# GabrieleCocco/CLFaceDetection

Hardware: AMD Instinct MI355X
Metric: candidate windows/sec, 1080p, haarcascade_frontalface_alt (higher is better)
Workload: dtype u32 gathers + f32 stage sums; 1 GPU; BASELINE config 3: 64x1920x1080 8-bit frames per step in the whole job (noise/smooth/blocks mix; sharded by whole frames over 1 GPU), haarcascade_frontalface_alt, scaleFactor 1.1f, raw candidates, frames resident in HBM; frames_on_rank_0=64, windows_per_frame=6290352, parallelism=single GPU, device=AMD Radeon Graphics (gfx950:sramecc+:xnack-), 256 CUs, pipeline=vj_stream, two batches in flight

## Files before the change

### clfacedetection_amd/api.py

```python
from __future__ import annotations

import ctypes as C
import os
from dataclasses import dataclass

import numpy as np

from .build import LIB_PATH, build_lib

VJ_MAX_STAGES = 64
VJ_FLAG_COUNTERS = 1 << 0
VJ_FLAG_SIGNED_MEAN = 1 << 1
VJ_FLAG_SKIP_LIST = 1 << 2
VJ_FLAG_SKIP_ROW = 1 << 3
VJ_FLAG_GRID_F64 = 1 << 4
VJ_FLAG_TILTED_AS_UPRIGHT = 1 << 5
VJ_FLAG_CV_CANNY_PRUNING = 1 << 6
VJ_FLAG_CV_SCALE_IMAGE = 1 << 7
VJ_FLAG_CV_FIND_BIGGEST = 1 << 8
VJ_FLAG_CV_ROUGH_SEARCH = 1 << 9
VJ_FLAG_CV_CHAIN_DEVICE = 1 << 10
VJ_FLAG_EQUALIZE_HIST = 1 << 11

CV_HAAR_DO_CANNY_PRUNING = 1
# ... 123 lines not shown
    _fields_ = [("min_w", C.c_int32), ("min_h", C.c_int32), ("max_w", C.c_int32), ("max_h", C.c_int32),
                ("scale_factor", C.c_double), ("min_neighbors", C.c_uint32), ("flags", C.c_uint32)]


class _RocResult(C.Structure):
    _fields_ = [("r", _Result), ("reject_levels", C.c_void_p), ("level_weights", C.c_void_p)]


WINDOW_DTYPE = np.dtype([("frame", "<i4"), ("x", "<i4"), ("y", "<i4"), ("scale", "<i4")])
WINDOW_RESULT_DTYPE = np.dtype([("result", "<i4"), ("reserved", "<i4"), ("stage_sum", "<f8")])
CLOD_WINDOW_RESULT_DTYPE = np.dtype([("result", "<i4"), ("variance", "<f4"), ("stage_sum", "<f4"), ("reserved", "<i4")])
VJ_WINDOW_OUTSIDE = -2**31
RECT_DTYPE = np.dtype([("x", "<i4"), ("y", "<i4"), ("w", "<i4"), ("h", "<i4"), ("weight", "<f4"),
                       ("frame", "<i4"), ("scale_idx", "<i4")])
STAGE_DTYPE = np.dtype([("first_tree", "<i4"), ("n_trees", "<i4"), ("threshold", "<f4"), ("parent", "<i4"),
                        ("next", "<i4"), ("child", "<i4")])
TREE_DTYPE = np.dtype([("first_node", "<i4"), ("n_nodes", "<i4"), ("first_alpha", "<i4")])
_RECT_DESC = np.dtype([("x", "<i4"), ("y", "<i4"), ("w", "<i4"), ("h", "<i4"), ("weight", "<f4")])
NODE_DTYPE = np.dtype([("n_rects", "<i4"), ("tilted", "<i4"), ("threshold", "<f4"), ("left", "<i4"),
                       ("right", "<i4"), ("rect", _RECT_DESC, 3)])

_SIGNATURES = {
    "vj_strerror": (C.c_char_p, [C.c_int]),
    "vj_last_error": (C.c_char_p, []),
    "vj_cascade_load_xml": (C.c_int, [C.c_char_p, C.POINTER(C.c_void_p)]),
    "vj_cascade_load": (C.c_int, [C.c_char_p, C.POINTER(C.c_void_p)]),
    "vj_cascade_save": (C.c_int, [C.c_void_p, C.c_char_p]),
    "vj_cascade_from_arrays": (C.c_int, [C.c_int, C.c_int, C.c_void_p, C.c_int, C.c_void_p, C.c_int, C.c_void_p, C.c_int,
                                         C.c_void_p, C.c_int, C.POINTER(C.c_void_p)]),
    "vj_cascade_free": (None, [C.c_void_p]),
    "vj_cascade_get_info": (C.c_int, [C.c_void_p, C.POINTER(CascadeInfo)]),
    "vj_cascade_stages": (C.c_void_p, [C.c_void_p]),
    "vj_cascade_trees": (C.c_void_p, [C.c_void_p]),
    "vj_cascade_nodes": (C.c_void_p, [C.c_void_p]),
    "vj_cascade_alpha": (C.c_void_p, [C.c_void_p]),
    "vj_cascade_notice": (C.c_char_p, [C.c_void_p]),
    "vj_params_default": (None, [C.POINTER(Params)]),
    "vj_plan_scales": (C.c_int, [C.c_void_p, C.c_int, C.c_int, C.POINTER(Params), C.POINTER(ScaleInfo), C.c_int,
                                 C.POINTER(C.c_int)]),
    "vj_plan_feature_table": (C.c_int, [C.c_void_p, C.c_int, C.POINTER(ScaleInfo), C.c_void_p, C.c_void_p]),
    "vj_plan_tiles": (C.c_int, [C.c_void_p, C.c_int, C.c_int, C.POINTER(Params), C.c_int, C.c_uint32, C.POINTER(TilePlanInfo),
                                C.POINTER(TileInfo), C.c_int, C.POINTER(C.c_int)]),
    "vj_plan_tiles_split": (C.c_int, [C.c_void_p, C.c_int, C.c_int, C.POINTER(Params), C.c_int, C.c_uint32, C.c_float,
                                      C.POINTER(TilePlanInfo), C.POINTER(TileCutInfo), C.POINTER(TileInfo), C.POINTER(C.c_uint64),
                                      C.c_int, C.POINTER(C.c_int)]),
    "vj_env_create": (C.c_int, [C.c_int, C.POINTER(C.c_void_p)]),
    "vj_env_destroy": (None, [C.c_void_p]),
    "vj_env_reserve": (C.c_int, [C.c_void_p, C.c_int, C.c_int, C.c_int]),
    "vj_env_device_name": (C.c_int, [C.c_void_p, C.c_char_p, C.c_size_t]),
    "vj_env_configure": (C.c_int, [C.c_void_p, C.c_char_p, C.c_char_p]),
    "vj_env_query": (C.c_int, [C.c_void_p, C.c_char_p, C.c_char_p, C.c_size_t]),
    "vj_integral": (C.c_int, [C.c_void_p, C.c_void_p, C.c_int, C.c_int, C.c_int, C.c_void_p, C.c_void_p]),
    "vj_integral_image": (C.c_int, [C.c_void_p, C.c_void_p, C.c_void_p, C.c_void_p]),
    "vj_integral_tilted": (C.c_int, [C.c_void_p, C.c_void_p, C.c_void_p]),
    "vj_grayscale": (C.c_int, [C.c_void_p, C.c_void_p, C.c_void_p, C.c_int]),
    "vj_canny": (C.c_int, [C.c_void_p, C.c_void_p, C.c_void_p, C.c_int]),
    "vj_equalize_hist": (C.c_int, [C.c_void_p, C.c_void_p, C.c_void_p, C.c_int]),
    "vj_resize_linear": (C.c_int, [C.c_void_p, C.c_void_p, C.c_int, C.c_int, C.c_void_p, C.c_int]),
    "vj_host_alloc": (C.c_int, [C.c_void_p, C.c_size_t, C.POINTER(C.c_void_p)]),
    "vj_host_free": (None, [C.c_void_p, C.c_void_p]),
    "vj_detect_chain": (C.c_int, [C.c_void_p, C.c_void_p, C.c_void_p, C.POINTER(_Image), C.c_int, C.POINTER(Params),
                                  C.POINTER(Params), C.POINTER(_Result), C.POINTER(_Result)]),
    "vj_stream_create": (C.c_int, [C.c_void_p, C.c_void_p, C.c_int, C.c_int, C.c_int, C.c_int, C.POINTER(Params),
                                   C.POINTER(C.c_void_p)]),
    "vj_stream_submit": (C.c_int, [C.c_void_p, C.POINTER(_Image), C.c_int]),
    "vj_stream_collect": (C.c_int, [C.c_void_p, C.POINTER(_Result)]),
    "vj_stream_destroy": (None, [C.c_void_p]),
    "vj_detect_rois": (C.c_int, [C.c_void_p, C.c_void_p, C.POINTER(_Image), C.c_int, C.c_void_p, C.c_int, C.POINTER(Params),
                                 C.POINTER(_Result)]),
    "vj_detect_opencv": (C.c_int, [C.c_void_p, C.c_void_p, C.POINTER(_Image), C.c_int, C.POINTER(CvParams),
                                   C.POINTER(_Result)]),
    "vj_detect_opencv_rois": (C.c_int, [C.c_void_p, C.c_void_p, C.POINTER(_Image), C.c_int, C.c_void_p, C.c_int, C.POINTER(CvParams),
                                        C.POINTER(_Result)]),
    "vj_detect_opencv_chain": (C.c_int, [C.c_void_p, C.c_void_p, C.c_void_p, C.POINTER(_Image), C.c_int, C.POINTER(CvParams),
                                         C.POINTER(CvParams), C.POINTER(_Result), C.POINTER(_Result)]),
    "vj_cv_params_default": (None, [C.POINTER(CvParams)]),
    "vj_cv_roc_params_default": (None, [C.POINTER(CvRocParams)]),
    "vj_detect_opencv_roc": (C.c_int, [C.c_void_p, C.c_void_p, C.POINTER(_Image), C.c_int, C.POINTER(CvRocParams),
                                       C.POINTER(_RocResult)]),
    "vj_roc_result_free": (None, [C.POINTER(_RocResult)]),
    "vj_run_windows_opencv": (C.c_int, [C.c_void_p, C.c_void_p, C.POINTER(_Image), C.c_int, C.c_void_p, C.c_int, C.c_void_p, C.c_uint32,
                                        C.c_int, C.c_void_p]),
    "vj_run_windows": (C.c_int, [C.c_void_p, C.c_void_p, C.POINTER(_Image), C.c_int, C.c_void_p, C.c_int, C.c_void_p, C.c_uint32,
                                 C.c_int, C.c_uint32, C.c_void_p]),
    "vj_run_windows_timing": (C.c_int, [C.c_void_p, C.POINTER(C.c_float), C.POINTER(C.c_float)]),
    "vj_cv_chain_info_get": (C.c_int, [C.c_void_p, C.POINTER(CvChainInfo)]),
    "vj_cv_rois_info_get": (C.c_int, [C.c_void_p, C.POINTER(CvRoisInfo)]),
    "vj_cv_plan_info_get": (C.c_int, [C.c_void_p, C.c_void_p, C.c_int, C.c_int, C.c_int, C.POINTER(CvParams), C.POINTER(CvPlanInfo)]),
    "vj_detect": (C.c_int, [C.c_void_p, C.c_void_p, C.POINTER(_Image), C.c_int, C.POINTER(Params),
                            C.POINTER(_Result)]),
    "vj_detect_mixed": (C.c_int, [C.c_void_p, C.c_void_p, C.POINTER(_Image), C.c_int, C.POINTER(Params), C.POINTER(MixedOpts),
                                  C.POINTER(_Result)]),
    "vj_detect_opencv_mixed": (C.c_int, [C.c_void_p, C.c_void_p, C.POINTER(_Image), C.c_int, C.POINTER(CvParams), C.POINTER(MixedOpts),
                                         C.POINTER(_Result)]),
    "vj_pack_frames": (C.c_int, [C.c_void_p, C.POINTER(_Image), C.c_int, C.c_uint64, C.c_void_p, C.c_int, C.POINTER(C.c_int),
                                 C.POINTER(C.c_int), C.c_void_p]),
    "vj_mixed_info_get": (C.c_int, [C.c_void_p, C.POINTER(MixedInfo)]),
    "vj_result_free": (None, [C.POINTER(_Result)]),
    "vj_group_rectangles": (C.c_int, [C.c_void_p, C.POINTER(C.c_uint32), C.c_int, C.c_double]),
    "vj_group_rectangles_levels": (C.c_int, [C.c_void_p, C.c_void_p, C.c_void_p, C.c_int, C.c_int, C.c_double]),
    "vj_count_windows": (C.c_int, [C.c_void_p, C.c_int, C.c_int, C.POINTER(Params), C.POINTER(C.c_uint64)]),
    "vj_shard_frames": (C.c_int, [C.c_int, C.c_int, C.c_int, C.POINTER(C.c_int), C.POINTER(C.c_int)]),
    "vj_shard_scales": (C.c_int, [C.c_void_p, C.c_int, C.c_int, C.POINTER(Params), C.c_int, C.c_int, C.POINTER(C.c_uint64)]),
}

_lib = None
# ... 172 lines not shown
    passes: list = None
    launches: list = None
    tile_split: float = 0.0
    balance_state: int = 0
    balance_calls: int = 0
    reject_levels: np.ndarray = None
    level_weights: np.ndarray = None

    @property
    def match_count(self) -> int:
        return len(self.rects)


class Environment:

    def __init__(self, device_index: int = 0):
        h = C.c_void_p()
        _check(load_library().vj_env_create(device_index, C.byref(h)), "vj_env_create")
        self._h = h

    @property
    def device_name(self) -> str:
        buf = C.create_string_buffer(256)
        _check(load_library().vj_env_device_name(self._h, buf, 256), "vj_env_device_name")
        return buf.value.decode()

    def configure(self, key: str, value) -> None:
        _check(load_library().vj_env_configure(self._h, key.encode(), str(value).encode()), f"vj_env_configure({key})")

    def query(self, key: str) -> str:
        buf = C.create_string_buffer(1024)
        _check(load_library().vj_env_query(self._h, key.encode(), buf, len(buf)), f"vj_env_query({key})")
        return buf.value.decode()

    def reserve(self, width: int, height: int, batch: int = 1):
        _check(load_library().vj_env_reserve(self._h, width, height, batch), "vj_env_reserve")

    def integral(self, gray: np.ndarray) -> tuple[np.ndarray, np.ndarray]:
        if gray.dtype != np.uint8 or gray.ndim not in (2, 3):
            raise ValueError("integral expects a 2-D uint8 image or a (h, w, 3|4) uint8 BGR/BGRA image")
        s = np.empty((gray.shape[0] + 1, gray.shape[1] + 1), np.uint32)
        q = np.empty((gray.shape[0] + 1, gray.shape[1] + 1), np.uint64)
        if gray.ndim == 3:
            g = _pixel_contiguous(gray)
            im = _Image(g.ctypes.data, g.shape[1], g.shape[0], g.strides[0], 0, g.shape[2])
            _check(load_library().vj_integral_image(self._h, C.byref(im), s.ctypes.data, q.ctypes.data), "vj_integral_image")
            return s, q
        g = gray if gray.strides[1] == 1 else np.ascontiguousarray(gray)
        h, w = g.shape
        _check(load_library().vj_integral(self._h, g.ctypes.data, w, h, g.strides[0], s.ctypes.data, q.ctypes.data),
               "vj_integral")
        return s, q

    def _one_image(self, img: np.ndarray):
        if img.dtype != np.uint8 or img.ndim not in (2, 3):
            raise ValueError("expected a 2-D uint8 image or a (h, w, 3|4) uint8 BGR/BGRA image")
        g = _pixel_contiguous(img) if img.ndim == 3 else (img if img.strides[1] == 1 else np.ascontiguousarray(img))
        return _Image(g.ctypes.data, g.shape[1], g.shape[0], g.strides[0], 0, g.shape[2] if g.ndim == 3 else 1), g

    def integral_tilted(self, img: np.ndarray) -> np.ndarray:
        im, keep = self._one_image(img)
        t = np.empty((img.shape[0] + 1, img.shape[1] + 1), np.uint32)
        _check(load_library().vj_integral_tilted(self._h, C.byref(im), t.ctypes.data), "vj_integral_tilted")
        return t

    def grayscale(self, img: np.ndarray) -> np.ndarray:
        im, keep = self._one_image(img)
        g = np.empty(img.shape[:2], np.uint8)
        _check(load_library().vj_grayscale(self._h, C.byref(im), g.ctypes.data, g.strides[0]), "vj_grayscale")
        return g

    def canny(self, img, color: bool = False) -> np.ndarray:
        imgs, n, keep = self._images(img, color)
        if n != 1:
            raise ValueError("canny takes one image")
        e = np.empty((imgs[0].height, imgs[0].width), np.uint8)
        _check(load_library().vj_canny(self._h, C.byref(imgs[0]), e.ctypes.data, e.strides[0]), "vj_canny")
        return e

    def equalize_hist(self, img, color: bool = False) -> np.ndarray:
        imgs, n, keep = self._images(img, color)
        if n != 1:
            raise ValueError("equalize_hist takes one image")
        d = np.empty((imgs[0].height, imgs[0].width), np.uint8)
        _check(load_library().vj_equalize_hist(self._h, C.byref(imgs[0]), d.ctypes.data, d.strides[0]), "vj_equalize_hist")
        return d

    def resize_linear(self, img, dst_w: int, dst_h: int, color: bool = False) -> np.ndarray:
        imgs, n, keep = self._images(img, color)
        if n != 1:
            raise ValueError("resize_linear takes one image")
        d = np.empty((int(dst_h), int(dst_w)), np.uint8)
        _check(load_library().vj_resize_linear(self._h, C.byref(imgs[0]), int(dst_w), int(dst_h), d.ctypes.data, d.strides[0]),
               "vj_resize_linear")
        return d

    def host_alloc(self, shape, dtype=np.uint8) -> np.ndarray:
        n = int(np.prod(shape)) * np.dtype(dtype).itemsize
        ptr = C.c_void_p()
        _check(load_library().vj_host_alloc(self._h, n, C.byref(ptr)), "vj_host_alloc")
        buf = (C.c_char * n).from_address(ptr.value)
        arr = np.frombuffer(buf, dtype).reshape(shape)
        self.__dict__.setdefault("_pinned", {})[arr.ctypes.data] = ptr.value
        return arr

    def host_free(self, arr: np.ndarray):
# ... 430 lines not shown
```

### clfacedetection_amd/build.py

```python
from __future__ import annotations

import os
import shutil
import subprocess
import sys

PKG_DIR = os.path.dirname(os.path.abspath(__file__))
CSRC = os.path.join(PKG_DIR, "csrc")
LIB_PATH = os.path.join(PKG_DIR, "libvjhip.so")
SOURCES = ["vj_cascade.cpp", "vj_plan.cpp", "vj_group.cpp", "vj_env.cpp", "vj_cv.cpp", "vj_cv_roi_host.cpp", "vj_cv_roi_levels_host.cpp", "vj_cv_points_host.cpp", "vj_points_host.cpp", "vj_points_driver.cpp", "vj_atlas_host.cpp", "vj_mixed.cpp", "vj_kernels.hip",
           "vj_cv_profile.hip", "vj_cv_tile.hip", "vj_group_dev.hip", "vj_canny.hip", "vj_pyramid.hip", "vj_cv_biggest.hip", "vj_cv_roi.hip", "vj_cv_chain.hip", "vj_cv_points.hip", "vj_points.hip", "vj_atlas.hip", "vj_equalize.hip"]
HEADERS = ["vj_internal.hpp", "vj_device.hpp", "vj_env_internal.hpp", "vj_devutil.hpp", "vj_cv_window.hpp", "vj_group_frame.hpp", "vj_cv_roi_units.hpp", "vj_cv_roi_host.hpp", "vj_cv_roi_levels_host.hpp", "vj_cv_points_units.hpp", "vj_cv_points_host.hpp", "vj_points_units.hpp", "vj_points_host.hpp", "vj_points_driver.hpp", "vj_clod_window.hpp", "vj_grid_parts.hpp", "vj_atlas_units.hpp", "vj_atlas_host.hpp", os.path.join("..", "..", "include", "vj.h")]
FLAGS = ["-O3", "-std=c++17", "-fPIC", "-ffp-contract=off", "-fno-fast-math", "--offload-arch=gfx950",
         "-Wall", "-Wno-unused-function", "-fvisibility=hidden", "-DVJ_BUILDING"] + \
    (["-DVJ_STAMPS=1"] if os.environ.get("VJ_STAMPS") else []) + \
    [f"-D{k}={v}" for k, v in (kv.split("=", 1) for kv in os.environ.get("VJ_DEFINES", "").split(",") if "=" in kv)]


def _hipcc() -> str:
    for cand in (os.environ.get("HIPCC"), shutil.which("hipcc"), "/opt/rocm/bin/hipcc"):
        if cand and os.path.exists(cand):
            return cand
    raise RuntimeError("hipcc not found; libvjhip.so cannot be built")


def _stale() -> bool:
    if not os.path.exists(LIB_PATH):
        return True
    t = os.path.getmtime(LIB_PATH)
    deps = [os.path.join(CSRC, s) for s in SOURCES + HEADERS] + [os.path.abspath(__file__)]
    return any(os.path.getmtime(d) > t for d in deps)


def build_lib(force: bool = False, verbose: bool = False) -> str:
    if not force and not _stale():
        return LIB_PATH
    objs = []
    build_dir = os.path.join(PKG_DIR, "build")
    os.makedirs(build_dir, exist_ok=True)
    hipcc = _hipcc()
    for src in SOURCES:
        obj = os.path.join(build_dir, os.path.splitext(src)[0] + ".o")
        cmd = [hipcc, *FLAGS, "-c", os.path.join(CSRC, src), "-o", obj]
        if verbose:
            print(" ".join(cmd), file=sys.stderr)
        r = subprocess.run(cmd, capture_output=True, text=True)
        if r.returncode != 0:
            raise RuntimeError(f"hipcc failed on {src}:\n{r.stdout}\n{r.stderr}")
        objs.append(obj)
    tmp = LIB_PATH + ".tmp"
    cmd = [hipcc, "-shared", "-fPIC", "--offload-arch=gfx950", *objs, "-o", tmp]
    r = subprocess.run(cmd, capture_output=True, text=True)
    if r.returncode != 0:
        raise RuntimeError(f"link failed:\n{r.stdout}\n{r.stderr}")
    os.replace(tmp, LIB_PATH)
    return LIB_PATH


if __name__ == "__main__":
    print(build_lib(force="--force" in sys.argv, verbose=True))
```

### clfacedetection_amd/csrc/vj_device.hpp

```cpp
#pragma once
#include <stdint.h>
#include "vj_cv_roi_units.hpp"

namespace vj {

struct ScaleDev {
    float    step;
    uint32_t nx;
    uint32_t nwin;
    uint32_t e_lt;
    uint32_t e_dw;
    uint32_t e_dh;
    float    area;
    uint32_t table_first;
    uint32_t q_base;
    uint32_t q_cap;
    uint32_t scale_idx;
    uint32_t ny;
    uint32_t tile_rw;
    uint32_t tile_pitch;
    uint32_t tile_rows;
    uint32_t tile_table_first;
    uint32_t te_lt;
    uint32_t te_dh;
    uint32_t tiles_x;
    uint32_t tile_tw;
    uint32_t tile_th;
    uint32_t tile_row_end;
    uint32_t tile_class;
    uint32_t tile_half;
    int32_t  te_dw;
    uint32_t skip_base;
    uint32_t skip_wpr;
    float    scale_f;
    uint32_t win_w, win_h;
    uint32_t pos_base;
    uint32_t grp_table_first;
    uint32_t grp_te_lt;
    uint32_t grp_te_dh;
    int32_t  grp_te_dw;
    uint32_t tile_tail_first;
    uint32_t grp_tail_first;
    uint32_t sq32;
};
static_assert(sizeof(ScaleDev) == 152, "ScaleDev is 152 bytes");

struct StageDev {
    uint32_t first_node;
    uint32_t n_nodes;
    float    threshold;
    int32_t  on_pass;
    int32_t  on_fail;
    uint32_t n_trees;
    uint32_t order;
    uint32_t sp_first;
    float    sp_delta;
    uint32_t cv_f64;
    uint32_t pad[2];
};
static_assert(sizeof(StageDev) == 48, "StageDev is 48 bytes");

struct UnitDev {
    uint32_t scale;
    uint32_t first;
    uint32_t count;
    uint32_t bw;
};

struct QEntry {
    uint32_t off;
    float    var;
};

struct DetEntry {
    uint32_t off;
    uint32_t scale;
};

struct RoiDev {
    int32_t frame, x, y, w, h;
};
struct RoiUnit {
    uint32_t roi;
    uint32_t slot;
    uint32_t first;
    uint32_t count;
    uint32_t nx, ny;
};
struct RoiDet {
    uint32_t off;
    uint32_t slot;
    uint32_t roi;
};
struct RoiTile {
    uint32_t roi;
    uint32_t slot;
    uint32_t first;
    uint32_t nxy;
    uint32_t twh;
};

struct SpBlock {
    uint32_t first_node;
    uint32_t desc;
};

constexpr int UNIT_WINDOWS = 512;
constexpr int WAVES_PER_BLOCK = 3;
constexpr int GATHER_WAVES_MAX = 4;
constexpr int MAX_SCALES = 128;
constexpr int MAX_PASSES = 8;
constexpr uint32_t Q_PARTS = 8;
constexpr int TILE_WAVES = 8;
constexpr int TILE_W = 64;
constexpr int TILE_WAVE_CAP = 256;
constexpr int TILE_CLASSES = 3;
constexpr int TILE_LDS_HEADER = (TILE_WAVES * TILE_WAVE_CAP * 2 + 32) * 4;
constexpr int TILE_SP_MAX_WINDOWS = 256;
constexpr int TILE_WS_MAX_WINDOWS = 512;
constexpr int TILE_SEG_MAX_WINDOWS = 256;
constexpr int TILE_SP_MAX_BLOCKS = 4;
constexpr int TILE_SP_BLOCK = 64;
constexpr int TILE_TAIL_BLOCK_RECS = (3 * 16 + 8) * TILE_SP_BLOCK / 64;
constexpr uint32_t SQ32_MAX_AREA = 66051;
static_assert(65025ull * SQ32_MAX_AREA < (1ull << 32) && 65025ull * (SQ32_MAX_AREA + 1ull) >= (1ull << 32), "SQ32_MAX_AREA");

struct CascadeArgs {
    const uint32_t* sum;
    const uint64_t* sqsum;
    const uint32_t* table;
    const ScaleDev* scales;
    const StageDev* stages;
    const UnitDev*  units;
    uint32_t n_units;
    const UnitDev*  tile_units;
    uint32_t n_tile_units;
    uint32_t tile_lds_bytes;
    uint32_t* tile_ticket;
    uint32_t n_frames;
    uint32_t n_scales;
    uint32_t frame_elems;
    uint32_t sum_bytes;
    uint32_t stride;
    uint32_t stage_begin, stage_end;
    uint32_t total_waves;
    uint32_t gather_waves;
    const QEntry*   q_in;
    const uint32_t* q_in_count;
    uint32_t* q_ticket;
    uint32_t wide_tail;
    uint32_t min_chunk;
    uint32_t q_slices;
    uint32_t* run_table;
    const UnitDev* q_groups;
    uint32_t n_q_groups;
    QEntry*   q_out;
    uint32_t* q_out_count;
    QEntry*   q_fail;
    uint32_t* q_fail_count;
    uint32_t  n_pass;
    uint32_t  pass_begin[MAX_PASSES + 1];
    QEntry*   q_pass[MAX_PASSES];
    uint32_t* q_pass_count[MAX_PASSES];
    uint32_t  tile_end;
    uint32_t  tile_min_lanes;
    unsigned long long tile_repack_mask;
    uint32_t  tile_sp_begin;
    uint32_t  identity_order;
    uint32_t  n_seg;
    uint32_t  seg_end[4];
    uint32_t  seg_chain;
    uint32_t  tree2;
    uint32_t  tile_ws_min;
    uint32_t  tile_ws_max;
    const SpBlock* sp_blocks;
    uint32_t  n_sp_blocks;
    DetEntry* det;
    uint32_t* det_count;
    uint32_t  det_cap;
    uint32_t  signed_mean;
    unsigned long long* stage_entered;
    unsigned long long* tree_ctr;
    unsigned long long* skip_bits;
    uint32_t  skip_frame_words;
    uint32_t  sp_tail_max;
    uint32_t  max_stage_nodes;
    uint32_t  gather_pairs;
    uint32_t  pos_mode;
    const uint32_t* pos_tab;
    const UnitDev* skip_units;
    uint32_t  n_skip_units;
    const UnitDev* skip_segs;
    uint32_t  n_skip_segs;
};

struct IntegralArgs {
    const uint8_t* gray;
    uint64_t gray_frame_bytes;
    uint32_t gray_stride;
    uint32_t channels;
    uint32_t width, height;
    uint32_t n_frames;
    uint32_t n_bands;
    uint32_t band_pitch;
    uint32_t* band_sum;
    uint32_t* band_sq;
    uint64_t* band_sq_prefix;
    uint32_t* sum;
    uint64_t* sqsum;
    uint32_t frame_elems;
    uint32_t rows_mode;
};
constexpr int BAND_ROWS = 8;

int launch_integral(const IntegralArgs& a, void* stream);
int launch_integral_sum(const IntegralArgs& a, void* stream);
int launch_cascade_pass(const CascadeArgs& a, bool from_grid, bool trees, bool last, bool count, bool general,
                        int n_blocks, void* stream);
int launch_cascade_tile_pass(const CascadeArgs& a, bool trees, bool count, int n_blocks, void* stream);

struct RoiArgs {
    const DetEntry* det_in;
    const uint32_t* det_in_count;
    uint32_t det_in_cap;
    const ScaleDev* scales_in;
    uint32_t frame_bytes;
    uint32_t stride;
    RoiDev* rois;
    uint32_t* n_rois;
    uint32_t max_rois;
    uint32_t n_frames;
    int32_t  frame_w, frame_h;
    int32_t  win_w0, win_h0;
    int32_t  min_w, min_h, max_w, max_h;
    RoiUnit* units;
    uint32_t* n_units;
    uint32_t max_units;
    uint32_t* ticket;
    RoiDet* det;
    uint32_t* det_count;
    uint32_t det_cap;
    RoiTile* tiles;
    uint32_t* n_tiles;
    uint32_t max_tiles;
    uint32_t tile_min_windows;
    uint32_t tile_blocks;
};
int launch_roi_chain(const RoiArgs& r, const CascadeArgs& a, bool from_dets, bool trees, bool count, bool general ,
                     int n_blocks, void* stream, void* stream2 , void* fork_ev, void* join_ev);

constexpr uint32_t GROUP_MAX = 2048;
struct GroupArgs {
    const DetEntry* det;
    const uint32_t* det_count;
    uint32_t det_cap;
    const ScaleDev* scales;
    uint32_t frame_bytes;
    uint32_t stride;
    uint32_t n_frames;
    int32_t  threshold;
    double   eps;
    uint32_t* frame_count;
    uint32_t* frame_cursor;
    uint32_t* grouped_count;
// ... 338 lines not shown
```

### clfacedetection_amd/csrc/vj_env.cpp

```cpp
#include "vj_internal.hpp"
#include "vj_device.hpp"

#include <hip/hip_runtime_api.h>

#include <algorithm>
#include <climits>
#include <cmath>
#include <cstdint>
#include <cstdio>
#include <cstdlib>
#include <cstring>
#include <map>
#include <memory>
#include <string>
#include <tuple>

#include "vj_env_internal.hpp"
#include "vj_grid_parts.hpp"
#include "vj_atlas_units.hpp"

using namespace vj;

namespace vj {

// ... 89 lines not shown
        set_error("stage links form a cycle");
        return VJ_ERR_UNSUPPORTED;
    }
    if (pl->general && e->general_prefix) {
        uint32_t P = 0;
        while (P + 1 < order.size() && order[P] == P && pl->prog.on_fail[P] == STAGE_REJECT &&
               pl->prog.on_pass[P] == (int)(P + 1) && order[P + 1] == P + 1)
            ++P;
        if (P >= 2) pl->general_prefix = P;
    }
    pl->scales_all = plan_scales(c, W, H, p);
    pl->frame_elems = frame_elems_for(W, H);
    const uint32_t stride = (uint32_t)W + 1u;
    const size_t n_nodes = c.nodes.size();

    const uint32_t tile_header_bytes = TILE_LDS_HEADER;
    uint32_t shape_header_bytes = tile_header_bytes;
    if (!pl->trees && !pl->general && e->tile_sp_begin < (int)c.stages.size()) {
        uint32_t mx = 0;
        for (size_t s = 0; s < c.stages.size(); ++s) mx = std::max(mx, pl->prog.n_nodes[s]);
        if (mx <= (uint32_t)TILE_SP_MAX_BLOCKS * TILE_SP_BLOCK) {
            pl->wave_tail = true;
            if (opt.former_shapes) shape_header_bytes += ((2u * 14u * (TILE_SP_BLOCK + 1u) + 2u * mx + 3u) & ~3u) * 4u;
        }
    }
    std::vector<NodeRec> table;
    std::vector<uint32_t> pos_tab;
    std::vector<std::pair<uint32_t, uint32_t>> tile_reach;
    for (const vj_scale_info& si : pl->scales_all) {
        if (!si.accepted || si.nx <= 0 || si.ny <= 0) continue;
        if ((p.scale_mask[0] | p.scale_mask[1]) != 0) {
            const int k = si.scale_idx;
            if (k >= 127 || !((p.scale_mask[k >> 6] >> (k & 63)) & 1ull)) continue;
        }
        if (pl->scales.size() >= (size_t)MAX_SCALES) {
            set_error("more than %d scales", MAX_SCALES);
            return VJ_ERR_LIMIT;
        }
        ScaleDev sd;
        memset(&sd, 0, sizeof(sd));
        sd.step = si.step;
        sd.nx = (uint32_t)si.nx;
        sd.nwin = (uint32_t)si.nx * (uint32_t)si.ny;
        sd.e_lt = (uint32_t)si.equ_y * stride + (uint32_t)si.equ_x;
        sd.e_dw = (uint32_t)si.equ_w;
        sd.e_dh = (uint32_t)si.equ_h * stride;
        sd.area = (float)si.area;
        sd.table_first = (uint32_t)table.size();
        sd.scale_idx = (uint32_t)si.scale_idx;
        sd.scale_f = si.scale;
        sd.win_w = (uint32_t)si.win_w;
        sd.win_h = (uint32_t)si.win_h;
        sd.sq32 = e->sq32 && (uint64_t)sd.win_w * sd.win_h <= SQ32_MAX_AREA ? 1u : 0u;
        table.resize(table.size() + n_nodes);
        int rc = build_node_table(c, W, si, table.data() + sd.table_first);
        if (rc) return rc;
        const uint32_t x_max = (uint32_t)std::lrint((double)((float)(si.nx - 1) * si.step)) + (pl->pos_mode != 0u ? 1u : 0u);
        const uint32_t y_max = (uint32_t)std::lrint((double)((float)(si.ny - 1) * si.step)) + (pl->pos_mode != 0u ? 1u : 0u);
        uint32_t reach = sd.e_lt + sd.e_dh + sd.e_dw;
        for (size_t k = 0; k < n_nodes; ++k) {
            const NodeRec& r = table[sd.table_first + k];
            const uint32_t dw[3] = {r.dw01 & 0xffffu, r.dw01 >> 16, r.dw2_flags & 0xffffu};
            for (int q = 0; q < 3; ++q)
                if (q < 2 || r.w[2] != 0.0f) reach = std::max(reach, (r.lt[q] + r.dh[q] + dw[q]) / 4u);
        }
        reach += y_max * stride + x_max;
        pl->max_reach_elems = std::max(pl->max_reach_elems, reach);
        pl->windows_per_frame += sd.nwin;
        sd.ny = (uint32_t)si.ny;
        if (pl->pos_mode & 2u) {
            if (pos_tab.empty()) pos_tab.push_back(0u);
            sd.pos_base = (uint32_t)pos_tab.size();
            const double stepd = std::max(2.0, (double)si.scale);
            const int n_pos = std::max(si.nx, si.ny) + 1;
            for (int i = 0; i < n_pos; ++i)
                pos_tab.push_back((pl->pos_mode & 1u) ? (uint32_t)std::round((double)i * stepd) : (uint32_t)std::lrint((double)i * stepd));
        }

        uint32_t reach_x = (uint32_t)(si.equ_x + si.equ_w), reach_y = (uint32_t)(si.equ_y + si.equ_h);
        for (size_t k = 0; k < n_nodes; ++k) {
            const NodeRec& r = table[sd.table_first + k];
            const uint32_t dw[3] = {r.dw01 & 0xffffu, r.dw01 >> 16, r.dw2_flags & 0xffffu};
            for (int q = 0; q < 3; ++q)
                if (q < 2 || r.w[2] != 0.0f) {
                    const uint32_t lt = r.lt[q] / 4u;
                    reach_x = std::max(reach_x, lt % stride + dw[q] / 4u);
                    reach_y = std::max(reach_y, lt / stride + (r.dh[q] / 4u) / stride);
                }
        }
        if ((!pl->general || pl->general_prefix) && si.ny < 65536 && si.nx < 65536) {
            static const uint32_t kTw[] = {64, 56, 48, 40, 32, 24, 16, 12, 8}, kTh[] = {32, 28, 24, 20, 16, 12, 8, 6, 4};
            auto former = [&](uint32_t v) { return opt.former_shapes && (v == 56u || v == 40u || v == 28u || v == 20u); };
            uint32_t best_cls = TILE_CLASSES, best_n = 0, b_tw = 0, b_th = 0, b_pitch = 0, b_rows = 0;
            for (uint32_t cls = 0; cls < TILE_CLASSES && best_n < (uint32_t)thresholds.min_windows; ++cls) {
                const int kb = e->tile_class_kb[cls];
                const uint32_t lds_cu = (160u - (uint32_t)e->tile_lds_reserve_kb) * 1024u;
                const uint64_t budget = kb < 0 ? ((lds_cu - 2048u) / (uint32_t)(-kb) - shape_header_bytes) & ~63ull
                                               : std::min<uint64_t>((uint64_t)kb * 1024u, 160u * 1024u - shape_header_bytes);
                for (uint32_t tw : kTw)
                    for (uint32_t th : kTh) {
                        const uint32_t nwt = tw * th;
                        if (nwt > TILE_WAVES * TILE_WAVE_CAP || nwt < 64 || nwt < best_n || (nwt == best_n && best_cls != cls)) continue;
                        if (former(tw) || former(th)) continue;
                        uint32_t pitch = (uint32_t)std::ceil((double)(tw - 1) * (double)si.step) + 3u + reach_x;
                        if (si.step != 2.0f) {
                            pitch = (pitch + 3u) & ~3u;
// ... 609 lines not shown
    }
    pl->last_used = ++e->plan_tick;
    *out = pl.get();
    e->plans[key] = std::move(pl);
    return VJ_OK;
}

int Lane::create() {
    for (auto& x : ev) HIP_TRY(hipEventCreate(&x));
    for (auto& x : pass_ev) HIP_TRY(hipEventCreate(&x));
    for (auto& x : launch_ev) HIP_TRY(hipEventCreate(&x));
    HIP_TRY(hipEventCreateWithFlags(&upload_done, hipEventDisableTiming));
    HIP_TRY(hipEventCreateWithFlags(&integral_done, hipEventDisableTiming));
    HIP_TRY(hipEventCreateWithFlags(&done, hipEventDisableTiming));
    h_pinned_bytes = (size_t)1 << 20;
    HIP_TRY(hipHostMalloc(&h_pinned, h_pinned_bytes, hipHostMallocDefault));
    return VJ_OK;
}

void Lane::destroy() {
    for (DevBuf* b : {&d_gray, &d_counts, &d_det, &d_eq_frames, &d_eq_hist, &d_eq_lut, &d_eq_gray}) b->release();
    if (h_pinned) (void)hipHostFree(h_pinned);
    if (h_stage) (void)hipHostFree(h_stage);
    h_pinned = h_stage = nullptr;
    for (auto& x : ev) if (x) (void)hipEventDestroy(x);
    for (auto& x : pass_ev) if (x) (void)hipEventDestroy(x);
    for (auto& x : launch_ev) if (x) (void)hipEventDestroy(x);
    for (hipEvent_t* x : {&upload_done, &integral_done, &done}) if (*x) (void)hipEventDestroy(*x);
}

int ensure_image_buffers(vj_env* e, int W, int H, int frames, bool need_gray, int channels, Lane* lane) {
    if (!lane) lane = &e->lane0;
    const size_t fe = frame_elems_for(W, H);
    const uint32_t n_bands = ((uint32_t)H + BAND_ROWS - 1) / BAND_ROWS;
    const uint32_t band_pitch = ((uint32_t)W + 3u) & ~3u;
    int rc;
    const size_t sum_bytes = fe * 4 * (size_t)frames, sq_bytes = fe * 8 * (size_t)frames;
    const bool grow = sum_bytes > e->d_sum.cap || sq_bytes > e->d_sqsum.cap;
    if ((rc = e->d_sum.ensure(sum_bytes))) return rc;
    if ((rc = e->d_sqsum.ensure(sq_bytes))) return rc;
    (void)grow;
    if (need_gray) {
        const size_t gstride = ((size_t)W * (size_t)channels + 3) & ~(size_t)3;
        if ((rc = lane->d_gray.ensure(gstride * (size_t)H * (size_t)frames))) return rc;
    }
    const size_t band_elems = (size_t)frames * n_bands * band_pitch;
    if ((rc = e->d_band_sum.ensure(band_elems * 4))) return rc;
    if ((rc = e->d_band_sq.ensure(band_elems * 4))) return rc;
    if ((rc = e->d_band_sqp.ensure(band_elems * 8))) return rc;
    return VJ_OK;
}

int enqueue_integral(vj_env* e, const uint8_t* d_gray, size_t frame_bytes, int stride, int W, int H, int frames,
                     int channels) {
    IntegralArgs ia;
    memset(&ia, 0, sizeof(ia));
    ia.channels = (uint32_t)channels;
    ia.gray = d_gray;
    ia.gray_frame_bytes = frame_bytes;
    ia.gray_stride = (uint32_t)stride;
    ia.width = (uint32_t)W;
    ia.height = (uint32_t)H;
    ia.n_frames = (uint32_t)frames;
    ia.n_bands = ((uint32_t)H + BAND_ROWS - 1) / BAND_ROWS;
    ia.band_pitch = ((uint32_t)W + 3u) & ~3u;
    ia.band_sum = (uint32_t*)e->d_band_sum.p;
    ia.band_sq = (uint32_t*)e->d_band_sq.p;
    ia.band_sq_prefix = (uint64_t*)e->d_band_sqp.p;
    ia.sum = (uint32_t*)e->d_sum.p;
    ia.sqsum = (uint64_t*)e->d_sqsum.p;
    ia.frame_elems = frame_elems_for(W, H);
    ia.rows_mode = (uint32_t)e->integral_rows_mode;
    const size_t used = (size_t)(W + 1) * (size_t)(H + 1);
    const bool zeroed = e->slack_w == W && e->slack_h == H && e->slack_frames >= frames && e->slack_sum == e->d_sum.p &&
                        e->slack_sq == e->d_sqsum.p;
    for (int f = 0; f < frames && !zeroed; ++f) {
        HIP_TRY(hipMemsetAsync((uint32_t*)e->d_sum.p + (size_t)f * ia.frame_elems + used, 0,
                               (ia.frame_elems - used) * 4, e->stream));
        HIP_TRY(hipMemsetAsync((uint64_t*)e->d_sqsum.p + (size_t)f * ia.frame_elems + used, 0,
                               (ia.frame_elems - used) * 8, e->stream));
    }
    if (!zeroed) {
        e->slack_w = W;
        e->slack_h = H;
        e->slack_frames = frames;
        e->slack_sum = e->d_sum.p;
        e->slack_sq = e->d_sqsum.p;
    }
    int hrc = launch_integral(ia, e->stream);
    if (hrc) {
        set_error("integral launch failed: %s", hipGetErrorString((hipError_t)hrc));
        return VJ_ERR_HIP;
    }
    return VJ_OK;
}

int enqueue_tilted(vj_env* e, const uint8_t* d_gray, size_t frame_bytes, int stride, int W, int H, int frames, int channels) {
    const uint32_t fe = frame_elems_for(W, H);
    int rc;
    if ((rc = e->d_tilted.ensure((size_t)fe * 4u * (size_t)frames))) return rc;
    HIP_TRY(hipMemsetAsync(e->d_tilted.p, 0, (size_t)fe * 4u * (size_t)frames, e->stream));
    TiltedArgs ta;
    memset(&ta, 0, sizeof(ta));
    ta.gray = d_gray;
    ta.gray_frame_bytes = frame_bytes;
    ta.gray_stride = (uint32_t)stride;
    ta.channels = (uint32_t)channels;
    ta.width = (uint32_t)W;
    ta.height = (uint32_t)H;
    ta.n_frames = (uint32_t)frames;
    ta.frame_elems = fe;
    ta.tilted = (uint32_t*)e->d_tilted.p;
    const size_t n_bands = ((size_t)H + 7u) / 8u;
    if ((rc = e->d_tilt_diag.ensure((size_t)frames * n_bands * 2u * (size_t)(W + H) * 4u))) return rc;
    if ((rc = e->d_tilt_col.ensure((size_t)frames * n_bands * (size_t)(W + 1) * 4u))) return rc;
    const int hrc = launch_tilted_bands(ta, (uint32_t*)e->d_tilt_diag.p, (uint32_t*)e->d_tilt_col.p, e->stream);
    if (hrc) {
        set_error("tilted integral launch failed (width %d): %s", W, hipGetErrorString((hipError_t)hrc));
        return hrc == (int)hipErrorInvalidValue ? VJ_ERR_LIMIT : VJ_ERR_HIP;
    }
    return VJ_OK;
}

int image_channels(const vj_image& im) { return im.channels <= 1 ? 1 : im.channels; }

int stage_frames(vj_env* e, const vj_image* frames, int n, int W, int H, const uint8_t** d_ptr, size_t* frame_bytes,
                 int* stride, Lane* lane, hipStream_t copy_stream) {
    if (!lane) lane = &e->lane0;
    hipStream_t cs = copy_stream ? copy_stream : e->stream;
    const size_t row_bytes = (size_t)W * (size_t)image_channels(frames[0]);
    bool all_dev = true, contiguous = true;
    for (int i = 0; i < n; ++i) {
        if (!frames[i].on_device) all_dev = false;
        if (i > 0 && (frames[i].stride != frames[0].stride ||
                      frames[i].data != frames[0].data + (size_t)i * (size_t)frames[0].stride * (size_t)H))
            contiguous = false;
    }
    if (all_dev && contiguous) {
        *d_ptr = frames[0].data;
        *stride = frames[0].stride;
// ... 119 lines not shown
        return VJ_ERR_LIMIT;
    }
    std::vector<AtlasFrameDev> recs((size_t)frames);
    for (int i = 0; i < frames; ++i)
        recs[(size_t)i] = AtlasFrameDev{*d_gray + (size_t)i * *frame_bytes, (uint32_t)*stride, (uint32_t)*channels, (uint32_t)W, (uint32_t)H, 0u, 0u,
                                        (uint32_t)(units_per_frame * (uint64_t)i), eq_hist_units((uint32_t)H) * (uint32_t)i};
    if ((rc = lane->d_eq_frames.ensure(recs.size() * sizeof(AtlasFrameDev)))) return rc;
    if ((rc = lane->d_eq_gray.ensure((size_t)pitch * (size_t)H * (size_t)frames))) return rc;
    HIP_TRY(hipMemcpyAsync(lane->d_eq_frames.p, recs.data(), recs.size() * sizeof(AtlasFrameDev), hipMemcpyHostToDevice, e->stream));
    const uint8_t* lut;
    if ((rc = enqueue_equalize_tables(e, lane, lane->d_eq_frames.p, (uint32_t)frames, eq_hist_units((uint32_t)H) * (uint32_t)frames, &lut))) return rc;
    EqualizeArgs a;
    memset(&a, 0, sizeof(a));
    a.frames = (const AtlasFrameDev*)lane->d_eq_frames.p;
    a.n_frames = (uint32_t)frames;
    a.n_units = (uint32_t)(units_per_frame * (uint64_t)frames);
    a.lut = (uint8_t*)lane->d_eq_lut.p;
    a.dst = (uint8_t*)lane->d_eq_gray.p;
    a.dst_pitch = pitch;
    a.dst_h = (uint32_t)H;
    a.dst_frame_bytes = (uint64_t)pitch * (uint64_t)H;
    const int hrc = launch_equalize_apply(a, e->stream);
    if (hrc) {
        set_error("equalization launch failed: %s", hipGetErrorString((hipError_t)hrc));
        return VJ_ERR_HIP;
    }
    *d_gray = (const uint8_t*)lane->d_eq_gray.p;
    *frame_bytes = (size_t)pitch * (size_t)H;
    *stride = (int)pitch;
    *channels = 1;
    return VJ_OK;
}

struct RawDet {
    int frame;
    uint32_t slot, x, y;
};

struct CountsLayout {
    static constexpr size_t q_counts = (size_t)MAX_SCALES * Q_PARTS;
    static constexpr size_t stage_off_u32 = MAX_PASSES * q_counts + 2;
    static constexpr size_t roi_off_u32 = stage_off_u32 + (size_t)(1 + VJ_MAX_LAUNCHES) * VJ_MAX_STAGES * 2;
    static constexpr size_t q2_off_u32 = roi_off_u32 + 8 + (size_t)VJ_MAX_STAGES * 2;
    static constexpr size_t bytes = (q2_off_u32 + MAX_PASSES * q_counts) * sizeof(uint32_t);
    static constexpr size_t pass_tickets_end = (size_t)MAX_PASSES * Q_PARTS;
    static constexpr size_t tile_tickets_begin = q_counts - 8u * TILE_CLASSES;
    static constexpr size_t roi_tickets_begin = q_counts - 40u;
};
static_assert(GRID_PARTS == Q_PARTS, "the grid pass's tickets are pass 0's range of queue 0's counters");
static_assert(CountsLayout::pass_tickets_end <= CountsLayout::roi_tickets_begin, "pass tickets (the grid pass's among them) end before the region pass's");
static_assert(CountsLayout::roi_tickets_begin + 8u <= CountsLayout::tile_tickets_begin, "the region pass's tile tickets end before the tile classes'");

static int enqueue_prepare(vj_env* e, Lane* L, Plan* pl, const vj_image* frames, int nf, int W, int H, bool fixed_queue_layout,
                           hipStream_t copy_stream, bool equalize = false) {
    int rc;
    int channels = image_channels(frames[0]);
    if ((rc = ensure_image_buffers(e, W, H, nf, true, channels, L))) return rc;
    uint64_t q_entries = 0;
    if (!fixed_queue_layout) {
        if ((rc = layout_queues(pl, nf, &q_entries))) return rc;
        const size_t n_pass = pl->pass_bounds.size() - 1;
        for (size_t ps = 1; ps < n_pass; ++ps)
            if ((rc = e->d_q[ps].ensure(std::max<uint64_t>(q_entries, 1) * sizeof(QEntry)))) return rc;
    }
    if ((rc = L->d_counts.ensure(CountsLayout::bytes))) return rc;
    if (L->det_cap == 0) {
        L->det_cap = e->det_cap_init;
        if ((rc = L->d_det.ensure((size_t)L->det_cap * sizeof(DetEntry)))) return rc;
    }
    const uint8_t* d_gray;
    size_t gray_frame_bytes;
    int gray_stride;
    if ((rc = stage_frames(e, frames, nf, W, H, &d_gray, &gray_frame_bytes, &gray_stride, L, copy_stream))) return rc;
    if (copy_stream) {
        HIP_TRY(hipEventRecord(L->upload_done, copy_stream));
        HIP_TRY(hipStreamWaitEvent(e->stream, L->upload_done, 0));
    }
    HIP_TRY(hipEventRecord(L->ev[0], e->stream));
    if (equalize && (rc = enqueue_equalize(e, L, &d_gray, &gray_frame_bytes, &gray_stride, &channels, W, H, nf))) return rc;
    L->src_gray = d_gray;
    L->src_frame_bytes = gray_frame_bytes;
    L->src_stride = gray_stride;
    L->src_channels = channels;
    if ((rc = enqueue_integral(e, d_gray, gray_frame_bytes, gray_stride, W, H, nf, channels))) return rc;
    HIP_TRY(hipEventRecord(L->ev[1], e->stream));
    HIP_TRY(hipEventRecord(L->integral_done, e->stream));
    L->nf = nf;
    return VJ_OK;
}

static int enqueue_cascade(vj_env* e, Lane* L, Plan* pl, int W, int , const vj_params& p) {
    int rc;
    const int nf = L->nf;
    const size_t n_pass = pl->pass_bounds.size() - 1;
    const size_t counts_bytes = CountsLayout::bytes;
    constexpr size_t q_counts = CountsLayout::q_counts;
    uint32_t* d_qcount[MAX_PASSES];
    for (int ps = 0; ps < MAX_PASSES; ++ps) d_qcount[ps] = (uint32_t*)L->d_counts.p + ps * q_counts;
    uint32_t* d_qcount2[MAX_PASSES];
    for (int ps = 0; ps < MAX_PASSES; ++ps) d_qcount2[ps] = (uint32_t*)L->d_counts.p + CountsLayout::q2_off_u32 + ps * q_counts;
    uint32_t* d_det_count = (uint32_t*)L->d_counts.p + MAX_PASSES * q_counts;
    unsigned long long* d_stage_entered = (unsigned long long*)((uint32_t*)L->d_counts.p + CountsLayout::stage_off_u32);
    const bool count = (p.flags & VJ_FLAG_COUNTERS) != 0;
    const int n_blocks = std::max(1, e->n_cu * e->blocks_per_cu);
    {
        HIP_TRY(hipMemsetAsync(L->d_counts.p, 0, counts_bytes, e->stream));
        HIP_TRY(hipEventRecord(L->ev[2], e->stream));
        CascadeArgs ca;
        memset(&ca, 0, sizeof(ca));
        ca.sum = (const uint32_t*)e->d_sum.p;
        ca.sqsum = (const uint64_t*)e->d_sqsum.p;
        ca.table = (const uint32_t*)pl->d_table.p;
        ca.scales = (const ScaleDev*)pl->d_scales.p;
        ca.stages = (const StageDev*)pl->d_stages.p;
        ca.units = (const UnitDev*)pl->d_units.p;
        ca.n_units = (uint32_t)pl->units.size();
        ca.tile_units = (const UnitDev*)pl->d_tile_units.p;
        ca.n_tile_units = (uint32_t)pl->tile_units.size();
        ca.n_frames = (uint32_t)nf;
        ca.n_scales = (uint32_t)pl->scales.size();
        ca.frame_elems = pl->frame_elems;
        ca.sum_bytes = (uint32_t)((uint64_t)pl->frame_elems * 4u * (uint64_t)nf);
        ca.stride = (uint32_t)W + 1u;
        ca.gather_waves = (uint32_t)e->gather_waves_for(nf, pl->general);
        ca.total_waves = (uint32_t)n_blocks * ca.gather_waves;
        ca.det = (DetEntry*)L->d_det.p;
        ca.det_count = d_det_count;
        ca.det_cap = L->det_cap;
        ca.signed_mean = (p.flags & VJ_FLAG_SIGNED_MEAN) ? 1u : 0u;
        ca.stage_entered = d_stage_entered;
        ca.tree_ctr = d_stage_entered;
        ca.n_pass = (uint32_t)n_pass;
        for (size_t ps = 0; ps <= n_pass; ++ps) ca.pass_begin[ps] = pl->pass_bounds[ps];
        for (size_t ps = 1; ps < n_pass; ++ps) {
            ca.q_pass[ps] = (QEntry*)e->d_q[ps].p;
            ca.q_pass_count[ps] = d_qcount[ps];
        }
        ca.tile_end = pl->general ? pl->general_prefix : (uint32_t)e->tile_end;
        ca.tile_min_lanes = (uint32_t)e->tile_min_lanes;
        ca.tile_repack_mask = e->tile_repack_mask;
        ca.tile_sp_begin = (!pl->general && (pl->wave_tail || pl->tree2)) ? (uint32_t)e->tile_sp_begin : 0xffffffffu;
        ca.tree2 = pl->tree2 ? 1u : 0u;
        ca.identity_order = pl->general ? 0u : 1u;
        ca.n_seg = e->tile_segments ? pl->tile_n_seg : 0u;
        for (int k = 0; k < 4; ++k) ca.seg_end[k] = pl->tile_seg_end[k];
        ca.seg_chain = pl->tile_seg_chain;
        ca.sp_blocks = (const SpBlock*)pl->d_sp_blocks.p;
        ca.n_sp_blocks = pl->n_sp_blocks;
        ca.tile_ws_min = pl->wave_tail ? (uint32_t)e->tile_ws_min : 0u;
        ca.tile_ws_max = (uint32_t)std::min(e->tile_ws_max, (int)TILE_WS_MAX_WINDOWS);
        ca.pos_mode = pl->pos_mode;
        ca.pos_tab = (const uint32_t*)pl->d_pos_tab.p;
        ca.gather_pairs = e->pairs_for(nf);
        ca.sp_tail_max = (uint32_t)std::max(0, std::min(e->sp_tail_max, 48));
        ca.max_stage_nodes = pl->max_stage_nodes;
        if (pl->skip_mode && pl->n_skip_units) {
            if ((rc = e->d_skip_bits.ensure((size_t)pl->skip_frame_words * 8u * (size_t)nf))) return rc;
            ca.skip_bits = (unsigned long long*)e->d_skip_bits.p;
            ca.skip_frame_words = pl->skip_frame_words;
            ca.skip_units = (const UnitDev*)pl->d_skip_units.p;
            ca.n_skip_units = pl->n_skip_units;
            ca.skip_segs = (const UnitDev*)pl->d_skip_segs.p;
            ca.n_skip_segs = pl->n_skip_segs;
            const int hrc = launch_skip_bitmap(ca, pl->trees, std::max(1, e->n_cu * 4), e->stream);
// ... 145 lines not shown
            for (size_t ps = split_sets ? 1 : first_joint_pass; ps < n_pass && !hrc; ++ps) {
                if (ps > first_joint_pass && ps < VJ_MAX_PASSES) HIP_TRY(hipEventRecord(L->pass_ev[ps], e->stream));
                CascadeArgs qa = queue_args(ps, split_sets ? 1 : 0);
                if ((rc = begin_launch(VJ_LAUNCH_QUEUE, 0, qa.stage_begin, qa.stage_end, 0, e->stream))) return rc;
                qa.stage_entered = launch_counters();
                hrc = launch_cascade_pass(qa, false, pl->trees, pass_is_last(ps), count, general_kernel, n_blocks, e->stream);
                if ((rc = end_launch(e->stream))) return rc;
            }
            if (hrc) {
                set_error("cascade launch failed: %s", hipGetErrorString((hipError_t)hrc));
                return VJ_ERR_HIP;
            }
            launches = (int)n_pass;
        }
        if (n_pass <= VJ_MAX_PASSES && launches) HIP_TRY(hipEventRecord(L->pass_ev[n_pass], e->stream));
        HIP_TRY(hipEventRecord(L->ev[3], e->stream));
        L->launches = launches;
    }
    L->n_pass = n_pass;
    L->count = count;
    HIP_TRY(hipMemcpyAsync(L->h_pinned, L->d_counts.p, counts_bytes, hipMemcpyDeviceToHost, e->stream));
    const size_t room = (L->h_pinned_bytes - ((counts_bytes + 255) & ~(size_t)255)) / sizeof(DetEntry);
    L->det_copied = (uint32_t)std::min<size_t>(room, L->det_cap);
    HIP_TRY(hipMemcpyAsync((char*)L->h_pinned + ((counts_bytes + 255) & ~(size_t)255), L->d_det.p, (size_t)L->det_copied * sizeof(DetEntry),
                           hipMemcpyDeviceToHost, e->stream));
    HIP_TRY(hipEventRecord(L->done, e->stream));
    L->pending = true;
    return VJ_OK;
}

static int finish_batch(vj_env* e, Lane* L, Plan* pl, int f0, int W, int H, const vj_params& p, std::vector<RawDet>* dets,
                        vj_counters* ctr, vj_timing* tm, std::vector<DetEntry>* raw_out = nullptr) {
    int rc;
    constexpr size_t q_counts = CountsLayout::q_counts;
    const size_t counts_bytes = CountsLayout::bytes;
    for (int attempt = 0; attempt < 3; ++attempt) {
        HIP_TRY(hipEventSynchronize(L->done));
        L->pending = false;
        const size_t n_pass = L->n_pass;
        const int launches = L->launches;
        const bool count = L->count;
        const std::vector<vj_launch>& linfo = L->linfo;
        const uint32_t n_det = ((const uint32_t*)L->h_pinned)[MAX_PASSES * q_counts];
        float ms_i = 0, ms_c = 0, ms_t = 0;
        HIP_TRY(hipEventElapsedTime(&ms_i, L->ev[0], L->ev[1]));
        HIP_TRY(hipEventElapsedTime(&ms_c, L->ev[2], L->ev[3]));
        HIP_TRY(hipEventElapsedTime(&ms_t, L->ev[0], L->ev[3]));
        if (n_det > L->det_cap) {
            const uint32_t want = grown_cap(L->det_cap, n_det);
            if ((rc = L->d_det.ensure((size_t)want * sizeof(DetEntry)))) return rc;
            L->det_cap = want;
            if (L->shared_integrals) {
                HIP_TRY(hipEventRecord(L->ev[0], e->stream));
                if ((rc = enqueue_integral(e, L->src_gray, L->src_frame_bytes, L->src_stride, W, H, L->nf, L->src_channels))) return rc;
                HIP_TRY(hipEventRecord(L->ev[1], e->stream));
            }
            if ((rc = enqueue_cascade(e, L, pl, W, H, p))) return rc;
            continue;
        }
        if (attempt == 0) tm->integral_ms += ms_i;
        tm->cascade_ms += ms_c;
        tm->total_ms += ms_t;
        if (launches && n_pass <= VJ_MAX_PASSES)
            for (size_t ps = 0; ps < n_pass; ++ps) {
                float ms = 0;
                HIP_TRY(hipEventElapsedTime(&ms, L->pass_ev[ps], L->pass_ev[ps + 1]));
                tm->pass_ms[ps] += ms;
                tm->pass_stage_begin[ps] = (int32_t)pl->pass_bounds[ps];
                tm->pass_stage_end[ps] = (int32_t)pl->pass_bounds[ps + 1];
            }
        tm->n_cascade_launches = std::max(tm->n_cascade_launches, launches);
        const unsigned long long* se_all = (const unsigned long long*)((const uint32_t*)L->h_pinned + CountsLayout::stage_off_u32);
        if (linfo.size() <= VJ_MAX_LAUNCHES) {
            for (size_t i = 0; i < linfo.size(); ++i) {
                float ms = 0;
                HIP_TRY(hipEventElapsedTime(&ms, L->launch_ev[2 * i], L->launch_ev[2 * i + 1]));
                vj_launch acc = tm->launch[i];
                tm->launch[i] = linfo[i];
                tm->launch[i].ms = acc.ms + ms;
                const unsigned long long* se = se_all + (1 + i) * VJ_MAX_STAGES;
                for (size_t s = 0; s < (size_t)VJ_MAX_STAGES; ++s)
                    tm->launch[i].stage_entered[s] = acc.stage_entered[s] + (count ? se[s] : 0ull);
            }
            tm->n_launches = (int32_t)linfo.size();
        }
#ifdef VJ_STAMPS
        if (getenv("VJ_DEBUG_STAMPS")) {
            const unsigned long long* se = se_all;
            for (size_t l = 0; l < linfo.size(); ++l)
                fprintf(stderr, "vj launch %zu kind %d class %d: max resident workgroups %llu\n", l, linfo[l].kind, linfo[l].lds_class,
                        se[(1 + l) * VJ_MAX_STAGES + 39]);
            for (size_t l = 0; l < linfo.size(); ++l)
                if (linfo[l].kind == 1)
                    fprintf(stderr, "vj queue launch %zu [%d,%d): chunks %llu sum %llu max %llu | tail A %llu B %llu pairs %llu stages %llu\n", l,
                            linfo[l].stage_begin, linfo[l].stage_end, se[(1 + l) * VJ_MAX_STAGES + 50], se[(1 + l) * VJ_MAX_STAGES + 48],
                            se[(1 + l) * VJ_MAX_STAGES + 49], se[(1 + l) * VJ_MAX_STAGES + 51], se[(1 + l) * VJ_MAX_STAGES + 52],
                            se[(1 + l) * VJ_MAX_STAGES + 53], se[(1 + l) * VJ_MAX_STAGES + 54]);
            for (size_t l = 0; l < linfo.size(); ++l)
                if (linfo[l].kind == VJ_LAUNCH_GRID) {
                    const unsigned long long* g = se + (1 + l) * VJ_MAX_STAGES + 40;
                    const double wgs = (double)std::max(1ull, g[5]), span = (double)(g[3] - ~g[4]);
                    fprintf(stderr, "vj grid launch %zu: workgroups %llu span %.0f ticks | per workgroup last - mean wave end: mean %.0f (%.2f %%) max %llu (%.2f %%) | "
                            "launch end - mean last wave end %.0f (%.2f %%)\n", l, g[5], span, (double)g[0] / wgs, 100.0 * (double)g[0] / wgs / span, g[1],
                            100.0 * (double)g[1] / span, (double)g[3] - (double)g[2] / wgs, 100.0 * ((double)g[3] - (double)g[2] / wgs) / span);
                }
            fprintf(stderr, "vj stamps:");
            for (int i = 40; i < 60; ++i) {
                unsigned long long v = 0;
                for (int l = 1; l <= VJ_MAX_LAUNCHES; ++l) v += se[l * VJ_MAX_STAGES + i];
                fprintf(stderr, " %llu", v);
            }
            fprintf(stderr, "\n");
        }
#endif
        if (count) {
            for (size_t s = 0; s < pl->stages.size(); ++s)
                for (int l = 1; l <= VJ_MAX_LAUNCHES; ++l) ctr->stage_entered[s] += se_all[(size_t)l * VJ_MAX_STAGES + s];
            ctr->stump_evals += se_all[0];
            ctr->gather_bytes += se_all[1];
        }
        std::vector<DetEntry> raw(n_det);
        const uint32_t have = std::min(n_det, L->det_copied);
        if (have) memcpy(raw.data(), (const char*)L->h_pinned + ((counts_bytes + 255) & ~(size_t)255), (size_t)have * sizeof(DetEntry));
        if (n_det > have)
            HIP_TRY(hipMemcpy(raw.data() + have, (const DetEntry*)L->d_det.p + have, (size_t)(n_det - have) * sizeof(DetEntry),
                              hipMemcpyDeviceToHost));
        const uint32_t stride = (uint32_t)W + 1u;
        const uint64_t fbytes = (uint64_t)pl->frame_elems * 4u;
        for (const DetEntry& d : raw) {
            const uint32_t f = (uint32_t)(d.off / fbytes);
            const uint32_t el = (uint32_t)((d.off - (uint64_t)f * fbytes) / 4u);
            dets->push_back(RawDet{f0 + (int)f, d.scale, el % stride, el / stride});
        }
        if (raw_out) *raw_out = std::move(raw);
        return VJ_OK;
    }
    set_error("detection buffer overflow persisted");
    return VJ_ERR_LIMIT;
}

static int detect_subbatch(vj_env* e, Plan* pl, const vj_image* frames, int f0, int nf, int W, int H,
                           const vj_params& p, bool equalize, std::vector<RawDet>* dets, vj_counters* ctr, vj_timing* tm) {
    int rc;
    Lane* L = &e->lane0;
    if ((rc = enqueue_prepare(e, L, pl, frames + f0, nf, W, H, false, nullptr, equalize))) return rc;
    if ((rc = enqueue_cascade(e, L, pl, W, H, p))) return rc;
    return finish_batch(e, L, pl, f0, W, H, p, dets, ctr, tm);
}

static void fill_counters(Plan* pl, int n_frames, const vj_params& p, vj_result* out) {
    if (!(p.flags & VJ_FLAG_COUNTERS)) return;
    vj_counters& k = out->counters;
    k.windows = pl->windows_per_frame * (uint64_t)n_frames;
    const uint64_t child_nodes = k.stump_evals, child_rects = k.gather_bytes;
    uint64_t rect_evals = pl->trees ? child_rects : 0;
    k.stump_evals = pl->trees ? child_nodes : 0;
    for (size_t s = 0; s < pl->stages.size(); ++s) {
        k.stump_evals += k.stage_entered[s] * (pl->trees ? pl->prog.n_roots[s] : pl->prog.n_nodes[s]);
        rect_evals += k.stage_entered[s] * (pl->trees ? pl->prog.n_root_rects[s] : pl->prog.n_rects[s]);
    }
    k.gather_bytes = 48ull * k.windows + 16ull * rect_evals;
}

static int build_result(Plan* pl, std::vector<RawDet>& dets, int n_frames, const vj_params& p, vj_result* out) {
    std::sort(dets.begin(), dets.end(), [](const RawDet& a, const RawDet& b) {
        return std::tie(a.frame, a.slot, a.y, a.x) < std::tie(b.frame, b.slot, b.y, b.x);
    });
    out->count = (uint32_t)dets.size();
    if (!dets.empty()) {
        out->rects = (vj_rect*)malloc(dets.size() * sizeof(vj_rect));
        if (!out->rects) return VJ_ERR_NOMEM;
        for (size_t i = 0; i < dets.size(); ++i) {
            const vj_scale_info& si = pl->scales_info[dets[i].slot];
            out->rects[i] = vj_rect{(int32_t)dets[i].x, (int32_t)dets[i].y, si.win_w, si.win_h, 0.0f, dets[i].frame,
                                    si.scale_idx};
        }
    }
    if (p.min_neighbors != 0 && out->count) {
        const int rc = vj_group_rectangles(out->rects, &out->count, (int)std::max<uint32_t>(p.min_neighbors, 1u), 0.2);
        if (rc) return rc;
    }
    fill_counters(pl, n_frames, p, out);
    return VJ_OK;
}

static uint64_t max_frames_per_subbatch(const vj_env* e, const Plan* pl) {
    const uint64_t frame_bytes = (uint64_t)pl->frame_elems * 4u;
    uint64_t max_frames = (0xffffffffull - (uint64_t)pl->max_reach_elems * 4u - 16u) / frame_bytes;
    const uint64_t q_budget = 6ull << 30;
    auto fit_parts = [](uint64_t frames_worth) {
        return frames_worth >= Q_PARTS ? frames_worth / Q_PARTS * Q_PARTS : std::max<uint64_t>(1, frames_worth);
    };
    if (pl->windows_per_frame) {
        max_frames = std::min<uint64_t>(max_frames, fit_parts(q_budget / (pl->windows_per_frame * sizeof(QEntry))));
        max_frames = std::min<uint64_t>(max_frames, fit_parts(0xffffffffull / pl->windows_per_frame));
    }
    if (e->max_subbatch > 0) max_frames = std::min<uint64_t>(max_frames, (uint64_t)e->max_subbatch);
    return max_frames;
// ... 241 lines not shown
        }
    }
    if (p->min_neighbors != 0 && out->count) {
        rc = vj_group_rectangles(out->rects, &out->count, (int)std::max<uint32_t>(p->min_neighbors, 1u), 0.2);
        if (rc) return rc;
    }
    if (count2) {
        vj_counters& k = out->counters;
        k.windows = k.stage_entered[0];
        uint64_t rect_evals = 0;
        for (size_t s2 = 0; s2 < pl2->stages.size(); ++s2) {
            k.stump_evals += k.stage_entered[s2] * (pl2->trees ? pl2->prog.n_roots[s2] : pl2->prog.n_nodes[s2]);
            rect_evals += k.stage_entered[s2] * (pl2->trees ? pl2->prog.n_root_rects[s2] : pl2->prog.n_rects[s2]);
        }
        if (pl2->trees) {
            k.stump_evals += child2_nodes;
            rect_evals += child2_rects;
        }
        k.gather_bytes = 48ull * k.windows + 16ull * rect_evals;
    }
    return VJ_OK;
}


extern "C" {

int vj_env_create(int device_index, vj_env** out) {
    if (!out) return VJ_ERR_ARG;
    *out = nullptr;
    int n = 0;
    hipError_t he = hipGetDeviceCount(&n);
    if (he != hipSuccess || n <= 0) {
        set_error("no HIP device (hipGetDeviceCount: %s); this library has no CPU fallback",
                  he == hipSuccess ? "0 devices" : hipGetErrorString(he));
        return VJ_ERR_NO_DEVICE;
    }
    if (device_index < 0 || device_index >= n) {
        set_error("device_index %d out of range [0,%d)", device_index, n);
        return VJ_ERR_ARG;
    }
    auto e = std::make_unique<vj_env>();
    e->device = device_index;
    HIP_TRY(hipSetDevice(device_index));
    hipDeviceProp_t prop;
    HIP_TRY(hipGetDeviceProperties(&prop, device_index));
    snprintf(e->name, sizeof(e->name), "%s (%s)", prop.name, prop.gcnArchName);
    if (strncmp(prop.gcnArchName, "gfx950", 6) != 0) {
        set_error("device %d is %s; the kernels are built for gfx950 only", device_index, prop.gcnArchName);
        return VJ_ERR_NO_DEVICE;
    }
    e->n_cu = prop.multiProcessorCount;
    if (const char* g = getenv("VJ_TILE_GROUP")) e->tile_group = std::max(1, std::min(atoi(g), (int)MAX_SCALES));
    if (const char* g = getenv("VJ_SQ32")) e->sq32 = atoi(g) != 0;
    if (const int hrc = prepare_tile_kernels()) {
        set_error("raising the dynamic LDS limit on device %d failed: %s", device_index, hipGetErrorString((hipError_t)hrc));
        return VJ_ERR_HIP;
    }
    if (const int hrc = prepare_cv_tile_kernels()) {
        set_error("raising the dynamic LDS limit on device %d failed: %s", device_index, hipGetErrorString((hipError_t)hrc));
        return VJ_ERR_HIP;
    }
    if (const int hrc = prepare_group_kernels()) {
        set_error("raising the dynamic LDS limit on device %d failed: %s", device_index, hipGetErrorString((hipError_t)hrc));
        return VJ_ERR_HIP;
    }
    if (const int hrc = prepare_cv_chain_kernels()) {
        set_error("raising the dynamic LDS limit on device %d failed: %s", device_index, hipGetErrorString((hipError_t)hrc));
        return VJ_ERR_HIP;
    }
    if (const int hrc = prepare_cv_biggest_kernels()) {
        set_error("raising the dynamic LDS limit on device %d failed: %s", device_index, hipGetErrorString((hipError_t)hrc));
        return VJ_ERR_HIP;
    }
    HIP_TRY(hipStreamCreateWithFlags(&e->stream, hipStreamNonBlocking));
    { const int lrc = e->lane0.create(); if (lrc) return lrc; }
    HIP_TRY(hipEventCreateWithFlags(&e->fork_ev, hipEventDisableTiming));
    HIP_TRY(hipEventCreateWithFlags(&e->join_ev, hipEventDisableTiming));
    for (hipEvent_t& ev : e->cv_chain_ev) HIP_TRY(hipEventCreate(&ev));
    for (hipEvent_t& ev : e->cv_rois_ev) HIP_TRY(hipEventCreate(&ev));
    for (hipEvent_t& ev : e->atlas_ev) HIP_TRY(hipEventCreate(&ev));
    HIP_TRY(hipStreamCreateWithFlags(&e->stream2, hipStreamNonBlocking));
    *out = e.release();
    return VJ_OK;
}

void vj_env_destroy(vj_env* e) {
    if (!e) return;
    (void)hipSetDevice(e->device);
    if (e->stream) (void)hipStreamSynchronize(e->stream);
    drop_plans(e);
    for (DevBuf* b : {&e->d_sum, &e->d_sqsum, &e->d_band_sum, &e->d_band_sq, &e->d_band_sqp, &e->d_tilted, &e->d_tilt_diag, &e->d_tilt_col, &e->d_out,
                      &e->d_skip_bits, &e->d_rois, &e->d_roi_units, &e->d_roi_det, &e->d_roi_tiles, &e->d_group, &e->d_cv_det, &e->d_cv_counts,
                      &e->d_cv_accept, &e->d_cv_tq, &e->d_cv_fail_rows, &e->d_cv_fail_walk, &e->d_run_table,
                      &e->d_canny_cls, &e->d_canny_label, &e->d_canny_flag, &e->d_edges, &e->d_edge_sum,
                      &e->d_cv_prune_bits, &e->d_pyr, &e->d_pyr_tab, &e->d_cv_big, &e->d_cv_rois, &e->d_cv_roi_units,
                      &e->d_cv_chain, &e->d_cv_chain_keys, &e->d_cv_chain_staged, &e->d_cv_roi_first, &e->d_cv_det2, &e->d_cv_counts2,
                      &e->d_cv_rl_levels, &e->d_cv_rl_taps, &e->d_cv_rl_scales, &e->d_cv_rl_rows, &e->d_cv_rl_table, &e->d_cv_rl_stages,
                      &e->d_points, &e->d_point_units, &e->d_point_scales, &e->d_point_out, &e->d_atlas, &e->d_atlas_src})
        b->release();
    e->lane0.destroy();
    for (DevBuf& b : e->d_q) b.release();
    for (DevBuf& b : e->d_q2) b.release();
    for (hipEvent_t& ev : e->cv_chain_ev)
        if (ev) (void)hipEventDestroy(ev);
    for (hipEvent_t& ev : e->cv_rois_ev)
        if (ev) (void)hipEventDestroy(ev);
// ... 279 lines not shown
                set_error("%s: expected comma-separated integers, got '%s'", key, value);
                return VJ_ERR_ARG;
            }
            e->*k->v = std::vector<int>(x.begin(), x.end());
            break;
        }
        case Kind::Custom:
            if (const int rc = k->set(e, value)) return rc;
    }
    if (k->effects & SET_THRESHOLDS) e->tile_thresholds_set = true;
    if (k->effects & SET_SPLIT) e->tile_split_set = true;
    if (k->effects & CLEAR_BALANCE) e->balance.clear();
    if (k->effects & (DROP_PLANS | DROP_CV_PLANS)) HIP_TRY(hipStreamSynchronize(e->stream));
    if (k->effects & DROP_PLANS) drop_plans(e);
    if (k->effects & DROP_CV_PLANS) {
        for (auto& kv : e->cv_plans) kv.second->release_device();
        e->cv_plans.clear();
        for (auto& kv : e->cv_roi_plans) kv.second->release_device();
        e->cv_roi_plans.clear();
        drop_cv_point_plans(e);
    }
    return VJ_OK;
}

int vj_env_reserve(vj_env* e, int max_w, int max_h, int max_batch) {
    if (!e || max_w <= 0 || max_h <= 0 || max_batch <= 0) return VJ_ERR_ARG;
    HIP_TRY(hipSetDevice(e->device));
    return ensure_image_buffers(e, max_w, max_h, max_batch, true);
}

int vj_integral_image(vj_env* e, const vj_image* image, uint32_t* sum, uint64_t* sqsum) {
    if (!e || !image || !image->data || !sum || !sqsum) return VJ_ERR_ARG;
    const int w = image->width, h = image->height, ch = image_channels(*image);
    if (w <= 0 || h <= 0 || (ch != 1 && ch != 3 && ch != 4) || image->stride < w * ch) return VJ_ERR_ARG;
    if ((uint64_t)(w + 1) * (uint64_t)(h + 3) >= (1ull << 30)) {
        set_error("image too large");
        return VJ_ERR_LIMIT;
    }
    HIP_TRY(hipSetDevice(e->device));
    int rc;
    if ((rc = ensure_image_buffers(e, w, h, 1, true, ch))) return rc;
    const uint8_t* d_gray;
    size_t fb;
    int gs;
    if ((rc = stage_frames(e, image, 1, w, h, &d_gray, &fb, &gs))) return rc;
    if ((rc = enqueue_integral(e, d_gray, fb, gs, w, h, 1, ch))) return rc;
    const size_t n = (size_t)(w + 1) * (size_t)(h + 1);
    HIP_TRY(hipMemcpyAsync(sum, e->d_sum.p, n * 4, hipMemcpyDeviceToHost, e->stream));
    HIP_TRY(hipMemcpyAsync(sqsum, e->d_sqsum.p, n * 8, hipMemcpyDeviceToHost, e->stream));
    HIP_TRY(hipStreamSynchronize(e->stream));
    return VJ_OK;
}

}

namespace vj {
int check_single_image(const vj_image* image, int* ch_out) {
    const int w = image->width, h = image->height, ch = image_channels(*image);
    if (w <= 0 || h <= 0 || (ch != 1 && ch != 3 && ch != 4) || image->stride < w * ch) return VJ_ERR_ARG;
    if ((uint64_t)(w + 1) * (uint64_t)(h + 3) >= (1ull << 30)) {
        set_error("image too large");
        return VJ_ERR_LIMIT;
    }
    *ch_out = ch;
    return VJ_OK;
}
}

extern "C" {

int vj_integral_tilted(vj_env* e, const vj_image* image, uint32_t* tilted) {
    if (!e || !image || !image->data || !tilted) return VJ_ERR_ARG;
    int ch, rc;
    if ((rc = check_single_image(image, &ch))) return rc;
    const int w = image->width, h = image->height;
    HIP_TRY(hipSetDevice(e->device));
    if ((rc = ensure_image_buffers(e, w, h, 1, true, ch))) return rc;
    const uint8_t* d_gray;
    size_t fb;
    int gs;
    if ((rc = stage_frames(e, image, 1, w, h, &d_gray, &fb, &gs))) return rc;
    if ((rc = enqueue_tilted(e, d_gray, fb, gs, w, h, 1, ch))) return rc;
    HIP_TRY(hipMemcpyAsync(tilted, e->d_tilted.p, (size_t)(w + 1) * (size_t)(h + 1) * 4, hipMemcpyDeviceToHost, e->stream));
    HIP_TRY(hipStreamSynchronize(e->stream));
    return VJ_OK;
}

int vj_grayscale(vj_env* e, const vj_image* image, uint8_t* gray, int gray_stride) {
    if (!e || !image || !image->data || !gray || gray_stride < image->width) return VJ_ERR_ARG;
    int ch, rc;
    if ((rc = check_single_image(image, &ch))) return rc;
    const int w = image->width, h = image->height;
    HIP_TRY(hipSetDevice(e->device));
    if ((rc = ensure_image_buffers(e, w, h, 1, true, ch))) return rc;
    const uint8_t* d_src;
    size_t fb;
    int gs;
    if ((rc = stage_frames(e, image, 1, w, h, &d_src, &fb, &gs))) return rc;
    const size_t pitch = ((size_t)w + 3) & ~(size_t)3;
    if ((rc = e->d_out.ensure(pitch * (size_t)h))) return rc;
    TiltedArgs ta;
    memset(&ta, 0, sizeof(ta));
    ta.gray = d_src;
    ta.gray_frame_bytes = fb;
    ta.gray_stride = (uint32_t)gs;
    ta.channels = (uint32_t)ch;
// ... 519 lines not shown
        vj_stream* s;
        ~Guard() { if (s) vj_stream_destroy(s); }
    } guard{nullptr};
    const vj_env::Balance* bal = balance_of(e, c, width, height, *p, max_batch, false);
    TileThresholds sth{e->tile_min_windows, e->tile_accept_windows, e->tile_max_dwords_per_window};
    if (bal && balance_choice(bal, -1).thr == 1 && !e->tile_thresholds_set) sth = TileThresholds{std::min(384, sth.min_windows), std::min(384, sth.accept_windows), sth.max_dwords_per_window};
    int rc = build_plan(e, *c, width, height, *p, s->plan.get(), bal ? bal->best : e->split_for(max_batch, *p), sth);
    if (rc) {
        s->plan->release_device();
        return rc;
    }
    vj_stream* raw = s.release();
    guard.s = raw;
    if ((uint64_t)max_batch > max_frames_per_subbatch(e, raw->plan.get())) {
        set_error("max_batch %d exceeds what one launch sequence can address at this frame size (%llu frames)", max_batch,
                  (unsigned long long)max_frames_per_subbatch(e, raw->plan.get()));
        return VJ_ERR_LIMIT;
    }
    for (Lane& L : raw->lanes) {
        if ((rc = L.create())) return rc;
        L.shared_integrals = true;
    }
    HIP_TRY(hipStreamCreateWithFlags(&raw->copy, hipStreamNonBlocking));
    for (Lane& L : raw->lanes)
        if ((rc = ensure_image_buffers(e, width, height, max_batch, true, CH, &L))) return rc;
    uint64_t q_entries = 0;
    if ((rc = layout_queues(raw->plan.get(), max_batch, &q_entries))) return rc;
    const size_t n_pass = raw->plan->pass_bounds.size() - 1;
    for (size_t ps = 1; ps < n_pass; ++ps)
        if ((rc = e->d_q[ps].ensure(std::max<uint64_t>(q_entries, 1) * sizeof(QEntry)))) return rc;
    guard.s = nullptr;
    *out = raw;
    return VJ_OK;
}

int vj_stream_submit(vj_stream* s, const vj_image* frames, int n_frames) {
    if (!s || !frames || n_frames <= 0 || n_frames > s->max_batch) return VJ_ERR_ARG;
    if (s->n_pending >= 2) {
        set_error("two batches are pending: collect one before submitting the next");
        return VJ_ERR_LIMIT;
    }
    int W, H, CH;
    int rc = check_frames(frames, n_frames, &W, &H, &CH);
    if (rc) return rc;
    if (W != s->W || H != s->H || CH != s->CH) {
        set_error("frames do not have the stream's size / channel count");
        return VJ_ERR_ARG;
    }
    vj_env* e = s->e;
    HIP_TRY(hipSetDevice(e->device));
    const int lane = s->n_pending == 0 ? 0 : 1 - s->fifo[0];
    Lane* L = &s->lanes[lane];
    HIP_TRY(hipEventSynchronize(L->integral_done));
    if ((rc = enqueue_prepare(e, L, s->plan.get(), frames, n_frames, W, H, true, s->copy))) return rc;
    if ((rc = enqueue_cascade(e, L, s->plan.get(), W, H, s->p))) return rc;
    s->fifo[s->n_pending] = lane;
    s->n_frames_of[lane] = n_frames;
    s->n_pending++;
    return VJ_OK;
}

int vj_stream_collect(vj_stream* s, vj_result* out) {
    if (!s || !out) return VJ_ERR_ARG;
    memset(out, 0, sizeof(*out));
    if (s->n_pending == 0) {
        set_error("no batch is pending");
        return VJ_ERR_ARG;
    }
    vj_env* e = s->e;
    HIP_TRY(hipSetDevice(e->device));
    const int lane = s->fifo[0];
    s->fifo[0] = s->fifo[1];
    s->n_pending--;
    Lane* L = &s->lanes[lane];
    std::vector<RawDet> dets;
    int rc = finish_batch(e, L, s->plan.get(), 0, s->W, s->H, s->p, &dets, &out->counters, &out->timing);
    if (rc) return rc;
    return build_result(s->plan.get(), dets, s->n_frames_of[lane], s->p, out);
}

void vj_stream_destroy(vj_stream* s) {
    if (!s) return;
    (void)hipSetDevice(s->e->device);
    if (s->e->stream) (void)hipStreamSynchronize(s->e->stream);
    if (s->e->stream2) (void)hipStreamSynchronize(s->e->stream2);
    if (s->copy) {
        (void)hipStreamSynchronize(s->copy);
        (void)hipStreamDestroy(s->copy);
    }
    for (Lane& L : s->lanes) L.destroy();
    if (s->plan) s->plan->release_device();
    delete s;
}

void vj_result_free(vj_result* r) {
    if (!r) return;
    free(r->rects);
    r->rects = nullptr;
    r->count = 0;
}

static int plan_tiles_query(const vj_cascade* c, int width, int height, const vj_params* p, int n_frames, uint32_t flags, float tile_split,
                            vj_tile_plan_info* info, vj_tile_cut_info* cut, vj_tile_info* out, uint64_t* gather_windows, int cap, int* n) {
    if (!c || !p || !n || width <= 0 || height <= 0 || n_frames <= 0 || (cap > 0 && !out) || tile_split != tile_split ||
        (flags & ~(uint32_t)(VJ_PLAN_TILES_FORMER_SHAPES | VJ_PLAN_TILES_NO_GROUPS)))
        return VJ_ERR_ARG;
    int rc = check_params(*p);
// ... 83 lines not shown
```

### clfacedetection_amd/csrc/vj_env_internal.hpp

```cpp
#pragma once
#include "vj_internal.hpp"
#include "vj_device.hpp"
#include "vj_cv_roi_host.hpp"
#include "vj_cv_points_host.hpp"
#include "vj_points_host.hpp"

#include <hip/hip_runtime_api.h>

#include <algorithm>
#include <cstring>
#include <map>
#include <memory>
#include <tuple>
#include <type_traits>
#include <vector>

namespace vj {

#define HIP_TRY(expr)                                                                        \
    do {                                                                                     \
        hipError_t e_ = (expr);                                                              \
        if (e_ != hipSuccess) {                                                              \
            set_error("%s failed: %s (%s:%d)", #expr, hipGetErrorString(e_), __FILE__, __LINE__); \
            return VJ_ERR_HIP;                                                               \
// ... 104 lines not shown
    StageProgram prog;
    uint32_t n_stages = 0, n_order = 0;
    bool trees = false, is_tree = false, has_tilted = false, tree2 = false;
    DevBuf d_table, d_scales, d_stages;
    std::vector<double> factor_values;
    DevBuf d_chain_factors;
    uint32_t chain_factors_n = 0;
    uint64_t last_used = 0;
    void release_device() {
        for (DevBuf* b : {&d_table, &d_scales, &d_stages, &d_chain_factors}) b->release();
        chain_factors_n = 0;
    }
};

struct PointCascade {
    uint32_t n_stages = 0, n_order = 0;
    bool trees = false, is_tree = false, has_tilted = false, tree2 = false;
    DevBuf d_stages;
    uint64_t last_used = 0;
    void release_device() { d_stages.release(); }
};
template <class ScaleDev>
struct PointPlan {
    typedef std::remove_cv_t<std::remove_pointer_t<decltype(ScaleDev::table)>> Node;
    ScaleDev rec = {};
    uint64_t max_reach = 0;
    DevBuf d_table;
    uint64_t last_used = 0;
    void release_device() { d_table.release(); }
};

}

namespace vj {


struct Lane {
    DevBuf d_gray, d_counts, d_det;
    DevBuf d_eq_frames, d_eq_hist, d_eq_lut, d_eq_gray;
    uint32_t det_cap = 0;
    void* h_pinned = nullptr;
    size_t h_pinned_bytes = 0;
    void* h_stage = nullptr;
    size_t h_stage_bytes = 0;
    hipEvent_t ev[4] = {};
    hipEvent_t pass_ev[VJ_MAX_PASSES + 1] = {};
    hipEvent_t launch_ev[2 * VJ_MAX_LAUNCHES] = {};
    hipEvent_t upload_done = nullptr, integral_done = nullptr, done = nullptr;
    bool pending = false;
    int nf = 0, first_frame = 0;
    const uint8_t* src_gray = nullptr;
    size_t src_frame_bytes = 0;
    int src_stride = 0, src_channels = 1;
    bool shared_integrals = false;
    size_t n_pass = 0;
    int launches = 0;
    bool count = false;
    uint32_t det_copied = 0;
    std::vector<vj_launch> linfo;
    int create();
    void destroy();
};

}

namespace vj {

struct Tunables {
    int max_subbatch = 0;
    uint32_t det_cap_init = 1u << 16;
    int concurrent = 1;
    int gather_waves = -1;
    int gather_waves_for(int n_frames, bool general) const {
        if (general) return vj::WAVES_PER_BLOCK;
        const int w = gather_waves > 0 ? gather_waves : (n_frames >= 8 ? vj::GATHER_WAVES_MAX : vj::WAVES_PER_BLOCK);
        return std::min(std::max(w, 1), (int)vj::GATHER_WAVES_MAX);
    }
    int concurrent_blocks_per_cu = 1;
    float tile_split = 1.25f;
    float tile_split_mid = 1.75f;
    float tile_split_small = 0.0f;
    int one_pass_max_frames = 0;
    float split_for(int n_frames) const {
        return n_frames <= 4 ? tile_split_small : n_frames < 8 ? std::min(tile_split_mid, 0.5f) : n_frames < 32 ? tile_split_mid : tile_split;
    }
    float split_for(int n_frames, const vj_params& p) const {
        return ((p.scale_mask[0] | p.scale_mask[1]) != 0 && !tile_split_set) ? 0.0f : split_for(n_frames);
    }
    int tile_segments = 1;
    int seg_cut2 = 0;
    int general_prefix = 1;
    int grid_block_w = 32;
    int tile_lds_reserve_kb = 16;
    int roi_tile_min_windows = 512;
    int balance_class(int n_frames) const {
        return n_frames < 8 ? n_frames : n_frames < 16 ? 8 : n_frames < 32 ? 16 : n_frames < 64 ? 32 : 64;
    }
    bool auto_balance = true, tile_split_set = false;
    int plan_cache_max = 48;
    int integral_rows_mode = 2;
    int blocks_per_cu = 8;
    int tile_class_kb[vj::TILE_CLASSES] = {-2, -1, 0};
    int tile_min_windows = 768;
    int tile_max_dwords_per_window = 600;
    bool tile_thresholds_set = false;
    int tile_accept_windows = 768;
    int tile_end = 64;
    int tile_min_lanes = 0;
    unsigned long long tile_repack_mask = ~3ull;
    int tile_sp_begin = 3;
    int tile_ws_max = 512;
    int tile_ws_min = 48;
    int group_max = (int)vj::GROUP_MAX;
    bool tree_split_queues = true;
    bool cv_tiles = true;
    int cv_tile_ws_max = 512;
    int cv_row_blocks = -1;
    int cv_row_blocks_tree = 2, cv_tile_min_windows_tree = 256;
    int cv_tail_max = 64;
    int cv_tree_chunk = 64, cv_tree_chain_blocks = 2;
    bool cv_tiles_tilted = true;
    bool cv_tree2 = true;
    int cv_row_band_px = 128;
    bool cv_tree_chains = true;
    int cv_tree_queue_cap = 0;
    int cv_tile_min_windows0 = 2048;
    int cv_tile_min_windows = -1;
    bool rois_on_device = true;
    int wide_tail = -1;
    int min_chunk = 32;
    int q_band_px = 128;
    int q_group_units = 4;
    int q_band_min_frames = 8;
    int q_slices = -1;
    int sp_tail_max = 48;
    int gather_pairs = -1;
    uint32_t pairs_for(int n_frames) const { return gather_pairs >= 0 ? (uint32_t)gather_pairs : n_frames <= 4 ? 2u : 0u; }
    std::vector<int> split_override;
    std::vector<int> pass_cut_nodes{35};
};

}

struct vj_env : vj::Tunables {
    int device = 0;
    int tile_group = 4;
    bool sq32 = true;
    hipStream_t stream = nullptr;
    vj::Lane lane0;
    hipEvent_t fork_ev = nullptr, join_ev = nullptr;
    hipStream_t stream2 = nullptr;
    char name[256] = "";
    int n_cu = 0;
    vj::DevBuf d_sum, d_sqsum, d_band_sum, d_band_sq, d_band_sqp;
    vj::DevBuf d_tilted;
    vj::DevBuf d_tilt_diag, d_tilt_col;
    vj::DevBuf d_out;
    int slack_w = 0, slack_h = 0, slack_frames = 0;
    void *slack_sum = nullptr, *slack_sq = nullptr;
    vj::DevBuf d_q[vj::MAX_PASSES];
    vj::DevBuf d_q2[vj::MAX_PASSES];
    vj::DevBuf d_skip_bits;
    vj::DevBuf d_run_table;
    vj::DevBuf d_rois, d_roi_units, d_roi_det, d_roi_tiles;
    uint32_t roi_tile_cap = 0;
    vj::DevBuf d_group;
    uint32_t roi_unit_cap = 0, roi_det_cap = 0;
    typedef std::tuple<uint64_t, int, int, int, int, int, int, uint32_t, uint64_t, uint64_t, uint32_t, uint32_t> PlanKey;
    std::map<PlanKey, std::unique_ptr<vj::Plan>> plans;
    struct Balance {
        float cur = 0, best = 0, best_ms = 0, cand_ms = 0;
        int phase = 0;
        int samples = 0, moved = 0, calls = 0;
        int thr = 0;
        bool thr_tried = false, far_tried = false;
        int n_ref = 0;
        int off_ref = 0;
        bool first_slow = false;
        uint64_t last_used = 0;
        uint32_t calls_total = 0, calls_on_candidate = 0;
    };
    typedef std::tuple<PlanKey, int> BalanceKey;
    std::map<BalanceKey, Balance> balance;
    uint64_t balance_tick = 0;
    typedef std::tuple<uint64_t, int, int, int, int, uint64_t, int, int> CvPlanKey;
    std::map<CvPlanKey, std::unique_ptr<vj::CvPlan>> cv_plans;
    typedef std::tuple<uint64_t, int, uint64_t> CvRoiPlanKey;
    std::map<CvRoiPlanKey, std::unique_ptr<vj::CvRoiPlan>> cv_roi_plans;
    vj::DevBuf d_cv_rois, d_cv_roi_units;
    vj::DevBuf d_cv_chain, d_cv_chain_keys, d_cv_chain_staged, d_cv_roi_first, d_cv_det2, d_cv_counts2;
    hipEvent_t cv_chain_ev[3] = {};
    vj_cv_chain_info cv_chain_info = {};
    vj::DevBuf d_cv_rl_levels, d_cv_rl_taps, d_cv_rl_scales, d_cv_rl_rows, d_cv_rl_table, d_cv_rl_stages;
    hipEvent_t cv_rois_ev[2] = {};
    vj_cv_rois_info cv_rois_info = {};
    typedef std::map<uint64_t, std::unique_ptr<vj::PointCascade>> PointCascades;
    PointCascades cv_point_cascades, clod_point_cascades;
    typedef std::tuple<uint64_t, int, uint64_t> CvPointPlanKey;
    std::map<CvPointPlanKey, std::unique_ptr<vj::PointPlan<vj::CvPointScaleDev>>> cv_point_plans;
    typedef std::tuple<uint64_t, int, uint32_t, int> ClodPointPlanKey;
    std::map<ClodPointPlanKey, std::unique_ptr<vj::PointPlan<vj::ClodPointScaleDev>>> clod_point_plans;
    float points_integral_ms = 0, points_pass_ms = 0;
    vj::DevBuf d_points, d_point_units, d_point_scales, d_point_out;
    vj::DevBuf d_cv_det, d_cv_counts;
    vj::DevBuf d_cv_accept, d_cv_tq;
    vj::DevBuf d_cv_fail_rows, d_cv_fail_walk;
    vj::DevBuf d_canny_cls, d_canny_label, d_canny_flag, d_edges, d_edge_sum, d_cv_prune_bits;
    vj::DevBuf d_pyr, d_pyr_tab;
    vj::DevBuf d_cv_big;
    int edge_slack_w = 0, edge_slack_h = 0, edge_slack_frames = 0;
    void* edge_slack_sum = nullptr;
    vj::DevBuf d_atlas, d_atlas_src;
    hipEvent_t atlas_ev[2] = {};
    vj_mixed_info mixed_info = {};
    uint64_t plan_tick = 0;
    int cv_tq_shift = 4;
};

namespace vj {
int image_channels(const vj_image& im);
int check_single_image(const vj_image* image, int* ch_out);
uint32_t frame_elems_for(int W, int H);
int ensure_image_buffers(vj_env* e, int W, int H, int frames, bool need_gray, int channels = 1, Lane* lane = nullptr);
int enqueue_integral(vj_env* e, const uint8_t* d_gray, size_t frame_bytes, int stride, int W, int H, int frames,
                     int channels = 1);
int stage_frames(vj_env* e, const vj_image* frames, int n, int W, int H, const uint8_t** d_ptr, size_t* frame_bytes,
                 int* stride, Lane* lane = nullptr, hipStream_t copy_stream = nullptr);
int enqueue_tilted(vj_env* e, const uint8_t* d_gray, size_t frame_bytes, int stride, int W, int H, int frames, int channels);
int enqueue_equalize(vj_env* e, Lane* lane, const uint8_t** d_gray, size_t* frame_bytes, int* stride, int* channels, int W, int H, int frames);
int enqueue_equalize_tables(vj_env* e, Lane* lane, const void* d_frame_recs, uint32_t n_frames, uint32_t n_hist_units, const uint8_t** lut);
int refuse_equalize(uint32_t flags, const char* entry_point);

template <typename Map>
void point_make_room(vj_env* e, Map& m, uint64_t call_tick) {
    while ((int)m.size() >= std::max(1, e->plan_cache_max)) {
        auto lru = m.end();
        for (auto i = m.begin(); i != m.end(); ++i)
            if (i->second->last_used < call_tick && (lru == m.end() || i->second->last_used < lru->second->last_used)) lru = i;
        if (lru == m.end()) return;
        lru->second->release_device();
        m.erase(lru);
    }
}
}
```

### clfacedetection_amd/csrc/vj_kernels.hip

```cpp
#include <hip/hip_runtime.h>
#include <algorithm>
#include <type_traits>
#include "vj_device.hpp"
#include "vj_devutil.hpp"
#include "vj_grid_parts.hpp"

#ifndef VJ_STAMPS
#define VJ_STAMPS 0
#endif
#ifndef VJ_SCHED_PREFETCH
#define VJ_SCHED_PREFETCH 0
#endif
#define VJ_PIN_PREFETCH() do { } while (0)
namespace vj {

__device__ __forceinline__ NodeRecDev rec_fetch(kptr<NodeRecDev> p) {
    NodeRecDev r;
    const uint64_t v = (uint64_t)(uintptr_t)p;
    const uint64_t u = (uint64_t)(uint32_t)__builtin_amdgcn_readfirstlane((int)(uint32_t)v) |
                       (uint64_t)(uint32_t)__builtin_amdgcn_readfirstlane((int)(uint32_t)(v >> 32)) << 32;
    asm volatile("s_load_dwordx16 %0, %1, 0x0" : "=&s"(r) : "s"(u));
    return r;
}
__device__ __forceinline__ void rec_arrived(NodeRecDev& r) { asm volatile("s_waitcnt lgkmcnt(0)" : "+s"(r)); }
__device__ __forceinline__ void rec_arrived(NodeRecDev& a, NodeRecDev& b) { asm volatile("s_waitcnt lgkmcnt(0)" : "+s"(a), "+s"(b)); }

__device__ __forceinline__ float wave_sum_to_lane63(float v) {
    auto dpp = [](float x, auto ctrl, auto row_mask) {
        return __int_as_float(__builtin_amdgcn_update_dpp(0, __float_as_int(x), decltype(ctrl)::value, decltype(row_mask)::value, 0xf, true));
    };
    using std::integral_constant;
    v += dpp(v, integral_constant<int, 0xB1>{}, integral_constant<int, 0xf>{});
    v += dpp(v, integral_constant<int, 0x4E>{}, integral_constant<int, 0xf>{});
    v += dpp(v, integral_constant<int, 0x141>{}, integral_constant<int, 0xf>{});
    v += dpp(v, integral_constant<int, 0x140>{}, integral_constant<int, 0xf>{});
    v += dpp(v, integral_constant<int, 0x142>{}, integral_constant<int, 0xa>{});
    v += dpp(v, integral_constant<int, 0x143>{}, integral_constant<int, 0xc>{});
    return v;
}

__device__ __forceinline__ void lds_barrier() { asm volatile("s_waitcnt lgkmcnt(0)\n\ts_barrier" ::: "memory"); }



template <bool SQ>
__device__ __forceinline__ void band_colsum_body(const IntegralArgs& a) {
    const uint32_t x = (blockIdx.x * 256u + threadIdx.x) * 4u;
    const uint32_t band = blockIdx.y, frame = blockIdx.z;
    if (x >= a.band_pitch) return;
    const uint8_t* img = a.gray + (size_t)frame * a.gray_frame_bytes;
    uint32_t s[4] = {0, 0, 0, 0}, q[4] = {0, 0, 0, 0};
    const uint32_t y0 = band * BAND_ROWS;
#pragma unroll
    for (int r = 0; r < BAND_ROWS; ++r) {
        const uint32_t y = y0 + r;
        if (y < a.height && x < a.width) {
            const uint32_t v = load_gray4(img + (size_t)y * a.gray_stride, x, a.width, a.channels);
#pragma unroll
            for (int c = 0; c < 4; ++c) {
                const uint32_t p = (v >> (8 * c)) & 0xffu;
                s[c] += p;
                q[c] += p * p;
            }
        }
    }
    const size_t o = ((size_t)frame * a.n_bands + band) * a.band_pitch + x;
    *reinterpret_cast<uint4*>(a.band_sum + o) = make_uint4(s[0], s[1], s[2], s[3]);
    if (SQ) *reinterpret_cast<uint4*>(a.band_sq + o) = make_uint4(q[0], q[1], q[2], q[3]);
}
__global__ __launch_bounds__(256) void band_colsum(IntegralArgs a) { band_colsum_body<true>(a); }
__global__ __launch_bounds__(256) void band_colsum_sum(IntegralArgs a) { band_colsum_body<false>(a); }

__global__ __launch_bounds__(256) void band_scan(IntegralArgs a) {
    const uint32_t x = blockIdx.x * 256u + threadIdx.x;
    const uint32_t frame = blockIdx.y;
    if (x >= a.band_pitch) return;
    uint32_t s = 0;
    uint64_t q = 0;
    size_t o = (size_t)frame * a.n_bands * a.band_pitch + x;
    for (uint32_t b0 = 0; b0 < a.n_bands; b0 += 8u) {
        uint32_t ts[8], tq[8];
#pragma unroll
        for (uint32_t k = 0; k < 8u; ++k) {
            const bool in = b0 + k < a.n_bands;
            ts[k] = in ? a.band_sum[o + (size_t)k * a.band_pitch] : 0u;
            tq[k] = in ? a.band_sq[o + (size_t)k * a.band_pitch] : 0u;
        }
#pragma unroll
        for (uint32_t k = 0; k < 8u; ++k) {
            if (b0 + k < a.n_bands) {
                a.band_sum[o + (size_t)k * a.band_pitch] = s;
                a.band_sq_prefix[o + (size_t)k * a.band_pitch] = q;
            }
            s += ts[k];
            q += tq[k];
        }
        o += (size_t)8u * a.band_pitch;
    }
}
__global__ __launch_bounds__(256) void band_scan_sum(IntegralArgs a) {
    const uint32_t x = blockIdx.x * 256u + threadIdx.x;
    if (x >= a.band_pitch) return;
    uint32_t s = 0;
    size_t o = (size_t)blockIdx.y * a.n_bands * a.band_pitch + x;
    for (uint32_t b0 = 0; b0 < a.n_bands; b0 += 8u) {
        uint32_t ts[8];
#pragma unroll
        for (uint32_t k = 0; k < 8u; ++k) ts[k] = b0 + k < a.n_bands ? a.band_sum[o + (size_t)k * a.band_pitch] : 0u;
#pragma unroll
        for (uint32_t k = 0; k < 8u; ++k) {
            if (b0 + k < a.n_bands) a.band_sum[o + (size_t)k * a.band_pitch] = s;
            s += ts[k];
        }
        o += (size_t)8u * a.band_pitch;
    }
}

template <int BPG>
__global__ __launch_bounds__(1024) void band_scan2(IntegralArgs a) {
    __shared__ uint32_t tot_s[16][64];
    __shared__ uint64_t tot_q[16][64];
    const uint32_t lane = threadIdx.x & 63u, g = threadIdx.x >> 6;
    const uint32_t x = blockIdx.x * 64u + lane, frame = blockIdx.y;
    const bool in = x < a.band_pitch;
    const uint32_t b0 = g * (uint32_t)BPG;
    const size_t o = ((size_t)frame * a.n_bands + b0) * a.band_pitch + x;
    uint32_t ts[BPG], tq[BPG];
#pragma unroll
    for (int k = 0; k < BPG; ++k) {
        const bool have = in && b0 + (uint32_t)k < a.n_bands;
        ts[k] = have ? a.band_sum[o + (size_t)k * a.band_pitch] : 0u;
        tq[k] = have ? a.band_sq[o + (size_t)k * a.band_pitch] : 0u;
    }
    uint32_t s = 0;
    uint64_t q = 0;
#pragma unroll
    for (int k = 0; k < BPG; ++k) {
        s += ts[k];
        q += tq[k];
    }
    tot_s[g][lane] = s;
    tot_q[g][lane] = q;
    __syncthreads();
    s = 0;
    q = 0;
    for (uint32_t h = 0; h < g; ++h) {
        s += tot_s[h][lane];
        q += tot_q[h][lane];
    }
#pragma unroll
    for (int k = 0; k < BPG; ++k) {
        if (in && b0 + (uint32_t)k < a.n_bands) {
            a.band_sum[o + (size_t)k * a.band_pitch] = s;
            a.band_sq_prefix[o + (size_t)k * a.band_pitch] = q;
        }
        s += ts[k];
        q += tq[k];
    }
}

template <int CTRL, int ROW_MASK>
__device__ __forceinline__ uint32_t dpp_or_zero(uint32_t v) {
    return (uint32_t)__builtin_amdgcn_update_dpp(0, (int)v, CTRL, ROW_MASK, 0xf, true);
}
__device__ __forceinline__ uint32_t wave_incl_scan(uint32_t v) {
    v += dpp_or_zero<0x111, 0xf>(v);
    v += dpp_or_zero<0x112, 0xf>(v);
    v += dpp_or_zero<0x114, 0xf>(v);
    v += dpp_or_zero<0x118, 0xf>(v);
    v += dpp_or_zero<0x142, 0xa>(v);
    v += dpp_or_zero<0x143, 0xc>(v);
    return v;
}
template <int CTRL, int ROW_MASK>
__device__ __forceinline__ uint64_t dpp_or_zero(uint64_t v) {
    return (uint64_t)dpp_or_zero<CTRL, ROW_MASK>((uint32_t)v) | (uint64_t)dpp_or_zero<CTRL, ROW_MASK>((uint32_t)(v >> 32)) << 32;
}
__device__ __forceinline__ uint64_t wave_incl_scan(uint64_t v) {
    v += dpp_or_zero<0x111, 0xf>(v);
    v += dpp_or_zero<0x112, 0xf>(v);
    v += dpp_or_zero<0x114, 0xf>(v);
    v += dpp_or_zero<0x118, 0xf>(v);
    v += dpp_or_zero<0x142, 0xa>(v);
    v += dpp_or_zero<0x143, 0xc>(v);
    return v;
}
template <typename T>
__device__ __forceinline__ T wave_last(T v);
template <>
__device__ __forceinline__ uint32_t wave_last(uint32_t v) { return (uint32_t)__builtin_amdgcn_readlane((int)v, 63); }
template <>
__device__ __forceinline__ uint64_t wave_last(uint64_t v) {
    return (uint64_t)wave_last((uint32_t)v) | (uint64_t)wave_last((uint32_t)(v >> 32)) << 32;
}

typedef uint32_t u32x4_unaligned __attribute__((ext_vector_type(4), aligned(4)));
typedef uint64_t u64x2_unaligned __attribute__((ext_vector_type(2), aligned(8)));
template <bool NT, typename V>
__device__ __forceinline__ void out_store(V* p, V v) {
    if constexpr (NT) __builtin_nontemporal_store(v, p);
    else *p = v;
}

template <typename Q, bool NT = false, bool SQ = true>
__device__ __forceinline__ void band_rows_body(const IntegralArgs& a) {
    const uint32_t lane = lane_id();
    const uint32_t band = blockIdx.x * 4u + (threadIdx.x >> 6);
    const uint32_t frame = blockIdx.y;
    if (band >= a.n_bands) return;
    const uint8_t* img = a.gray + (size_t)frame * a.gray_frame_bytes;
    uint32_t* sum = a.sum + (size_t)frame * a.frame_elems;
    uint64_t* sqs = a.sqsum + (size_t)frame * a.frame_elems;
    const uint32_t ow = a.width + 1u;
    const uint32_t y0 = band * BAND_ROWS;
    const size_t bo = ((size_t)frame * a.n_bands + band) * a.band_pitch;

    if (band == 0) {
        for (uint32_t x = lane; x < ow; x += 64u) {
            sum[x] = 0u;
            if (SQ) sqs[x] = 0ull;
        }
    }
    uint32_t rs[BAND_ROWS];
    Q rq[BAND_ROWS];
#pragma unroll
    for (int r = 0; r < BAND_ROWS; ++r) {
        rs[r] = 0;
        rq[r] = 0;
    }
    uint32_t top_s = 0;
    uint64_t top_q = 0;
    for (uint32_t x0 = 0; x0 < a.width; x0 += 256u) {
        const uint32_t x = x0 + lane * 4u;
        const bool in = x < a.width;
        uint32_t v[BAND_ROWS];
#pragma unroll
        for (int r = 0; r < BAND_ROWS; ++r)
            v[r] = in && y0 + r < a.height ? load_gray4(img + (size_t)(y0 + r) * a.gray_stride, x, a.width, a.channels) : 0u;
        uint32_t as[4] = {0, 0, 0, 0};
        uint64_t aq[4] = {0, 0, 0, 0};
        if (in) {
            const uint4 t = *reinterpret_cast<const uint4*>(a.band_sum + bo + x);
            as[0] = t.x; as[1] = as[0] + t.y; as[2] = as[1] + t.z; as[3] = as[2] + t.w;
        }
        if (in && SQ) {
            const ulonglong2 u0 = *reinterpret_cast<const ulonglong2*>(a.band_sq_prefix + bo + x);
            const ulonglong2 u1 = *reinterpret_cast<const ulonglong2*>(a.band_sq_prefix + bo + x + 2);
            aq[0] = u0.x; aq[1] = aq[0] + u0.y; aq[2] = aq[1] + u1.x; aq[3] = aq[2] + u1.y;
        }
        {
            const uint32_t is = wave_incl_scan(as[3]);
            const uint64_t iq = wave_incl_scan(aq[3]);
            const uint32_t base_s = top_s + (is - as[3]);
            const uint64_t base_q = top_q + (iq - aq[3]);
#pragma unroll
            for (int c = 0; c < 4; ++c) {
                as[c] += base_s;
                aq[c] += base_q;
            }
            top_s += wave_last(is);
            top_q += wave_last(iq);
        }
#pragma unroll
        for (int r = 0; r < BAND_ROWS; ++r) {
            const uint32_t y = y0 + r;
            if (y < a.height) {
                uint32_t ls[4];
                Q lq[4];
#pragma unroll
                for (int c = 0; c < 4; ++c) {
                    const uint32_t p = (v[r] >> (8 * c)) & 0xffu;
                    ls[c] = p + (c ? ls[c - 1] : 0u);
                    lq[c] = (Q)(p * p) + (c ? lq[c - 1] : (Q)0);
                }
                const uint32_t is = wave_incl_scan(ls[3]);
                const Q iq = wave_incl_scan(lq[3]);
                const uint32_t base_s = rs[r] + (is - ls[3]);
                const Q base_q = rq[r] + (iq - lq[3]);
#pragma unroll
                for (int c = 0; c < 4; ++c) {
                    as[c] += base_s + ls[c];
                    aq[c] += (uint64_t)(Q)(base_q + lq[c]);
                }
                const size_t ro = (size_t)(y + 1u) * ow;
                if (x0 == 0 && lane == 0) {
                    sum[ro] = 0u;
                    if (SQ) sqs[ro] = 0ull;
                }
                if (x + 4u <= a.width) {
                    out_store<NT>(reinterpret_cast<u32x4_unaligned*>(sum + ro + x + 1u), u32x4_unaligned{as[0], as[1], as[2], as[3]});
                    if (SQ) {
                        out_store<NT>(reinterpret_cast<u64x2_unaligned*>(sqs + ro + x + 1u), u64x2_unaligned{aq[0], aq[1]});
                        out_store<NT>(reinterpret_cast<u64x2_unaligned*>(sqs + ro + x + 3u), u64x2_unaligned{aq[2], aq[3]});
                    }
                } else {
#pragma unroll
                    for (int c = 0; c < 4; ++c)
                        if (x + c < a.width) {
                            sum[ro + x + c + 1u] = as[c];
                            if (SQ) sqs[ro + x + c + 1u] = aq[c];
                        }
                }
                rs[r] += wave_last(is);
                rq[r] += wave_last(iq);
            }
        }
    }
}

template <typename Q>
__global__ __launch_bounds__(256) void band_rows(IntegralArgs a) { band_rows_body<Q>(a); }
template <typename Q>
__global__ __launch_bounds__(256) __attribute__((amdgpu_waves_per_eu(3, 3))) void band_rows_w3(IntegralArgs a) { band_rows_body<Q, true>(a); }
__global__ __launch_bounds__(256) void band_rows_sum(IntegralArgs a) { band_rows_body<uint32_t, false, false>(a); }

template <typename Q>
__global__ __launch_bounds__(512) void band_rows_par(IntegralArgs a) {
    __shared__ uint32_t tot_s[2][BAND_ROWS + 1][8];
    __shared__ uint64_t tot_q[2][BAND_ROWS + 1][8];
    const uint32_t lane = lane_id();
    const uint32_t w = __builtin_amdgcn_readfirstlane(threadIdx.x >> 6), nw = blockDim.x >> 6;
    const uint32_t band = blockIdx.x, frame = blockIdx.y;
    const uint8_t* img = a.gray + (size_t)frame * a.gray_frame_bytes;
    uint32_t* sum = a.sum + (size_t)frame * a.frame_elems;
    uint64_t* sqs = a.sqsum + (size_t)frame * a.frame_elems;
    const uint32_t ow = a.width + 1u;
    const uint32_t y0 = band * BAND_ROWS;
    const size_t bo = ((size_t)frame * a.n_bands + band) * a.band_pitch;
    if (band == 0) {
        for (uint32_t x = threadIdx.x; x < ow; x += blockDim.x) {
            sum[x] = 0u;
            sqs[x] = 0ull;
        }
    }
    uint32_t carry_s[BAND_ROWS + 1];
    uint64_t carry_q[BAND_ROWS + 1];
#pragma unroll
    for (int r = 0; r <= BAND_ROWS; ++r) {
        carry_s[r] = 0u;
        carry_q[r] = 0ull;
    }
    uint32_t buf = 0;
    for (uint32_t x0 = 0; x0 < a.width; x0 += 256u * nw, buf ^= 1u) {
        const uint32_t x = x0 + w * 256u + lane * 4u;
        const bool in = x < a.width;
        uint32_t v[BAND_ROWS];
#pragma unroll
        for (int r = 0; r < BAND_ROWS; ++r)
            v[r] = in && y0 + r < a.height ? load_gray4(img + (size_t)(y0 + r) * a.gray_stride, x, a.width, a.channels) : 0u;
        uint32_t as[4] = {0, 0, 0, 0};
        uint64_t aq[4] = {0, 0, 0, 0};
        if (in) {
            const uint4 t = *reinterpret_cast<const uint4*>(a.band_sum + bo + x);
            as[0] = t.x; as[1] = as[0] + t.y; as[2] = as[1] + t.z; as[3] = as[2] + t.w;
            const ulonglong2 u0 = *reinterpret_cast<const ulonglong2*>(a.band_sq_prefix + bo + x);
            const ulonglong2 u1 = *reinterpret_cast<const ulonglong2*>(a.band_sq_prefix + bo + x + 2);
            aq[0] = u0.x; aq[1] = aq[0] + u0.y; aq[2] = aq[1] + u1.x; aq[3] = aq[2] + u1.y;
        }
        uint32_t ex_s[BAND_ROWS + 1], t_s[BAND_ROWS + 1];
        uint64_t ex_top_q, t_q[BAND_ROWS + 1];
        Q ex_q[BAND_ROWS];
        {
            const uint32_t is = wave_incl_scan(as[3]);
            const uint64_t iq = wave_incl_scan(aq[3]);
            ex_s[0] = is - as[3];
            ex_top_q = iq - aq[3];
            t_s[0] = wave_last(is);
            t_q[0] = wave_last(iq);
        }
#pragma unroll
        for (int r = 0; r < BAND_ROWS; ++r) {
            uint32_t ls = 0;
            Q lq = 0;
#pragma unroll
            for (int c = 0; c < 4; ++c) {
                const uint32_t p = (v[r] >> (8 * c)) & 0xffu;
                ls += p;
                lq += (Q)(p * p);
            }
            const uint32_t is = wave_incl_scan(ls);
            const Q iq = wave_incl_scan(lq);
            ex_s[1 + r] = is - ls;
            ex_q[r] = iq - lq;
            t_s[1 + r] = wave_last(is);
            t_q[1 + r] = (uint64_t)wave_last(iq);
        }
        if (lane == 0) {
#pragma unroll
            for (int r = 0; r <= BAND_ROWS; ++r) {
                tot_s[buf][r][w] = t_s[r];
                tot_q[buf][r][w] = t_q[r];
            }
        }
        __syncthreads();
        uint32_t pre_s = 0, all_s = 0;
        uint64_t pre_q = 0, all_q = 0;
        if (lane <= (uint32_t)BAND_ROWS) {
            for (uint32_t k = 0; k < nw; ++k) {
                const uint32_t ts = tot_s[buf][lane][k];
                const uint64_t tq = tot_q[buf][lane][k];
                if (k < w) {
                    pre_s += ts;
                    pre_q += tq;
                }
                all_s += ts;
                all_q += tq;
            }
        }
        auto lane_u32 = [&](uint32_t val, int r) { return (uint32_t)__builtin_amdgcn_readlane((int)val, r); };
        auto lane_u64 = [&](uint64_t val, int r) { return (uint64_t)lane_u32((uint32_t)val, r) | (uint64_t)lane_u32((uint32_t)(val >> 32), r) << 32; };
        {
            const uint32_t base_s = carry_s[0] + lane_u32(pre_s, 0) + ex_s[0];
            const uint64_t base_q = carry_q[0] + lane_u64(pre_q, 0) + ex_top_q;
#pragma unroll
            for (int c = 0; c < 4; ++c) {
                as[c] += base_s;
                aq[c] += base_q;
            }
            carry_s[0] += lane_u32(all_s, 0);
            carry_q[0] += lane_u64(all_q, 0);
        }
#pragma unroll
        for (int r = 0; r < BAND_ROWS; ++r) {
            const uint32_t y = y0 + r;
            if (y < a.height) {
                const uint32_t base_s = carry_s[1 + r] + lane_u32(pre_s, 1 + r) + ex_s[1 + r];
                const Q base_q = (Q)(carry_q[1 + r] + lane_u64(pre_q, 1 + r)) + ex_q[r];
                uint32_t ls = 0;
                Q lq = 0;
#pragma unroll
                for (int c = 0; c < 4; ++c) {
                    const uint32_t p = (v[r] >> (8 * c)) & 0xffu;
                    ls += p;
                    lq += (Q)(p * p);
                    as[c] += base_s + ls;
                    aq[c] += (uint64_t)(Q)(base_q + lq);
                }
                const size_t ro = (size_t)(y + 1u) * ow;
                if (x == 0u) {
                    sum[ro] = 0u;
                    sqs[ro] = 0ull;
                }
                if (x + 4u <= a.width) {
                    out_store<false>(reinterpret_cast<u32x4_unaligned*>(sum + ro + x + 1u), u32x4_unaligned{as[0], as[1], as[2], as[3]});
                    out_store<false>(reinterpret_cast<u64x2_unaligned*>(sqs + ro + x + 1u), u64x2_unaligned{aq[0], aq[1]});
                    out_store<false>(reinterpret_cast<u64x2_unaligned*>(sqs + ro + x + 3u), u64x2_unaligned{aq[2], aq[3]});
                } else {
#pragma unroll
                    for (int c = 0; c < 4; ++c)
                        if (x + c < a.width) {
                            sum[ro + x + c + 1u] = as[c];
                            sqs[ro + x + c + 1u] = aq[c];
                        }
                }
                carry_s[1 + r] += lane_u32(all_s, 1 + r);
                carry_q[1 + r] += lane_u64(all_q, 1 + r);
            }
        }
    }
}

int launch_integral_sum(const IntegralArgs& a, void* stream_) {
    hipStream_t stream = (hipStream_t)stream_;
    hipLaunchKernelGGL(band_colsum_sum, dim3((a.band_pitch / 4u + 255u) / 256u, a.n_bands, a.n_frames), dim3(256), 0, stream, a);
    hipLaunchKernelGGL(band_scan_sum, dim3((a.band_pitch + 255u) / 256u, a.n_frames, 1), dim3(256), 0, stream, a);
    hipLaunchKernelGGL(band_rows_sum, dim3((a.n_bands + 3u) / 4u, a.n_frames, 1), dim3(256), 0, stream, a);
    return (int)hipGetLastError();
}

int launch_integral(const IntegralArgs& a, void* stream_) {
    hipStream_t stream = (hipStream_t)stream_;
    const uint32_t quads = a.band_pitch / 4u;
    dim3 g1((quads + 255u) / 256u, a.n_bands, a.n_frames);
    hipLaunchKernelGGL(band_colsum, g1, dim3(256), 0, stream, a);
    const dim3 g2b((a.band_pitch + 63u) / 64u, a.n_frames, 1);
    if (a.n_bands <= 16u * 8u) hipLaunchKernelGGL(band_scan2<8>, g2b, dim3(1024), 0, stream, a);
    else if (a.n_bands <= 16u * 16u) hipLaunchKernelGGL(band_scan2<16>, g2b, dim3(1024), 0, stream, a);
    else if (a.n_bands <= 16u * 32u) hipLaunchKernelGGL(band_scan2<32>, g2b, dim3(1024), 0, stream, a);
    else {
        dim3 g2((a.band_pitch + 255u) / 256u, a.n_frames, 1);
        hipLaunchKernelGGL(band_scan, g2, dim3(256), 0, stream, a);
    }
    if (a.rows_mode != 0u) {
        const bool batch_p = (uint64_t)a.n_frames * a.n_bands >= 2048u;
        if (a.rows_mode == 1u || !batch_p) {
            const uint32_t nw = min(8u, (a.width + 255u) / 256u);
            dim3 gp(a.n_bands, a.n_frames, 1);
            if ((uint64_t)a.width * 65025ull < (1ull << 32)) hipLaunchKernelGGL(band_rows_par<uint32_t>, gp, dim3(64u * nw), 0, stream, a);
            else hipLaunchKernelGGL(band_rows_par<uint64_t>, gp, dim3(64u * nw), 0, stream, a);
            return (int)hipGetLastError();
        }
    }
    dim3 g3((a.n_bands + 3u) / 4u, a.n_frames, 1);
    const bool batch = (uint64_t)a.n_frames * a.n_bands >= 2048u;
    if ((uint64_t)a.width * 65025ull < (1ull << 32)) {
        if (batch) hipLaunchKernelGGL(band_rows_w3<uint32_t>, g3, dim3(256), 0, stream, a);
        else hipLaunchKernelGGL(band_rows<uint32_t>, g3, dim3(256), 0, stream, a);
    } else {
        if (batch) hipLaunchKernelGGL(band_rows_w3<uint64_t>, g3, dim3(256), 0, stream, a);
        else hipLaunchKernelGGL(band_rows<uint64_t>, g3, dim3(256), 0, stream, a);
    }
    return (int)hipGetLastError();
}


__device__ __forceinline__ uint32_t window_pos(const CascadeArgs& a, uint32_t pos_base, uint32_t i, float step) {
    if (pos_base != 0u) return a.pos_tab[pos_base + i];
    const float v = (float)i * step;
    return (a.pos_mode & 1u) ? (uint32_t)roundf(v) : (uint32_t)__float2int_rn(v);
}

__device__ __forceinline__ bool window_visited(const CascadeArgs& a, uint32_t frame, uint32_t skip_base, uint32_t skip_wpr,
                                               uint32_t nx, uint32_t ix, uint32_t iy) {
    uint32_t word, bit;
    if (skip_wpr != 0u) {
        word = skip_base + iy * skip_wpr + (ix >> 6);
        bit = ix & 63u;
    } else {
        const uint32_t i = iy * nx + ix;
        word = skip_base + (i >> 6);
        bit = i & 63u;
    }
    return ((a.skip_bits[(size_t)frame * a.skip_frame_words + word] >> bit) & 1ull) != 0ull;
}

__device__ __forceinline__ float window_variance(rsrc_t sum_f, rsrc_t sq_f, uint32_t e, uint32_t e_lt, uint32_t e_dw,
                                                 uint32_t e_dh, float area, bool signed_mean) {
    const uint32_t c0 = e_lt, c1 = e_lt + e_dw, c2 = e_lt + e_dh, c3 = e_lt + e_dh + e_dw;
    const uint32_t s = ld_u32(sum_f, e * 4u, c0 * 4u) - ld_u32(sum_f, e * 4u, c1 * 4u) - ld_u32(sum_f, e * 4u, c2 * 4u) +
                       ld_u32(sum_f, e * 4u, c3 * 4u);
    const uint64_t q = ld_u64(sq_f, e * 8u, c0 * 8u) - ld_u64(sq_f, e * 8u, c1 * 8u) - ld_u64(sq_f, e * 8u, c2 * 8u) +
                       ld_u64(sq_f, e * 8u, c3 * 8u);
    const float mean = (signed_mean ? (float)(int32_t)s : (float)s) / area;
    float variance = (float)q;
    variance = (variance / area) - (mean * mean);
    return variance >= 0.0f ? sqrtf(variance) : 1.0f;
}

struct GlobalImgByStump {
    rsrc_t r;
    __device__ __forceinline__ uint32_t ld(uint32_t uni_window_off, uint32_t lane_corner_off) const {
        return ld_u32(r, lane_corner_off, __builtin_amdgcn_readfirstlane(uni_window_off));
    }
};
struct GlobalImg {
    rsrc_t r;
    __device__ __forceinline__ uint32_t ld(uint32_t lane_off, uint32_t uni_off) const { return ld_u32(r, lane_off, uni_off); }
    __device__ __forceinline__ GlobalImgByStump by_stump() const { return GlobalImgByStump{r}; }
};
struct LdsImg {
    const char* base;
    __device__ __forceinline__ uint32_t ld(uint32_t lane_off, uint32_t uni_off) const {
        return *reinterpret_cast<const uint32_t*>(base + (lane_off + uni_off));
    }
    __device__ __forceinline__ LdsImg by_stump() const { return *this; }
};

template <typename Img>
__device__ __forceinline__ float node_rect_sum(const Img& img, const NodeRecDev& r, uint32_t off) {
    const uint32_t lt0 = r[0], lt1 = r[1], lt2 = r[2];
    const uint32_t dh0 = r[3], dh1 = r[4], dh2 = r[5];
    const uint32_t dw0 = (uint32_t)(int32_t)(int16_t)(r[6] & 0xffffu), dw1 = (uint32_t)((int32_t)r[6] >> 16),
                   dw2 = (uint32_t)(int32_t)(int16_t)(r[7] & 0xffffu);
    const float w0 = __uint_as_float(r[8]), w1 = __uint_as_float(r[9]), w2 = __uint_as_float(r[10]);
    const uint32_t r0 = img.ld(off, lt0) - img.ld(off, lt0 + dw0) - img.ld(off, lt0 + dh0) + img.ld(off, lt0 + dh0 + dw0);
    const uint32_t r1 = img.ld(off, lt1) - img.ld(off, lt1 + dw1) - img.ld(off, lt1 + dh1) + img.ld(off, lt1 + dh1 + dw1);
    float rect_sum = (float)r0 * w0;
    rect_sum += (float)r1 * w1;
    if (w2 != 0.0f) {
        const uint32_t r2 =
            img.ld(off, lt2) - img.ld(off, lt2 + dw2) - img.ld(off, lt2 + dh2) + img.ld(off, lt2 + dh2 + dw2);
        rect_sum += (float)r2 * w2;
    }
    return rect_sum;
}

template <typename Img>
__device__ __forceinline__ void node_rect_sum_pair(const Img& img, const NodeRecDev& ra, const NodeRecDev& rb, uint32_t off,
                                                   float& sum_a, float& sum_b);
template <int NC, bool COUNT = false, typename Img>
__device__ __forceinline__ void stage_sum_tree2_multi(const Img& img, kptr<NodeRecDev> tab, uint32_t n_trees,
                                                      const uint32_t (&off)[NC], const float (&var)[NC],
                                                      float (&stage_sum)[NC], uint32_t (*cnt)[2] = nullptr);

__device__ __forceinline__ void tree_count_flush(const CascadeArgs& a, uint32_t nodes, uint32_t rects, uint32_t lane) {
#pragma unroll
    for (int d = 32; d >= 1; d >>= 1) {
// ... 479 lines not shown
__global__ __launch_bounds__(GATHER_WAVES_MAX * 64) void cascade_pass(CascadeArgs a) {
    __shared__ QEntry lds_q[(GENERAL ? WAVES_PER_BLOCK : GATHER_WAVES_MAX) * UNIT_WINDOWS];
    __shared__ int32_t lds_tgt[GENERAL ? WAVES_PER_BLOCK * UNIT_WINDOWS : 1];
    const uint32_t lane = lane_id();
    const uint32_t wib = __builtin_amdgcn_readfirstlane(threadIdx.x >> 6);
    const uint32_t wpb = blockDim.x >> 6;
    QEntry* q = lds_q + wib * UNIT_WINDOWS;
    kptr<ScaleDev> scales = as_k(a.scales);
    const rsrc_t img = make_rsrc(a.sum, a.sum_bytes);

    if (FROM_GRID) {
        const unsigned long long t_enter = VJ_STAMPS ? __builtin_amdgcn_s_memrealtime() : 0ull;
        kptr<UnitDev> units = as_k(a.units);
        const uint32_t total_units = a.n_units * a.n_frames;
        const uint32_t frame_bytes4 = a.frame_elems * 4u;
        uint32_t part = grid_part_home(blockIdx.x);
        uint32_t p_lo = grid_part_begin(total_units, part), p_n = grid_part_size(total_units, part);
        auto issue = [&]() -> uint32_t {
            uint32_t t = 0;
            if (lane == 0) t = atomicAdd(a.q_ticket + part, 1u);
            return t;
        };
        auto resolve = [&](uint32_t t_v) -> uint32_t {
            uint32_t t = __builtin_amdgcn_readfirstlane(t_v);
            while (t >= p_n) {
                bool has = false;
                if (lane < GRID_PARTS)
                    has = __hip_atomic_load(a.q_ticket + lane, __ATOMIC_RELAXED, __HIP_MEMORY_SCOPE_AGENT) < grid_part_size(total_units, lane);
                const uint32_t open = (uint32_t)__ballot(has) & ((1u << GRID_PARTS) - 1u);
                if (open == 0u) return total_units;
                const uint32_t turn = ((open >> part) | (open << (GRID_PARTS - part))) & ((1u << GRID_PARTS) - 1u);
                part = (part + (uint32_t)__builtin_ctz(turn)) & (GRID_PARTS - 1u);
                p_lo = grid_part_begin(total_units, part);
                p_n = grid_part_size(total_units, part);
                t = __builtin_amdgcn_readfirstlane(issue());
            }
            return p_lo + t;
        };
        uint32_t u = resolve(p_n != 0u ? issue() : 0u);
        while (u < total_units) {
            const uint32_t t_next = issue();
            const uint32_t frame = u / a.n_units;
            const uint32_t r = u - frame * a.n_units;
            const uint32_t slot = units[r].scale;
            const uint32_t first = units[r].first;
            const uint32_t count = units[r].count;
            const float step = scales[slot].step;
            const uint32_t pos_base = scales[slot].pos_base;
            const uint32_t nx = scales[slot].nx;
            const uint32_t e_lt = scales[slot].e_lt, e_dw = scales[slot].e_dw, e_dh = scales[slot].e_dh;
            const float area = scales[slot].area;
            const size_t frame_off = (size_t)frame * a.frame_elems;
            const rsrc_t sum_f = make_rsrc(a.sum + frame_off, frame_bytes4);
            const rsrc_t sq_f = make_rsrc(a.sqsum + frame_off, frame_bytes4 * 2u);
            const uint32_t frame_bytes = frame * frame_bytes4;
            const uint32_t bw = units[r].bw, ny = scales[slot].ny;
            uint32_t n_q = 0;
            for (uint32_t i0 = 0; i0 < count; i0 += 64u) {
                const uint32_t i = i0 + lane;
                uint32_t ix, iy;
                if (bw != 0u) {
                    const uint32_t ty = i / bw;
                    ix = (first & 0xffffu) + (i - ty * bw);
                    iy = (first >> 16) + ty;
                } else {
                    iy = (first + i) / nx;
                    ix = first + i - iy * nx;
                }
                bool valid = i < count && ix < nx && iy < ny;
                if (a.skip_bits != nullptr && valid)
                    valid = window_visited(a, frame, scales[slot].skip_base, scales[slot].skip_wpr, nx, ix, iy);
                QEntry en{0u, 0.0f};
                if (valid) {
                    const uint32_t x = window_pos(a, pos_base, ix, step);
                    const uint32_t y = window_pos(a, pos_base, iy, step);
                    const uint32_t e = y * a.stride + x;
                    en.var = window_variance(sum_f, sq_f, e, e_lt, e_dw, e_dh, area, a.signed_mean != 0u);
                    en.off = frame_bytes + e * 4u;
                }
                const unsigned long long mask = __ballot(valid);
                if (valid) q[n_q + mbcnt(mask)] = en;
                n_q += (uint32_t)__popcll(mask);
            }
            __builtin_amdgcn_wave_barrier();
            if (GENERAL)
                run_stages_general<TREES, COUNT>(a, img, q, lds_tgt + wib * UNIT_WINDOWS, n_q, slot,
                                                 scales[slot].table_first, lane);
            else
                run_stages_linear<TREES, LAST, COUNT>(a, img, q, n_q, slot, scales[slot].table_first,
                                                      scales[slot].q_base, lane, a.stage_begin, frame_part(a, frame),
                                                      a.run_table != nullptr ? u : 0xffffffffu);
            __builtin_amdgcn_wave_barrier();
            u = resolve(t_next);
        }
        if (VJ_STAMPS) {
            static_assert(sizeof(QEntry) == sizeof(unsigned long long), "a stamp fits a queue entry");
            unsigned long long* lds_end = reinterpret_cast<unsigned long long*>(lds_q);
            if (lane == 0) lds_end[wib * UNIT_WINDOWS] = __builtin_amdgcn_s_memrealtime();
            __syncthreads();
            if (threadIdx.x == 0) {
                unsigned long long last = 0, sum = 0;
                for (uint32_t w = 0; w < wpb; ++w) {
                    last = max(last, lds_end[w * UNIT_WINDOWS]);
                    sum += lds_end[w * UNIT_WINDOWS];
                }
                const unsigned long long tail = last - sum / wpb;
                atomicAdd(a.stage_entered + 40, tail);
                atomicMax(a.stage_entered + 41, tail);
                atomicAdd(a.stage_entered + 42, last);
                atomicMax(a.stage_entered + 43, last);
                atomicMax(a.stage_entered + 44, ~t_enter);
                atomicAdd(a.stage_entered + 45, 1ull);
            }
        }
    } else if (!GENERAL && a.q_groups != nullptr) {
        kptr<UnitDev> groups = as_k(a.q_groups);
        kptr<uint32_t> runs = as_k(a.run_table);
        const uint32_t nG = a.n_q_groups;
        uint32_t part = blockIdx.x & (Q_PARTS - 1u);
        for (uint32_t tries = 0; tries < Q_PARTS;) {
            const uint32_t f_lo = a.n_frames >= Q_PARTS ? (uint32_t)(((unsigned long long)part * a.n_frames + Q_PARTS - 1u) / Q_PARTS) : min(part, a.n_frames);
            const uint32_t f_hi = a.n_frames >= Q_PARTS ? (uint32_t)(((unsigned long long)(part + 1u) * a.n_frames + Q_PARTS - 1u) / Q_PARTS)
                                                        : min(part + 1u, a.n_frames);
            const uint32_t n_items = (f_hi - f_lo) * nG;
            uint32_t t = n_items;
            if (n_items != 0u) {
                if (lane == 0) t = atomicAdd(a.q_ticket + part, 1u);
                t = __builtin_amdgcn_readfirstlane(t);
            }
            if (t >= n_items) {
// ... 94 lines not shown
            const uint32_t q_base = scales[slot].q_base;
            const size_t base = (size_t)q_base + (size_t)part * scales[slot].q_cap;
            const uint32_t c0 = c * chunk;
            const uint32_t n = min(cnt - c0, chunk);
            for (uint32_t i = lane; i < n; i += 64u) q[i] = a.q_in[base + c0 + i];
            __builtin_amdgcn_wave_barrier();
            const unsigned long long t_chunk = VJ_STAMPS ? __builtin_amdgcn_s_memtime() : 0ull;
            if (GENERAL)
                run_stages_general<TREES, COUNT>(a, img, q, lds_tgt + wib * UNIT_WINDOWS, n, slot, scales[slot].table_first, lane);
            else
                run_stages_linear<TREES, LAST, COUNT, NW>(a, img, q, n, slot, scales[slot].table_first, q_base, lane, a.stage_begin, part);
            __builtin_amdgcn_wave_barrier();
            if (VJ_STAMPS && lane == 0) {
                const unsigned long long dt = __builtin_amdgcn_s_memtime() - t_chunk;
                atomicAdd(a.stage_entered + 48, dt);
                atomicMax(a.stage_entered + 49, dt);
                atomicAdd(a.stage_entered + 50, 1ull);
            }
        }
    }
}


template <bool TREES>
__global__ __launch_bounds__(256) void skip_fail_bits(CascadeArgs a) {
    const uint32_t lane = lane_id();
    const uint32_t rank = blockIdx.x * 4u + (threadIdx.x >> 6);
    kptr<ScaleDev> scales = as_k(a.scales);
    kptr<StageDev> stages = as_k(a.stages);
    kptr<UnitDev> units = as_k(a.skip_units);
    const uint32_t total = a.n_skip_units * a.n_frames;
    const uint32_t frame_bytes4 = a.frame_elems * 4u;
    const rsrc_t img = make_rsrc(a.sum, a.sum_bytes);
    for (uint32_t u = rank; u < total; u += gridDim.x * 4u) {
        const uint32_t frame = u / a.n_skip_units;
        const uint32_t r = u - frame * a.n_skip_units;
        const uint32_t slot = units[r].scale, first = units[r].first, count = units[r].count, word = units[r].bw;
        const uint32_t nx = scales[slot].nx;
        const float step = scales[slot].step;
        const uint32_t pos_base = scales[slot].pos_base;
        uint32_t ix, iy;
        if (scales[slot].skip_wpr != 0u) {
            ix = (first & 0xffffu) + lane;
            iy = first >> 16;
        } else {
            const uint32_t i = first + lane;
            iy = i / nx;
            ix = i - iy * nx;
        }
        bool fail = false;
        if (lane < count) {
            const size_t frame_off = (size_t)frame * a.frame_elems;
            const rsrc_t sum_f = make_rsrc(a.sum + frame_off, frame_bytes4);
            const rsrc_t sq_f = make_rsrc(a.sqsum + frame_off, frame_bytes4 * 2u);
            const uint32_t x = window_pos(a, pos_base, ix, step), y = window_pos(a, pos_base, iy, step);
            const uint32_t e = y * a.stride + x;
            const float var = window_variance(sum_f, sq_f, e, scales[slot].e_lt, scales[slot].e_dw, scales[slot].e_dh, scales[slot].area,
                                              a.signed_mean != 0u);
            kptr<NodeRecDev> tab = as_k(reinterpret_cast<const NodeRecDev*>(a.table)) + scales[slot].table_first + stages[0].first_node;
            fail = !(stage_sum_of<TREES>(GlobalImg{img}, tab, stages[0].n_nodes, frame * frame_bytes4 + e * 4u, var) >= stages[0].threshold);
        }
        const unsigned long long F = __ballot(fail);
        if (lane == 0) a.skip_bits[(size_t)frame * a.skip_frame_words + word] = F;
    }
}

__global__ __launch_bounds__(256) void skip_resolve(CascadeArgs a) {
    const uint32_t lane = lane_id();
    const uint32_t rank = blockIdx.x * 4u + (threadIdx.x >> 6);
    kptr<UnitDev> segs = as_k(a.skip_segs);
    const uint32_t total = a.n_skip_segs * a.n_frames;
    const unsigned long long below = (1ull << lane) - 1ull;
    for (uint32_t u = rank; u < total; u += gridDim.x * 4u) {
        const uint32_t frame = u / a.n_skip_segs;
        const uint32_t r = u - frame * a.n_skip_segs;
        unsigned long long* words = a.skip_bits + (size_t)frame * a.skip_frame_words + segs[r].first;
        const uint32_t n_words = segs[r].count;
        uint32_t carry = 0;
        for (uint32_t w0 = 0; w0 < n_words; w0 += 64u) {
            const bool act = w0 + lane < n_words;
            const unsigned long long F = act ? words[w0 + lane] : 0ull;
            const bool through = F == ~0ull;
            const uint32_t tpar = (uint32_t)__clzll((long long)~F) & 1u;
            const unsigned long long m = __ballot(act && !through);
            const unsigned long long lower = m & below;
            const uint32_t src = lower != 0ull ? 63u - (uint32_t)__clzll((long long)lower) : 0u;
            const uint32_t from_lane = (uint32_t)__shfl((int)tpar, (int)src, 64);
            uint32_t p = lower != 0ull ? from_lane : carry;
            unsigned long long V = 0ull;
#pragma unroll 8
            for (uint32_t b = 0; b < 64u; ++b) {
                V |= (unsigned long long)(p ^ 1u) << b;
                p = ((F >> b) & 1ull) != 0ull ? p ^ 1u : 0u;
            }
            if (act) words[w0 + lane] = V;
            if (m != 0ull) carry = (uint32_t)__shfl((int)tpar, 63 - __clzll((long long)m), 64);
        }
    }
}

int launch_skip_resolve(const CascadeArgs& a, int n_blocks, void* stream_) {
    hipLaunchKernelGGL(skip_resolve, dim3(n_blocks), dim3(256), 0, (hipStream_t)stream_, a);
    return (int)hipGetLastError();
}

int launch_skip_bitmap(const CascadeArgs& a, bool trees, int n_blocks, void* stream_) {
    hipStream_t stream = (hipStream_t)stream_;
    if (trees) hipLaunchKernelGGL(skip_fail_bits<true>, dim3(n_blocks), dim3(256), 0, stream, a);
    else       hipLaunchKernelGGL(skip_fail_bits<false>, dim3(n_blocks), dim3(256), 0, stream, a);
    hipLaunchKernelGGL(skip_resolve, dim3(n_blocks), dim3(256), 0, stream, a);
    return (int)hipGetLastError();
// ... 41 lines not shown
            const uint32_t tw = ((uint32_t)nx + tx - 1u) / tx, th = ((uint32_t)ny + ty - 1u) / ty;
            const uint32_t base = atomicAdd(r.n_tiles, tx * ty);
            for (uint32_t j = 0; j < tx * ty && base + j < r.max_tiles; ++j)
                r.tiles[base + j] = RoiTile{roi, slot, (j % tx) * tw | ((j / tx) * th) << 16, (uint32_t)nx | (uint32_t)ny << 16, tw | th << 16};
            continue;
        }
        const uint32_t nun = (nwin + UNIT_WINDOWS - 1u) / UNIT_WINDOWS;
        const uint32_t base = atomicAdd(r.n_units, nun);
        for (uint32_t j = 0; j < nun && base + j < r.max_units; ++j)
            r.units[base + j] = RoiUnit{roi, slot, j * UNIT_WINDOWS, min((uint32_t)UNIT_WINDOWS, nwin - j * UNIT_WINDOWS), (uint32_t)nx, (uint32_t)ny};
    }
}

template <bool TREES, bool COUNT, bool GENERAL>
__global__ __launch_bounds__(GATHER_WAVES_MAX * 64) void cascade_roi_pass(RoiArgs r, CascadeArgs a) {
    __shared__ QEntry lds_q[(GENERAL ? WAVES_PER_BLOCK : GATHER_WAVES_MAX) * UNIT_WINDOWS];
    __shared__ int32_t lds_tgt[GENERAL ? WAVES_PER_BLOCK * UNIT_WINDOWS : 1];
    const uint32_t lane = lane_id();
    const uint32_t wib = __builtin_amdgcn_readfirstlane(threadIdx.x >> 6);
    QEntry* q = lds_q + wib * UNIT_WINDOWS;
    kptr<ScaleDev> scales = as_k(a.scales);
    const rsrc_t img = make_rsrc(a.sum, a.sum_bytes);
    const uint32_t n_units = min(*r.n_units, r.max_units);
    const uint32_t frame_bytes4 = a.frame_elems * 4u;
    while (true) {
        uint32_t t = 0;
        if (lane == 0) t = atomicAdd(r.ticket, 1u);
        t = __builtin_amdgcn_readfirstlane(t);
        if (t >= n_units) break;
        const RoiUnit un = r.units[t];
        const uint32_t roi = __builtin_amdgcn_readfirstlane(un.roi), slot = __builtin_amdgcn_readfirstlane(un.slot);
        const uint32_t first = __builtin_amdgcn_readfirstlane(un.first), count = __builtin_amdgcn_readfirstlane(un.count);
        const uint32_t nx = __builtin_amdgcn_readfirstlane(un.nx);
        const RoiDev R = r.rois[roi];
        const uint32_t frame = __builtin_amdgcn_readfirstlane((uint32_t)R.frame);
        const uint32_t x0 = __builtin_amdgcn_readfirstlane((uint32_t)R.x), y0 = __builtin_amdgcn_readfirstlane((uint32_t)R.y);
        const float step = scales[slot].step;
        const uint32_t e_lt = scales[slot].e_lt, e_dw = scales[slot].e_dw, e_dh = scales[slot].e_dh;
        const float area = scales[slot].area;
        const size_t frame_off = (size_t)frame * a.frame_elems;
        const rsrc_t sum_f = make_rsrc(a.sum + frame_off, frame_bytes4);
        const rsrc_t sq_f = make_rsrc(a.sqsum + frame_off, frame_bytes4 * 2u);
        const uint32_t frame_bytes = frame * frame_bytes4;
        uint32_t n_q = 0;
        for (uint32_t i0 = 0; i0 < count; i0 += 64u) {
            const bool valid = i0 + lane < count;
            const uint32_t i = first + i0 + lane;
            const uint32_t iy = i / nx, ix = i - iy * nx;
            QEntry en{0u, 0.0f};
            if (valid) {
                const uint32_t x = x0 + (uint32_t)__float2int_rn((float)ix * step);
                const uint32_t y = y0 + (uint32_t)__float2int_rn((float)iy * step);
                const uint32_t e = y * a.stride + x;
                en.var = window_variance(sum_f, sq_f, e, e_lt, e_dw, e_dh, area, a.signed_mean != 0u);
                en.off = frame_bytes + e * 4u;
            }
            const unsigned long long mask = __ballot(valid);
            if (valid) q[n_q + mbcnt(mask)] = en;
            n_q += (uint32_t)__popcll(mask);
        }
        __builtin_amdgcn_wave_barrier();
        if (GENERAL) {
            run_stages_general_to<TREES, COUNT>(a, img, q, lds_tgt + wib * UNIT_WINDOWS, n_q, scales[slot].table_first, lane,
                                                [&](unsigned long long acc_mask, bool mine, uint32_t off) {
                uint32_t g = 0;
                if (lane == 0) g = atomicAdd(r.det_count, (uint32_t)__popcll(acc_mask));
                g = __builtin_amdgcn_readfirstlane(g);
                const uint32_t pos = g + mbcnt(acc_mask);
                if (mine && pos < r.det_cap) r.det[pos] = RoiDet{off, slot, roi};
            });
            __builtin_amdgcn_wave_barrier();
            continue;
        }
        kptr<NodeRecDev> table = as_k(reinterpret_cast<const NodeRecDev*>(a.table)) + scales[slot].table_first;
        const uint32_t n = sweep_stages<TREES, COUNT>(a, GlobalImg{img}, table, q, n_q, lane, a.stage_begin, a.stage_end);
        if (n != 0u) {
            uint32_t g = 0;
            if (lane == 0) g = atomicAdd(r.det_count, n);
            g = __builtin_amdgcn_readfirstlane(g);
            for (uint32_t i = lane; i < n; i += 64u)
                if (g + i < r.det_cap) r.det[g + i] = RoiDet{q[i].off, slot, roi};
        }
        __builtin_amdgcn_wave_barrier();
    }
}

template <bool COUNT>
__global__ void cascade_tile_roi_pass(RoiArgs r, CascadeArgs a);

template <bool GENERAL>
static void launch_roi_pass(const RoiArgs& r, const CascadeArgs& a, bool trees, bool count, dim3 g, dim3 b, hipStream_t stream) {
    if (trees) {
        if (count) hipLaunchKernelGGL((cascade_roi_pass<true, true, GENERAL>), g, b, 0, stream, r, a);
        else       hipLaunchKernelGGL((cascade_roi_pass<true, false, GENERAL>), g, b, 0, stream, r, a);
    } else {
        if (count) hipLaunchKernelGGL((cascade_roi_pass<false, true, GENERAL>), g, b, 0, stream, r, a);
        else       hipLaunchKernelGGL((cascade_roi_pass<false, false, GENERAL>), g, b, 0, stream, r, a);
    }
}

static uint32_t gather_block_threads(const CascadeArgs& a, bool general) {
    const uint32_t most = general ? (uint32_t)WAVES_PER_BLOCK : (uint32_t)GATHER_WAVES_MAX;
    return 64u * std::min(std::max(a.gather_waves, 1u), most);
}

int launch_roi_chain(const RoiArgs& r, const CascadeArgs& a, bool from_dets, bool trees, bool count, bool general, int n_blocks,
                     void* stream_, void* stream2_, void* fork_ev_, void* join_ev_) {
// ... 428 lines not shown
                cur_part = x;
                return cand;
            }
        }
        return total_units;
    };
    uint32_t u = part_begin(my_xcd) + (blockIdx.x >> 3);
    if (u >= part_begin(my_xcd + 1u)) {
        if (threadIdx.x == 0) lds_cnt[TILE_WAVES + 8] = draw();
        __syncthreads();
        u = __builtin_amdgcn_readfirstlane(lds_cnt[TILE_WAVES + 8]);
    }
    while (u < total_units) {
        uint32_t next_u = 0;
        if (threadIdx.x == 0) next_u = draw();
        uint32_t frame, slot0, ix0, iy0, roi_nx = 0, roi_ny = 0, ox = 0, oy = 0, roi = 0, n_mem = 1;
        if constexpr (ROI) {
            kptr<RoiTile> rt = as_k(r_->tiles);
            roi = rt[u].roi;
            slot0 = rt[u].slot;
            ix0 = rt[u].first & 0xffffu;
            iy0 = rt[u].first >> 16;
            roi_nx = rt[u].nxy & 0xffffu;
            roi_ny = rt[u].nxy >> 16;
            const RoiDev R = r_->rois[roi];
            frame = __builtin_amdgcn_readfirstlane((uint32_t)R.frame);
            ox = __builtin_amdgcn_readfirstlane((uint32_t)R.x);
            oy = __builtin_amdgcn_readfirstlane((uint32_t)R.y);
        } else {
            frame = u / a.n_tile_units;
            const uint32_t r = u - frame * a.n_tile_units;
            slot0 = units[r].scale;
            ix0 = units[r].first & 0xffffu;
            iy0 = units[r].first >> 16;
            n_mem = max(units[r].count, 1u);
        }
        const uint32_t lead = slot0 + n_mem - 1u;
        const float step = scales[slot0].step;
        uint32_t tw = scales[lead].tile_tw, th = scales[lead].tile_th;
        const uint32_t pitch = scales[lead].tile_pitch;
        uint32_t rows = scales[lead].tile_rows, cols = pitch;
        if constexpr (ROI) {
            const uint32_t tw_s = tw, th_s = th;
            tw = as_k(r_->tiles)[u].twh & 0xffffu;
            th = as_k(r_->tiles)[u].twh >> 16;
            const uint32_t full_y = (uint32_t)((float)(th_s - 1u) * step), need_y = (uint32_t)((float)(th - 1u) * step) + 2u;
            const uint32_t full_x = (uint32_t)((float)(tw_s - 1u) * step), need_x = (uint32_t)((float)(tw - 1u) * step) + 2u;
            if (need_y < full_y) rows -= full_y - need_y;
            if (need_x < full_x) cols -= full_x - need_x;
        }
        const uint32_t frame_bytes = frame * frame_bytes4;
        const size_t frame_off = (size_t)frame * a.frame_elems;
        const rsrc_t sum_f = make_rsrc(a.sum + frame_off, frame_bytes4);
        const rsrc_t sq_f = make_rsrc(a.sqsum + frame_off, frame_bytes4 * 2u);
        const uint32_t x0 = ox + __builtin_amdgcn_readfirstlane(window_pos(a, scales[slot0].pos_base, ix0, step));
        const uint32_t y0 = oy + __builtin_amdgcn_readfirstlane(window_pos(a, scales[slot0].pos_base, iy0, step));

        __syncthreads();
        STAMP(0);
        const uint32_t half = scales[lead].tile_half;
        for (uint32_t rr = wib; rr < rows; rr += TILE_WAVES) {
            const uint32_t g_row = ((y0 + rr) * a.stride + x0) * 4u;
            if (half == 0u) {
                for (uint32_t c0 = 0; c0 < cols; c0 += 256u) {
                    const uint32_t soff = __builtin_amdgcn_readfirstlane(g_row + c0 * 4u);
                    if (c0 + lane * 4u < cols)
                        __builtin_amdgcn_raw_ptr_buffer_load_lds(
                            sum_f, (__attribute__((address_space(3))) uint32_t*)(lds_img + rr * pitch + c0), 16,
                            lane * 16u, soff, 0, 0);
                }
            } else {
                for (uint32_t plane = 0; plane < 2u; ++plane) {
                    const uint32_t n_cols = min(plane == 0u ? half : pitch - half, (cols + 1u) / 2u + 1u);
                    for (uint32_t c0 = 0; c0 < n_cols; c0 += 64u) {
                        const uint32_t soff = __builtin_amdgcn_readfirstlane(g_row + (c0 * 2u + plane) * 4u);
                        if (c0 + lane < n_cols)
                            __builtin_amdgcn_raw_ptr_buffer_load_lds(
                                sum_f,
                                (__attribute__((address_space(3))) uint32_t*)(lds_img + rr * pitch + plane * half + c0), 4,
                                lane * 8u, soff, 0, 0);
                    }
                }
            }
        }
        bool skip_front = false;
        for (uint32_t m = 0; m < n_mem; ++m) {
            const uint32_t slot = slot0 + m;
            asm volatile("" : "+s"(tw), "+s"(th), "+s"(ix0), "+s"(iy0));
            const uint32_t nx = ROI ? roi_nx : scales[slot].nx, ny = ROI ? roi_ny : scales[slot].ny;
            if (n_mem > 1u && (ix0 >= nx || iy0 >= scales[slot].tile_row_end)) continue;
            const uint32_t pos_base = scales[slot].pos_base;
            q = lds_q + wib * TILE_WAVE_CAP;
            const uint32_t n_tile = tw * th;
            const uint32_t n_chunks = (n_tile + 63u) >> 6;
            const uint32_t c_base = n_chunks / TILE_WAVES, c_extra = n_chunks % TILE_WAVES;
            const uint32_t t_begin = min((wib * c_base + min(wib, c_extra)) * 64u, n_tile);
            const uint32_t t_end = min(t_begin + (c_base + (wib < c_extra ? 1u : 0u)) * 64u, n_tile);
            const uint32_t te_lt = (ROI ? scales[slot].te_lt : scales[slot].grp_te_lt) * 4u;
            const uint32_t te_dh = (ROI ? scales[slot].te_dh : scales[slot].grp_te_dh) * 4u, e_dw = scales[slot].e_dw;
            const uint32_t te_dw = (uint32_t)(ROI ? scales[slot].te_dw : scales[slot].grp_te_dw) * 4u;
            const uint32_t e_lt = scales[slot].e_lt, e_dh = scales[slot].e_dh;
            const float area = scales[slot].area;
            constexpr int NCH = TILE_WAVE_CAP / 64;
            const bool sq32 = scales[slot].sq32 != 0u;
            uint32_t w_lo4[NCH];
            float w_q[NCH];
            bool w_valid[NCH];
#pragma unroll
            for (int k = 0; k < NCH; ++k) {
                const uint32_t t = t_begin + (uint32_t)k * 64u + lane;
                const uint32_t ty = t / tw, tx = t - ty * tw;
                const uint32_t iy = iy0 + ty, ix = ix0 + tx;
                w_valid[k] = t < t_end && iy < ny && ix < nx;
                if (!ROI && a.skip_bits != nullptr && w_valid[k])
                    w_valid[k] = window_visited(a, frame, scales[slot].skip_base, scales[slot].skip_wpr, nx, ix, iy);
                w_lo4[k] = 0u;
                w_q[k] = 0.0f;
                if (w_valid[k]) {
                    const uint32_t x = ox + window_pos(a, pos_base, ix, step);
                    const uint32_t y = oy + window_pos(a, pos_base, iy, step);
                    const uint32_t e = y * a.stride + x;
                    w_lo4[k] = ((y - y0) * pitch + (half ? (x - x0) >> 1 : x - x0)) * 4u;
                    const uint32_t c0 = e_lt, c1 = e_lt + e_dw, c2 = e_lt + e_dh, c3 = e_lt + e_dh + e_dw;
                    if (sq32)
                        w_q[k] = (float)(uint32_t)(ld_u32(sq_f, e * 8u, c0 * 8u) - ld_u32(sq_f, e * 8u, c1 * 8u) -
                                                   ld_u32(sq_f, e * 8u, c2 * 8u) + ld_u32(sq_f, e * 8u, c3 * 8u));
                    else
                        w_q[k] = (float)(uint64_t)(ld_u64(sq_f, e * 8u, c0 * 8u) - ld_u64(sq_f, e * 8u, c1 * 8u) -
                                                   ld_u64(sq_f, e * 8u, c2 * 8u) + ld_u64(sq_f, e * 8u, c3 * 8u));
                }
            }
            if (!skip_front) __syncthreads();
            STAMP(1);

            uint32_t n = 0;
            const LdsImg img{reinterpret_cast<const char*>(lds_img)};
#pragma unroll
            for (int k = 0; k < NCH; ++k) {
                QEntry en{0u, 0.0f};
                if (w_valid[k]) {
                    const uint32_t lo4 = w_lo4[k];
                    const uint32_t s4 = img.ld(lo4, te_lt) - img.ld(lo4, te_lt + te_dw) - img.ld(lo4, te_lt + te_dh) +
                                        img.ld(lo4, te_lt + te_dh + te_dw);
                    const float mean = (a.signed_mean ? (float)(int32_t)s4 : (float)s4) / area;
                    float variance = w_q[k];
                    variance = (variance / area) - (mean * mean);
                    en.var = variance >= 0.0f ? sqrtf(variance) : 1.0f;
                    en.off = lo4;
                }
                const unsigned long long mask = __ballot(w_valid[k]);
                if (w_valid[k]) q[n + mbcnt(mask)] = en;
                n += (uint32_t)__popcll(mask);
            }
            __builtin_amdgcn_wave_barrier();
            const uint32_t table_first = ROI ? scales[slot].tile_table_first : scales[slot].grp_table_first;
            kptr<NodeRecDev> table = as_k(reinterpret_cast<const NodeRecDev*>(a.table)) + table_first;
            STAMP(2);
            auto flush_wave = [&](const QEntry* qq, uint32_t nn, uint32_t dest_) {
                if constexpr (ROI) {
                    uint32_t g = 0;
                    if (lane == 0) g = atomicAdd(r_->det_count, nn);
                    g = __builtin_amdgcn_readfirstlane(g);
                    for (uint32_t i = lane; i < nn; i += 64u) {
                        const uint32_t lo = qq[i].off >> 2;
                        const uint32_t ly = lo / pitch, lc = lo - ly * pitch;
                        const uint32_t lx = half ? lc * 2u : lc;
                        if (g + i < r_->det_cap) r_->det[g + i] = RoiDet{frame_bytes + ((y0 + ly) * a.stride + (x0 + lx)) * 4u, slot, roi};
                    }
                    return;
                }
                const bool is_det = dest_ == a.n_pass;
                const uint32_t part = frame_part(a, frame);
                uint32_t g = 0;
                if (lane == 0)
                    g = is_det ? atomicAdd(a.det_count, nn) : atomicAdd(a.q_pass_count[dest_] + slot * Q_PARTS + part, nn);
                g = __builtin_amdgcn_readfirstlane(g);
                const size_t q_base = (size_t)scales[slot].q_base + (size_t)part * scales[slot].q_cap;
// ... 206 lines not shown
```

### include/vj.h

```cpp
#ifndef VJ_H_
#define VJ_H_

#include <stdint.h>
#include <stddef.h>

#ifdef __cplusplus
extern "C" {
#endif
#if defined(VJ_BUILDING) && defined(__GNUC__)
#pragma GCC visibility push(default)
#endif

enum {
    VJ_OK = 0,
    VJ_ERR_ARG = 1,
    VJ_ERR_IO = 2,
    VJ_ERR_PARSE = 3,
    VJ_ERR_UNSUPPORTED = 4,
    VJ_ERR_NO_DEVICE = 5,
    VJ_ERR_HIP = 6,
    VJ_ERR_NOMEM = 7,
    VJ_ERR_LIMIT = 8
};
const char* vj_strerror(int code);
// ... 85 lines not shown
int vj_plan_feature_table(const vj_cascade* c, int width, const vj_scale_info* s,
                          uint32_t* offsets, float* weights);

typedef struct vj_tile_info {
    int32_t  scale_idx;
    float    scale, step;
    int32_t  nx, ny;
    int32_t  lds_class;
    int32_t  tile_w, tile_h;
    int32_t  pitch, rows;
    int32_t  reach_x, reach_y;
    int32_t  lead_scale_idx;
    int32_t  tile_row_end;
} vj_tile_info;
typedef struct vj_tile_plan_info {
    uint32_t header_bytes;
    uint32_t gather_reserve_bytes;
    uint32_t max_tile_windows;
    uint32_t n_classes;
    uint32_t class_lds[4];
    int32_t  class_per_cu[4];
    uint32_t class_tiles[4];
} vj_tile_plan_info;
#define VJ_PLAN_TILES_FORMER_SHAPES 1u
#define VJ_PLAN_TILES_NO_GROUPS     2u
int vj_plan_tiles(const vj_cascade* c, int width, int height, const vj_params* p, int n_frames,
                  uint32_t flags, vj_tile_plan_info* info, vj_tile_info* out, int cap, int* n);
typedef struct vj_tile_cut_info {
    float    tile_split;
    uint32_t gather_units;
    uint64_t gather_windows;
    uint64_t plan_windows;
} vj_tile_cut_info;
int vj_plan_tiles_split(const vj_cascade* c, int width, int height, const vj_params* p, int n_frames,
                        uint32_t flags, float tile_split, vj_tile_plan_info* info, vj_tile_cut_info* cut,
                        vj_tile_info* out, uint64_t* gather_windows, int cap, int* n);

typedef struct vj_env vj_env;
int  vj_env_create(int device_index, vj_env** out);
void vj_env_destroy(vj_env* e);
int  vj_env_reserve(vj_env* e, int max_w, int max_h, int max_batch);
int  vj_env_device_name(const vj_env* e, char* buf, size_t cap);
int  vj_env_configure(vj_env* e, const char* key, const char* value);
int  vj_env_query(const vj_env* e, const char* key, char* buf, size_t cap);

int vj_integral(vj_env* e, const uint8_t* gray, int w, int h, int stride,
                uint32_t* sum, uint64_t* sqsum);

int  vj_host_alloc(vj_env* e, size_t bytes, void** out);
void vj_host_free(vj_env* e, void* p);

struct vj_image;
int  vj_integral_image(vj_env* e, const struct vj_image* image, uint32_t* sum, uint64_t* sqsum);
int  vj_grayscale(vj_env* e, const struct vj_image* image, uint8_t* gray, int gray_stride);
int  vj_integral_tilted(vj_env* e, const struct vj_image* image, uint32_t* tilted);
int  vj_canny(vj_env* e, const struct vj_image* image, uint8_t* edges, int edges_stride);
int  vj_resize_linear(vj_env* e, const struct vj_image* image, int dst_w, int dst_h, uint8_t* dst, int dst_stride);
int  vj_equalize_hist(vj_env* e, const struct vj_image* image, uint8_t* dst, int dst_stride);
typedef struct vj_image {
    const uint8_t* data;
    int32_t width, height;
    int32_t stride;
    int32_t on_device;
    int32_t channels;
} vj_image;

typedef struct vj_rect {
    int32_t x, y, w, h;
    float   weight;
    int32_t frame;
    int32_t scale_idx;
} vj_rect;

#define VJ_MAX_STAGES 64
typedef struct vj_counters {
    uint64_t windows;
    uint64_t stump_evals;
    uint64_t gather_bytes;
    uint64_t stage_entered[VJ_MAX_STAGES];
} vj_counters;

#define VJ_MAX_PASSES 8
#define VJ_MAX_LAUNCHES 16
enum { VJ_LAUNCH_GRID = 0,
       VJ_LAUNCH_QUEUE = 1,
       VJ_LAUNCH_TILE = 2,
       VJ_LAUNCH_BLOCK = 3 };
typedef struct vj_launch {
    int32_t  kind;
    int32_t  lds_class;
    int32_t  stage_begin, stage_end;
    float    ms;
    uint32_t lds_bytes;
    uint64_t scale_mask[2];
    uint64_t stage_entered[VJ_MAX_STAGES];
} vj_launch;
typedef struct vj_timing {
    float integral_ms;
    float cascade_ms;
    float total_ms;
    int32_t n_cascade_launches;
    float pass_ms[VJ_MAX_PASSES];
    int32_t pass_stage_begin[VJ_MAX_PASSES];
    int32_t pass_stage_end[VJ_MAX_PASSES];
    int32_t n_launches;
    vj_launch launch[VJ_MAX_LAUNCHES];
// ... 148 lines not shown
```

Baseline: 11.49 billion windows/s.

## Store squared integral image as wrapping u32 with strip-split variance sums

Stores the squared-pixel integral as modular 32-bit values instead of 64-bit in the stream and batch paths. This halves the memory written by the integral kernels and read by variance normalisation. Large windows whose squared sum could overflow 32 bits are split into horizontal strips. Each strip's difference is exact modulo 2^32 and is summed in 64 bits. The change adds extra loads for large scales and templated scan and store paths. It also adds a host API to fetch batch integrals with the 32-bit squared table.

```diff
diff --git a/clfacedetection_amd/api.py b/clfacedetection_amd/api.py
--- a/clfacedetection_amd/api.py
+++ b/clfacedetection_amd/api.py
@@ -199,6 +199,7 @@
     "vj_env_query": (C.c_int, [C.c_void_p, C.c_char_p, C.c_char_p, C.c_size_t]),
     "vj_integral": (C.c_int, [C.c_void_p, C.c_void_p, C.c_int, C.c_int, C.c_int, C.c_void_p, C.c_void_p]),
     "vj_integral_image": (C.c_int, [C.c_void_p, C.c_void_p, C.c_void_p, C.c_void_p]),
+    "vj_integral_batch_sq32": (C.c_int, [C.c_void_p, C.c_void_p, C.c_int, C.c_void_p, C.c_void_p]),
     "vj_integral_tilted": (C.c_int, [C.c_void_p, C.c_void_p, C.c_void_p]),
     "vj_grayscale": (C.c_int, [C.c_void_p, C.c_void_p, C.c_void_p, C.c_int]),
     "vj_canny": (C.c_int, [C.c_void_p, C.c_void_p, C.c_void_p, C.c_int]),
@@ -477,6 +478,15 @@
                "vj_integral")
         return s, q
 
+    def integral_sq32(self, frames, color: bool = False) -> tuple[np.ndarray, np.ndarray]:
+        imgs, n, keep = self._images(frames, color)
+        if n == 0:
+            raise ValueError("integral_sq32 expects at least one frame")
+        s = np.empty((n, imgs[0].height + 1, imgs[0].width + 1), np.uint32)
+        q = np.empty_like(s)
+        _check(load_library().vj_integral_batch_sq32(self._h, imgs, n, s.ctypes.data, q.ctypes.data), "vj_integral_batch_sq32")
+        return s, q
+
     def _one_image(self, img: np.ndarray):
         if img.dtype != np.uint8 or img.ndim not in (2, 3):
             raise ValueError("expected a 2-D uint8 image or a (h, w, 3|4) uint8 BGR/BGRA image")
diff --git a/clfacedetection_amd/build.py b/clfacedetection_amd/build.py
--- a/clfacedetection_amd/build.py
+++ b/clfacedetection_amd/build.py
@@ -10,7 +10,7 @@
 LIB_PATH = os.path.join(PKG_DIR, "libvjhip.so")
 SOURCES = ["vj_cascade.cpp", "vj_plan.cpp", "vj_group.cpp", "vj_env.cpp", "vj_cv.cpp", "vj_cv_roi_host.cpp", "vj_cv_roi_levels_host.cpp", "vj_cv_points_host.cpp", "vj_points_host.cpp", "vj_points_driver.cpp", "vj_atlas_host.cpp", "vj_mixed.cpp", "vj_kernels.hip",
            "vj_cv_profile.hip", "vj_cv_tile.hip", "vj_group_dev.hip", "vj_canny.hip", "vj_pyramid.hip", "vj_cv_biggest.hip", "vj_cv_roi.hip", "vj_cv_chain.hip", "vj_cv_points.hip", "vj_points.hip", "vj_atlas.hip", "vj_equalize.hip"]
-HEADERS = ["vj_internal.hpp", "vj_device.hpp", "vj_env_internal.hpp", "vj_devutil.hpp", "vj_cv_window.hpp", "vj_group_frame.hpp", "vj_cv_roi_units.hpp", "vj_cv_roi_host.hpp", "vj_cv_roi_levels_host.hpp", "vj_cv_points_units.hpp", "vj_cv_points_host.hpp", "vj_points_units.hpp", "vj_points_host.hpp", "vj_points_driver.hpp", "vj_clod_window.hpp", "vj_grid_parts.hpp", "vj_atlas_units.hpp", "vj_atlas_host.hpp", os.path.join("..", "..", "include", "vj.h")]
+HEADERS = ["vj_internal.hpp", "vj_device.hpp", "vj_env_internal.hpp", "vj_devutil.hpp", "vj_cv_window.hpp", "vj_group_frame.hpp", "vj_cv_roi_units.hpp", "vj_cv_roi_host.hpp", "vj_cv_roi_levels_host.hpp", "vj_cv_points_units.hpp", "vj_cv_points_host.hpp", "vj_points_units.hpp", "vj_points_host.hpp", "vj_points_driver.hpp", "vj_clod_window.hpp", "vj_grid_parts.hpp", "vj_sq_strips.hpp", "vj_atlas_units.hpp", "vj_atlas_host.hpp", os.path.join("..", "..", "include", "vj.h")]
 FLAGS = ["-O3", "-std=c++17", "-fPIC", "-ffp-contract=off", "-fno-fast-math", "--offload-arch=gfx950",
          "-Wall", "-Wno-unused-function", "-fvisibility=hidden", "-DVJ_BUILDING"] + \
     (["-DVJ_STAMPS=1"] if os.environ.get("VJ_STAMPS") else []) + \
diff --git a/clfacedetection_amd/csrc/vj_device.hpp b/clfacedetection_amd/csrc/vj_device.hpp
--- a/clfacedetection_amd/csrc/vj_device.hpp
+++ b/clfacedetection_amd/csrc/vj_device.hpp
@@ -1,6 +1,7 @@
 #pragma once
 #include <stdint.h>
 #include "vj_cv_roi_units.hpp"
+#include "vj_sq_strips.hpp"
 
 namespace vj {
 
@@ -42,8 +43,9 @@
     uint32_t tile_tail_first;
     uint32_t grp_tail_first;
     uint32_t sq32;
-};
-static_assert(sizeof(ScaleDev) == 152, "ScaleDev is 152 bytes");
+    uint32_t sq_strip;
+};
+static_assert(sizeof(ScaleDev) == 156, "ScaleDev is 156 bytes");
 
 struct StageDev {
     uint32_t first_node;
@@ -122,8 +124,6 @@
 constexpr int TILE_SP_MAX_BLOCKS = 4;
 constexpr int TILE_SP_BLOCK = 64;
 constexpr int TILE_TAIL_BLOCK_RECS = (3 * 16 + 8) * TILE_SP_BLOCK / 64;
-constexpr uint32_t SQ32_MAX_AREA = 66051;
-static_assert(65025ull * SQ32_MAX_AREA < (1ull << 32) && 65025ull * (SQ32_MAX_AREA + 1ull) >= (1ull << 32), "SQ32_MAX_AREA");
 
 struct CascadeArgs {
     const uint32_t* sum;
@@ -192,6 +192,7 @@
     uint32_t  n_skip_units;
     const UnitDev* skip_segs;
     uint32_t  n_skip_segs;
+    uint32_t  sq_u32;
 };
 
 struct IntegralArgs {
@@ -210,6 +211,7 @@
     uint64_t* sqsum;
     uint32_t frame_elems;
     uint32_t rows_mode;
+    uint32_t sq_u32;
 };
 constexpr int BAND_ROWS = 8;
 
diff --git a/clfacedetection_amd/csrc/vj_env.cpp b/clfacedetection_amd/csrc/vj_env.cpp
--- a/clfacedetection_amd/csrc/vj_env.cpp
+++ b/clfacedetection_amd/csrc/vj_env.cpp
@@ -165,6 +165,7 @@
         sd.win_w = (uint32_t)si.win_w;
         sd.win_h = (uint32_t)si.win_h;
         sd.sq32 = e->sq32 && (uint64_t)sd.win_w * sd.win_h <= SQ32_MAX_AREA ? 1u : 0u;
+        sd.sq_strip = sd.sq32 ? 0u : sq_strip_rows(sd.e_dw) * stride;
         table.resize(table.size() + n_nodes);
         int rc = build_node_table(c, W, si, table.data() + sd.table_first);
         if (rc) return rc;
@@ -880,7 +881,7 @@
 }
 
 int enqueue_integral(vj_env* e, const uint8_t* d_gray, size_t frame_bytes, int stride, int W, int H, int frames,
-                     int channels) {
+                     int channels, bool sq_u32) {
     IntegralArgs ia;
     memset(&ia, 0, sizeof(ia));
     ia.channels = (uint32_t)channels;
@@ -899,14 +900,16 @@
     ia.sqsum = (uint64_t*)e->d_sqsum.p;
     ia.frame_elems = frame_elems_for(W, H);
     ia.rows_mode = (uint32_t)e->integral_rows_mode;
+    ia.sq_u32 = sq_u32 ? 1u : 0u;
     const size_t used = (size_t)(W + 1) * (size_t)(H + 1);
     const bool zeroed = e->slack_w == W && e->slack_h == H && e->slack_frames >= frames && e->slack_sum == e->d_sum.p &&
-                        e->slack_sq == e->d_sqsum.p;
+                        e->slack_sq == e->d_sqsum.p && e->slack_sq_u32 == sq_u32;
+    const size_t sq_elem = sq_u32 ? 4 : 8;
     for (int f = 0; f < frames && !zeroed; ++f) {
         HIP_TRY(hipMemsetAsync((uint32_t*)e->d_sum.p + (size_t)f * ia.frame_elems + used, 0,
                                (ia.frame_elems - used) * 4, e->stream));
-        HIP_TRY(hipMemsetAsync((uint64_t*)e->d_sqsum.p + (size_t)f * ia.frame_elems + used, 0,
-                               (ia.frame_elems - used) * 8, e->stream));
+        HIP_TRY(hipMemsetAsync((char*)e->d_sqsum.p + ((size_t)f * ia.frame_elems + used) * sq_elem, 0,
+                               (ia.frame_elems - used) * sq_elem, e->stream));
     }
     if (!zeroed) {
         e->slack_w = W;
@@ -914,6 +917,7 @@
         e->slack_frames = frames;
         e->slack_sum = e->d_sum.p;
         e->slack_sq = e->d_sqsum.p;
+        e->slack_sq_u32 = sq_u32;
     }
     int hrc = launch_integral(ia, e->stream);
     if (hrc) {
@@ -1139,7 +1143,7 @@
 static_assert(CountsLayout::roi_tickets_begin + 8u <= CountsLayout::tile_tickets_begin, "the region pass's tile tickets end before the tile classes'");
 
 static int enqueue_prepare(vj_env* e, Lane* L, Plan* pl, const vj_image* frames, int nf, int W, int H, bool fixed_queue_layout,
-                           hipStream_t copy_stream, bool equalize = false) {
+                           hipStream_t copy_stream, bool equalize = false, bool sq_u32 = false) {
     int rc;
     int channels = image_channels(frames[0]);
     if ((rc = ensure_image_buffers(e, W, H, nf, true, channels, L))) return rc;
@@ -1169,7 +1173,8 @@
     L->src_frame_bytes = gray_frame_bytes;
     L->src_stride = gray_stride;
     L->src_channels = channels;
-    if ((rc = enqueue_integral(e, d_gray, gray_frame_bytes, gray_stride, W, H, nf, channels))) return rc;
+    L->sq_u32 = sq_u32 && e->sq32 && e->sq_u32 && (uint32_t)W <= SQ32_MAX_AREA;
+    if ((rc = enqueue_integral(e, d_gray, gray_frame_bytes, gray_stride, W, H, nf, channels, L->sq_u32))) return rc;
     HIP_TRY(hipEventRecord(L->ev[1], e->stream));
     HIP_TRY(hipEventRecord(L->integral_done, e->stream));
     L->nf = nf;
@@ -1197,6 +1202,7 @@
         memset(&ca, 0, sizeof(ca));
         ca.sum = (const uint32_t*)e->d_sum.p;
         ca.sqsum = (const uint64_t*)e->d_sqsum.p;
+        ca.sq_u32 = L->sq_u32 ? 1u : 0u;
         ca.table = (const uint32_t*)pl->d_table.p;
         ca.scales = (const ScaleDev*)pl->d_scales.p;
         ca.stages = (const StageDev*)pl->d_stages.p;
@@ -1448,7 +1454,7 @@
             L->det_cap = want;
             if (L->shared_integrals) {
                 HIP_TRY(hipEventRecord(L->ev[0], e->stream));
-                if ((rc = enqueue_integral(e, L->src_gray, L->src_frame_bytes, L->src_stride, W, H, L->nf, L->src_channels))) return rc;
+                if ((rc = enqueue_integral(e, L->src_gray, L->src_frame_bytes, L->src_stride, W, H, L->nf, L->src_channels, L->sq_u32))) return rc;
                 HIP_TRY(hipEventRecord(L->ev[1], e->stream));
             }
             if ((rc = enqueue_cascade(e, L, pl, W, H, p))) return rc;
@@ -1539,7 +1545,7 @@
                            const vj_params& p, bool equalize, std::vector<RawDet>* dets, vj_counters* ctr, vj_timing* tm) {
     int rc;
     Lane* L = &e->lane0;
-    if ((rc = enqueue_prepare(e, L, pl, frames + f0, nf, W, H, false, nullptr, equalize))) return rc;
+    if ((rc = enqueue_prepare(e, L, pl, frames + f0, nf, W, H, false, nullptr, equalize, true))) return rc;
     if ((rc = enqueue_cascade(e, L, pl, W, H, p))) return rc;
     return finish_batch(e, L, pl, f0, W, H, p, dets, ctr, tm);
 }
@@ -1887,6 +1893,7 @@
     e->n_cu = prop.multiProcessorCount;
     if (const char* g = getenv("VJ_TILE_GROUP")) e->tile_group = std::max(1, std::min(atoi(g), (int)MAX_SCALES));
     if (const char* g = getenv("VJ_SQ32")) e->sq32 = atoi(g) != 0;
+    if (const char* g = getenv("VJ_SQ_U32")) e->sq_u32 = atoi(g) != 0;
     if (const int hrc = prepare_tile_kernels()) {
         set_error("raising the dynamic LDS limit on device %d failed: %s", device_index, hipGetErrorString((hipError_t)hrc));
         return VJ_ERR_HIP;
@@ -2272,6 +2279,29 @@
     return VJ_OK;
 }
 
+int vj_integral_batch_sq32(vj_env* e, const vj_image* frames, int n_frames, uint32_t* sum, uint32_t* sqsum32) {
+    if (!e || !frames || n_frames <= 0 || !sum || !sqsum32) return VJ_ERR_ARG;
+    int W, H, CH, rc;
+    if ((rc = check_frames(frames, n_frames, &W, &H, &CH))) return rc;
+    const size_t fe = frame_elems_for(W, H);
+    if (fe * 8u * (size_t)n_frames > 0xfffffff0ull) {
+        set_error("vj_integral_batch_sq32: %d frames of %d x %d exceed one batch", n_frames, W, H);
+        return VJ_ERR_LIMIT;
+    }
+    HIP_TRY(hipSetDevice(e->device));
+    if ((rc = ensure_image_buffers(e, W, H, n_frames, true, CH))) return rc;
+    const uint8_t* d_gray;
+    size_t fb;
+    int gs;
+    if ((rc = stage_frames(e, frames, n_frames, W, H, &d_gray, &fb, &gs))) return rc;
+    if ((rc = enqueue_integral(e, d_gray, fb, gs, W, H, n_frames, CH, true))) return rc;
+    const size_t row = (size_t)(W + 1) * (size_t)(H + 1) * 4;
+    HIP_TRY(hipMemcpy2DAsync(sum, row, e->d_sum.p, fe * 4, row, (size_t)n_frames, hipMemcpyDeviceToHost, e->stream));
+    HIP_TRY(hipMemcpy2DAsync(sqsum32, row, e->d_sqsum.p, fe * 4, row, (size_t)n_frames, hipMemcpyDeviceToHost, e->stream));
+    HIP_TRY(hipStreamSynchronize(e->stream));
+    return VJ_OK;
+}
+
 }
 
 namespace vj {
@@ -2897,7 +2927,7 @@
     const int lane = s->n_pending == 0 ? 0 : 1 - s->fifo[0];
     Lane* L = &s->lanes[lane];
     HIP_TRY(hipEventSynchronize(L->integral_done));
-    if ((rc = enqueue_prepare(e, L, s->plan.get(), frames, n_frames, W, H, true, s->copy))) return rc;
+    if ((rc = enqueue_prepare(e, L, s->plan.get(), frames, n_frames, W, H, true, s->copy, false, true))) return rc;
     if ((rc = enqueue_cascade(e, L, s->plan.get(), W, H, s->p))) return rc;
     s->fifo[s->n_pending] = lane;
     s->n_frames_of[lane] = n_frames;
diff --git a/clfacedetection_amd/csrc/vj_env_internal.hpp b/clfacedetection_amd/csrc/vj_env_internal.hpp
--- a/clfacedetection_amd/csrc/vj_env_internal.hpp
+++ b/clfacedetection_amd/csrc/vj_env_internal.hpp
@@ -180,6 +180,7 @@
     const uint8_t* src_gray = nullptr;
     size_t src_frame_bytes = 0;
     int src_stride = 0, src_channels = 1;
+    bool sq_u32 = false;
     bool shared_integrals = false;
     size_t n_pass = 0;
     int launches = 0;
@@ -274,6 +275,7 @@
     int device = 0;
     int tile_group = 4;
     bool sq32 = true;
+    bool sq_u32 = true;
     hipStream_t stream = nullptr;
     vj::Lane lane0;
     hipEvent_t fork_ev = nullptr, join_ev = nullptr;
@@ -286,6 +288,7 @@
     vj::DevBuf d_out;
     int slack_w = 0, slack_h = 0, slack_frames = 0;
     void *slack_sum = nullptr, *slack_sq = nullptr;
+    bool slack_sq_u32 = false;
     vj::DevBuf d_q[vj::MAX_PASSES];
     vj::DevBuf d_q2[vj::MAX_PASSES];
     vj::DevBuf d_skip_bits;
@@ -351,7 +354,7 @@
 uint32_t frame_elems_for(int W, int H);
 int ensure_image_buffers(vj_env* e, int W, int H, int frames, bool need_gray, int channels = 1, Lane* lane = nullptr);
 int enqueue_integral(vj_env* e, const uint8_t* d_gray, size_t frame_bytes, int stride, int W, int H, int frames,
-                     int channels = 1);
+                     int channels = 1, bool sq_u32 = false);
 int stage_frames(vj_env* e, const vj_image* frames, int n, int W, int H, const uint8_t** d_ptr, size_t* frame_bytes,
                  int* stride, Lane* lane = nullptr, hipStream_t copy_stream = nullptr);
 int enqueue_tilted(vj_env* e, const uint8_t* d_gray, size_t frame_bytes, int stride, int W, int H, int frames, int channels);
diff --git a/clfacedetection_amd/csrc/vj_kernels.hip b/clfacedetection_amd/csrc/vj_kernels.hip
--- a/clfacedetection_amd/csrc/vj_kernels.hip
+++ b/clfacedetection_amd/csrc/vj_kernels.hip
@@ -71,12 +71,14 @@
 __global__ __launch_bounds__(256) void band_colsum(IntegralArgs a) { band_colsum_body<true>(a); }
 __global__ __launch_bounds__(256) void band_colsum_sum(IntegralArgs a) { band_colsum_body<false>(a); }
 
+template <typename P>
 __global__ __launch_bounds__(256) void band_scan(IntegralArgs a) {
     const uint32_t x = blockIdx.x * 256u + threadIdx.x;
     const uint32_t frame = blockIdx.y;
     if (x >= a.band_pitch) return;
+    P* const sq_prefix = reinterpret_cast<P*>(a.band_sq_prefix);
     uint32_t s = 0;
-    uint64_t q = 0;
+    P q = 0;
     size_t o = (size_t)frame * a.n_bands * a.band_pitch + x;
     for (uint32_t b0 = 0; b0 < a.n_bands; b0 += 8u) {
         uint32_t ts[8], tq[8];
@@ -90,7 +92,7 @@
         for (uint32_t k = 0; k < 8u; ++k) {
             if (b0 + k < a.n_bands) {
                 a.band_sum[o + (size_t)k * a.band_pitch] = s;
-                a.band_sq_prefix[o + (size_t)k * a.band_pitch] = q;
+                sq_prefix[o + (size_t)k * a.band_pitch] = q;
             }
             s += ts[k];
             q += tq[k];
@@ -116,10 +118,11 @@
     }
 }
 
-template <int BPG>
+template <int BPG, typename P>
 __global__ __launch_bounds__(1024) void band_scan2(IntegralArgs a) {
     __shared__ uint32_t tot_s[16][64];
-    __shared__ uint64_t tot_q[16][64];
+    __shared__ P tot_q[16][64];
+    P* const sq_prefix = reinterpret_cast<P*>(a.band_sq_prefix);
     const uint32_t lane = threadIdx.x & 63u, g = threadIdx.x >> 6;
     const uint32_t x = blockIdx.x * 64u + lane, frame = blockIdx.y;
     const bool in = x < a.band_pitch;
@@ -133,7 +136,7 @@
         tq[k] = have ? a.band_sq[o + (size_t)k * a.band_pitch] : 0u;
     }
     uint32_t s = 0;
-    uint64_t q = 0;
+    P q = 0;
 #pragma unroll
     for (int k = 0; k < BPG; ++k) {
         s += ts[k];
@@ -152,7 +155,7 @@
     for (int k = 0; k < BPG; ++k) {
         if (in && b0 + (uint32_t)k < a.n_bands) {
             a.band_sum[o + (size_t)k * a.band_pitch] = s;
-            a.band_sq_prefix[o + (size_t)k * a.band_pitch] = q;
+            sq_prefix[o + (size_t)k * a.band_pitch] = q;
         }
         s += ts[k];
         q += tq[k];
@@ -202,15 +205,36 @@
     else *p = v;
 }
 
-template <typename Q, bool NT = false, bool SQ = true>
+template <typename S>
+__device__ __forceinline__ void load_sq_prefix4(const IntegralArgs& a, size_t i, S (&aq)[4]) {
+    if constexpr (sizeof(S) == 8) {
+        const ulonglong2 u0 = *reinterpret_cast<const ulonglong2*>(a.band_sq_prefix + i);
+        const ulonglong2 u1 = *reinterpret_cast<const ulonglong2*>(a.band_sq_prefix + i + 2);
+        aq[0] = u0.x; aq[1] = aq[0] + u0.y; aq[2] = aq[1] + u1.x; aq[3] = aq[2] + u1.y;
+    } else {
+        const uint4 t = *reinterpret_cast<const uint4*>(reinterpret_cast<const uint32_t*>(a.band_sq_prefix) + i);
+        aq[0] = t.x; aq[1] = aq[0] + t.y; aq[2] = aq[1] + t.z; aq[3] = aq[2] + t.w;
+    }
+}
+template <bool NT, typename S>
+__device__ __forceinline__ void store_sq4(S* p, const S (&aq)[4]) {
+    if constexpr (sizeof(S) == 8) {
+        out_store<NT>(reinterpret_cast<u64x2_unaligned*>(p), u64x2_unaligned{aq[0], aq[1]});
+        out_store<NT>(reinterpret_cast<u64x2_unaligned*>(p + 2), u64x2_unaligned{aq[2], aq[3]});
+    } else {
+        out_store<NT>(reinterpret_cast<u32x4_unaligned*>(p), u32x4_unaligned{aq[0], aq[1], aq[2], aq[3]});
+    }
+}
+template <typename Q, bool NT = false, bool SQ = true, typename S = uint64_t>
 __device__ __forceinline__ void band_rows_body(const IntegralArgs& a) {
+    static_assert(sizeof(S) == 8 || sizeof(Q) == 4, "a 32-bit squared integral scans its rows in 32 bits");
     const uint32_t lane = lane_id();
     const uint32_t band = blockIdx.x * 4u + (threadIdx.x >> 6);
     const uint32_t frame = blockIdx.y;
     if (band >= a.n_bands) return;
     const uint8_t* img = a.gray + (size_t)frame * a.gray_frame_bytes;
     uint32_t* sum = a.sum + (size_t)frame * a.frame_elems;
-    uint64_t* sqs = a.sqsum + (size_t)frame * a.frame_elems;
+    S* sqs = reinterpret_cast<S*>(a.sqsum) + (size_t)frame * a.frame_elems;
     const uint32_t ow = a.width + 1u;
     const uint32_t y0 = band * BAND_ROWS;
     const size_t bo = ((size_t)frame * a.n_bands + band) * a.band_pitch;
@@ -218,7 +242,7 @@
     if (band == 0) {
         for (uint32_t x = lane; x < ow; x += 64u) {
             sum[x] = 0u;
-            if (SQ) sqs[x] = 0ull;
+            if (SQ) sqs[x] = 0;
         }
     }
     uint32_t rs[BAND_ROWS];
@@ -229,7 +253,7 @@
         rq[r] = 0;
     }
     uint32_t top_s = 0;
-    uint64_t top_q = 0;
+    S top_q = 0;
     for (uint32_t x0 = 0; x0 < a.width; x0 += 256u) {
         const uint32_t x = x0 + lane * 4u;
         const bool in = x < a.width;
@@ -238,21 +262,17 @@
         for (int r = 0; r < BAND_ROWS; ++r)
             v[r] = in && y0 + r < a.height ? load_gray4(img + (size_t)(y0 + r) * a.gray_stride, x, a.width, a.channels) : 0u;
         uint32_t as[4] = {0, 0, 0, 0};
-        uint64_t aq[4] = {0, 0, 0, 0};
+        S aq[4] = {0, 0, 0, 0};
         if (in) {
             const uint4 t = *reinterpret_cast<const uint4*>(a.band_sum + bo + x);
             as[0] = t.x; as[1] = as[0] + t.y; as[2] = as[1] + t.z; as[3] = as[2] + t.w;
         }
-        if (in && SQ) {
-            const ulonglong2 u0 = *reinterpret_cast<const ulonglong2*>(a.band_sq_prefix + bo + x);
-            const ulonglong2 u1 = *reinterpret_cast<const ulonglong2*>(a.band_sq_prefix + bo + x + 2);
-            aq[0] = u0.x; aq[1] = aq[0] + u0.y; aq[2] = aq[1] + u1.x; aq[3] = aq[2] + u1.y;
-        }
+        if (in && SQ) load_sq_prefix4(a, bo + x, aq);
         {
             const uint32_t is = wave_incl_scan(as[3]);
-            const uint64_t iq = wave_incl_scan(aq[3]);
+            const S iq = wave_incl_scan(aq[3]);
             const uint32_t base_s = top_s + (is - as[3]);
-            const uint64_t base_q = top_q + (iq - aq[3]);
+            const S base_q = top_q + (iq - aq[3]);
 #pragma unroll
             for (int c = 0; c < 4; ++c) {
                 as[c] += base_s;
@@ -280,19 +300,16 @@
 #pragma unroll
                 for (int c = 0; c < 4; ++c) {
                     as[c] += base_s + ls[c];
-                    aq[c] += (uint64_t)(Q)(base_q + lq[c]);
+                    aq[c] += (S)(Q)(base_q + lq[c]);
                 }
                 const size_t ro = (size_t)(y + 1u) * ow;
                 if (x0 == 0 && lane == 0) {
                     sum[ro] = 0u;
-                    if (SQ) sqs[ro] = 0ull;
+                    if (SQ) sqs[ro] = 0;
                 }
                 if (x + 4u <= a.width) {
                     out_store<NT>(reinterpret_cast<u32x4_unaligned*>(sum + ro + x + 1u), u32x4_unaligned{as[0], as[1], as[2], as[3]});
-                    if (SQ) {
-                        out_store<NT>(reinterpret_cast<u64x2_unaligned*>(sqs + ro + x + 1u), u64x2_unaligned{aq[0], aq[1]});
-                        out_store<NT>(reinterpret_cast<u64x2_unaligned*>(sqs + ro + x + 3u), u64x2_unaligned{aq[2], aq[3]});
-                    }
+                    if (SQ) store_sq4<NT>(sqs + ro + x + 1u, aq);
                 } else {
 #pragma unroll
                     for (int c = 0; c < 4; ++c)
@@ -308,37 +325,38 @@
     }
 }
 
-template <typename Q>
-__global__ __launch_bounds__(256) void band_rows(IntegralArgs a) { band_rows_body<Q>(a); }
-template <typename Q>
-__global__ __launch_bounds__(256) __attribute__((amdgpu_waves_per_eu(3, 3))) void band_rows_w3(IntegralArgs a) { band_rows_body<Q, true>(a); }
+template <typename Q, typename S = uint64_t>
+__global__ __launch_bounds__(256) void band_rows(IntegralArgs a) { band_rows_body<Q, false, true, S>(a); }
+template <typename Q, typename S = uint64_t>
+__global__ __launch_bounds__(256) __attribute__((amdgpu_waves_per_eu(3, 3))) void band_rows_w3(IntegralArgs a) { band_rows_body<Q, true, true, S>(a); }
 __global__ __launch_bounds__(256) void band_rows_sum(IntegralArgs a) { band_rows_body<uint32_t, false, false>(a); }
 
-template <typename Q>
+template <typename Q, typename S = uint64_t>
 __global__ __launch_bounds__(512) void band_rows_par(IntegralArgs a) {
+    static_assert(sizeof(S) == 8 || sizeof(Q) == 4, "a 32-bit squared integral scans its rows in 32 bits");
     __shared__ uint32_t tot_s[2][BAND_ROWS + 1][8];
-    __shared__ uint64_t tot_q[2][BAND_ROWS + 1][8];
+    __shared__ S tot_q[2][BAND_ROWS + 1][8];
     const uint32_t lane = lane_id();
     const uint32_t w = __builtin_amdgcn_readfirstlane(threadIdx.x >> 6), nw = blockDim.x >> 6;
     const uint32_t band = blockIdx.x, frame = blockIdx.y;
     const uint8_t* img = a.gray + (size_t)frame * a.gray_frame_bytes;
     uint32_t* sum = a.sum + (size_t)frame * a.frame_elems;
-    uint64_t* sqs = a.sqsum + (size_t)frame * a.frame_elems;
+    S* sqs = reinterpret_cast<S*>(a.sqsum) + (size_t)frame * a.frame_elems;
     const uint32_t ow = a.width + 1u;
     const uint32_t y0 = band * BAND_ROWS;
     const size_t bo = ((size_t)frame * a.n_bands + band) * a.band_pitch;
     if (band == 0) {
         for (uint32_t x = threadIdx.x; x < ow; x += blockDim.x) {
             sum[x] = 0u;
-            sqs[x] = 0ull;
+            sqs[x] = 0;
         }
     }
     uint32_t carry_s[BAND_ROWS + 1];
-    uint64_t carry_q[BAND_ROWS + 1];
+    S carry_q[BAND_ROWS + 1];
 #pragma unroll
     for (int r = 0; r <= BAND_ROWS; ++r) {
         carry_s[r] = 0u;
-        carry_q[r] = 0ull;
+        carry_q[r] = 0;
     }
     uint32_t buf = 0;
     for (uint32_t x0 = 0; x0 < a.width; x0 += 256u * nw, buf ^= 1u) {
@@ -349,20 +367,18 @@
         for (int r = 0; r < BAND_ROWS; ++r)
             v[r] = in && y0 + r < a.height ? load_gray4(img + (size_t)(y0 + r) * a.gray_stride, x, a.width, a.channels) : 0u;
         uint32_t as[4] = {0, 0, 0, 0};
-        uint64_t aq[4] = {0, 0, 0, 0};
+        S aq[4] = {0, 0, 0, 0};
         if (in) {
             const uint4 t = *reinterpret_cast<const uint4*>(a.band_sum + bo + x);
             as[0] = t.x; as[1] = as[0] + t.y; as[2] = as[1] + t.z; as[3] = as[2] + t.w;
-            const ulonglong2 u0 = *reinterpret_cast<const ulonglong2*>(a.band_sq_prefix + bo + x);
-            const ulonglong2 u1 = *reinterpret_cast<const ulonglong2*>(a.band_sq_prefix + bo + x + 2);
-            aq[0] = u0.x; aq[1] = aq[0] + u0.y; aq[2] = aq[1] + u1.x; aq[3] = aq[2] + u1.y;
+            load_sq_prefix4(a, bo + x, aq);
         }
         uint32_t ex_s[BAND_ROWS + 1], t_s[BAND_ROWS + 1];
-        uint64_t ex_top_q, t_q[BAND_ROWS + 1];
+        S ex_top_q, t_q[BAND_ROWS + 1];
         Q ex_q[BAND_ROWS];
         {
             const uint32_t is = wave_incl_scan(as[3]);
-            const uint64_t iq = wave_incl_scan(aq[3]);
+            const S iq = wave_incl_scan(aq[3]);
             ex_s[0] = is - as[3];
             ex_top_q = iq - aq[3];
             t_s[0] = wave_last(is);
@@ -383,7 +399,7 @@
             ex_s[1 + r] = is - ls;
             ex_q[r] = iq - lq;
             t_s[1 + r] = wave_last(is);
-            t_q[1 + r] = (uint64_t)wave_last(iq);
+            t_q[1 + r] = (S)wave_last(iq);
         }
         if (lane == 0) {
 #pragma unroll
@@ -394,11 +410,11 @@
         }
         __syncthreads();
         uint32_t pre_s = 0, all_s = 0;
-        uint64_t pre_q = 0, all_q = 0;
+        S pre_q = 0, all_q = 0;
         if (lane <= (uint32_t)BAND_ROWS) {
             for (uint32_t k = 0; k < nw; ++k) {
                 const uint32_t ts = tot_s[buf][lane][k];
-                const uint64_t tq = tot_q[buf][lane][k];
+                const S tq = tot_q[buf][lane][k];
                 if (k < w) {
                     pre_s += ts;
                     pre_q += tq;
@@ -408,24 +424,27 @@
             }
         }
         auto lane_u32 = [&](uint32_t val, int r) { return (uint32_t)__builtin_amdgcn_readlane((int)val, r); };
-        auto lane_u64 = [&](uint64_t val, int r) { return (uint64_t)lane_u32((uint32_t)val, r) | (uint64_t)lane_u32((uint32_t)(val >> 32), r) << 32; };
+        auto lane_q = [&](S val, int r) -> S {
+            if constexpr (sizeof(S) == 8) return (uint64_t)lane_u32((uint32_t)val, r) | (uint64_t)lane_u32((uint32_t)((uint64_t)val >> 32), r) << 32;
+            else return lane_u32(val, r);
+        };
         {
             const uint32_t base_s = carry_s[0] + lane_u32(pre_s, 0) + ex_s[0];
-            const uint64_t base_q = carry_q[0] + lane_u64(pre_q, 0) + ex_top_q;
+            const S base_q = carry_q[0] + lane_q(pre_q, 0) + ex_top_q;
 #pragma unroll
             for (int c = 0; c < 4; ++c) {
                 as[c] += base_s;
                 aq[c] += base_q;
             }
             carry_s[0] += lane_u32(all_s, 0);
-            carry_q[0] += lane_u64(all_q, 0);
+            carry_q[0] += lane_q(all_q, 0);
         }
 #pragma unroll
         for (int r = 0; r < BAND_ROWS; ++r) {
             const uint32_t y = y0 + r;
             if (y < a.height) {
                 const uint32_t base_s = carry_s[1 + r] + lane_u32(pre_s, 1 + r) + ex_s[1 + r];
-                const Q base_q = (Q)(carry_q[1 + r] + lane_u64(pre_q, 1 + r)) + ex_q[r];
+                const Q base_q = (Q)(carry_q[1 + r] + lane_q(pre_q, 1 + r)) + ex_q[r];
                 uint32_t ls = 0;
                 Q lq = 0;
 #pragma unroll
@@ -434,17 +453,16 @@
                     ls += p;
                     lq += (Q)(p * p);
                     as[c] += base_s + ls;
-                    aq[c] += (uint64_t)(Q)(base_q + lq);
+                    aq[c] += (S)(Q)(base_q + lq);
                 }
                 const size_t ro = (size_t)(y + 1u) * ow;
                 if (x == 0u) {
                     sum[ro] = 0u;
-                    sqs[ro] = 0ull;
+                    sqs[ro] = 0;
                 }
                 if (x + 4u <= a.width) {
                     out_store<false>(reinterpret_cast<u32x4_unaligned*>(sum + ro + x + 1u), u32x4_unaligned{as[0], as[1], as[2], as[3]});
-                    out_store<false>(reinterpret_cast<u64x2_unaligned*>(sqs + ro + x + 1u), u64x2_unaligned{aq[0], aq[1]});
-                    out_store<false>(reinterpret_cast<u64x2_unaligned*>(sqs + ro + x + 3u), u64x2_unaligned{aq[2], aq[3]});
+                    store_sq4<false>(sqs + ro + x + 1u, aq);
                 } else {
 #pragma unroll
                     for (int c = 0; c < 4; ++c)
@@ -454,7 +472,7 @@
                         }
                 }
                 carry_s[1 + r] += lane_u32(all_s, 1 + r);
-                carry_q[1 + r] += lane_u64(all_q, 1 + r);
+                carry_q[1 + r] += lane_q(all_q, 1 + r);
             }
         }
     }
@@ -474,26 +492,38 @@
     dim3 g1((quads + 255u) / 256u, a.n_bands, a.n_frames);
     hipLaunchKernelGGL(band_colsum, g1, dim3(256), 0, stream, a);
     const dim3 g2b((a.band_pitch + 63u) / 64u, a.n_frames, 1);
-    if (a.n_bands <= 16u * 8u) hipLaunchKernelGGL(band_scan2<8>, g2b, dim3(1024), 0, stream, a);
-    else if (a.n_bands <= 16u * 16u) hipLaunchKernelGGL(band_scan2<16>, g2b, dim3(1024), 0, stream, a);
-    else if (a.n_bands <= 16u * 32u) hipLaunchKernelGGL(band_scan2<32>, g2b, dim3(1024), 0, stream, a);
-    else {
+    const bool q32 = a.sq_u32 != 0u;
+    if (a.n_bands <= 16u * 8u) {
+        if (q32) hipLaunchKernelGGL((band_scan2<8, uint32_t>), g2b, dim3(1024), 0, stream, a);
+        else hipLaunchKernelGGL((band_scan2<8, uint64_t>), g2b, dim3(1024), 0, stream, a);
+    } else if (a.n_bands <= 16u * 16u) {
+        if (q32) hipLaunchKernelGGL((band_scan2<16, uint32_t>), g2b, dim3(1024), 0, stream, a);
+        else hipLaunchKernelGGL((band_scan2<16, uint64_t>), g2b, dim3(1024), 0, stream, a);
+    } else if (a.n_bands <= 16u * 32u) {
+        if (q32) hipLaunchKernelGGL((band_scan2<32, uint32_t>), g2b, dim3(1024), 0, stream, a);
+        else hipLaunchKernelGGL((band_scan2<32, uint64_t>), g2b, dim3(1024), 0, stream, a);
+    } else {
         dim3 g2((a.band_pitch + 255u) / 256u, a.n_frames, 1);
-        hipLaunchKernelGGL(band_scan, g2, dim3(256), 0, stream, a);
+        if (q32) hipLaunchKernelGGL(band_scan<uint32_t>, g2, dim3(256), 0, stream, a);
+        else hipLaunchKernelGGL(band_scan<uint64_t>, g2, dim3(256), 0, stream, a);
     }
     if (a.rows_mode != 0u) {
         const bool batch_p = (uint64_t)a.n_frames * a.n_bands >= 2048u;
         if (a.rows_mode == 1u || !batch_p) {
             const uint32_t nw = min(8u, (a.width + 255u) / 256u);
             dim3 gp(a.n_bands, a.n_frames, 1);
-            if ((uint64_t)a.width * 65025ull < (1ull << 32)) hipLaunchKernelGGL(band_rows_par<uint32_t>, gp, dim3(64u * nw), 0, stream, a);
+            if (q32) hipLaunchKernelGGL((band_rows_par<uint32_t, uint32_t>), gp, dim3(64u * nw), 0, stream, a);
+            else if ((uint64_t)a.width * 65025ull < (1ull << 32)) hipLaunchKernelGGL(band_rows_par<uint32_t>, gp, dim3(64u * nw), 0, stream, a);
             else hipLaunchKernelGGL(band_rows_par<uint64_t>, gp, dim3(64u * nw), 0, stream, a);
             return (int)hipGetLastError();
         }
     }
     dim3 g3((a.n_bands + 3u) / 4u, a.n_frames, 1);
     const bool batch = (uint64_t)a.n_frames * a.n_bands >= 2048u;
-    if ((uint64_t)a.width * 65025ull < (1ull << 32)) {
+    if (q32) {
+        if (batch) hipLaunchKernelGGL((band_rows_w3<uint32_t, uint32_t>), g3, dim3(256), 0, stream, a);
+        else hipLaunchKernelGGL((band_rows<uint32_t, uint32_t>), g3, dim3(256), 0, stream, a);
+    } else if ((uint64_t)a.width * 65025ull < (1ull << 32)) {
         if (batch) hipLaunchKernelGGL(band_rows_w3<uint32_t>, g3, dim3(256), 0, stream, a);
         else hipLaunchKernelGGL(band_rows<uint32_t>, g3, dim3(256), 0, stream, a);
     } else {
@@ -524,15 +554,29 @@
     return ((a.skip_bits[(size_t)frame * a.skip_frame_words + word] >> bit) & 1ull) != 0ull;
 }
 
+__device__ __forceinline__ rsrc_t sq_frame_rsrc(const CascadeArgs& a, uint32_t frame, bool sq_u32) {
+    const uint32_t frame_bytes = a.frame_elems * (sq_u32 ? 4u : 8u);
+    return make_rsrc(reinterpret_cast<const char*>(a.sqsum) + (size_t)frame * frame_bytes, frame_bytes);
+}
+
+__device__ __forceinline__ float window_sq_f32(rsrc_t sq_f, uint32_t e, uint32_t c0, uint32_t e_dw, uint32_t e_dh, bool sq_u32,
+                                               uint32_t strip) {
+    if (!sq_u32)
+        return (float)(uint64_t)(ld_u64(sq_f, e * 8u, c0 * 8u) - ld_u64(sq_f, e * 8u, (c0 + e_dw) * 8u) -
+                                 ld_u64(sq_f, e * 8u, (c0 + e_dh) * 8u) + ld_u64(sq_f, e * 8u, (c0 + e_dh + e_dw) * 8u));
+    if (strip == 0u)
+        return (float)(uint32_t)(ld_u32(sq_f, e * 4u, c0 * 4u) - ld_u32(sq_f, e * 4u, (c0 + e_dw) * 4u) -
+                                 ld_u32(sq_f, e * 4u, (c0 + e_dh) * 4u) + ld_u32(sq_f, e * 4u, (c0 + e_dh + e_dw) * 4u));
+    return (float)sq_window_strips([&](uint32_t i) { return ld_u32(sq_f, e * 4u, i * 4u); }, c0, e_dw, e_dh, strip);
+}
+
 __device__ __forceinline__ float window_variance(rsrc_t sum_f, rsrc_t sq_f, uint32_t e, uint32_t e_lt, uint32_t e_dw,
-                                                 uint32_t e_dh, float area, bool signed_mean) {
+                                                 uint32_t e_dh, float area, bool signed_mean, bool sq_u32, uint32_t sq_strip) {
     const uint32_t c0 = e_lt, c1 = e_lt + e_dw, c2 = e_lt + e_dh, c3 = e_lt + e_dh + e_dw;
     const uint32_t s = ld_u32(sum_f, e * 4u, c0 * 4u) - ld_u32(sum_f, e * 4u, c1 * 4u) - ld_u32(sum_f, e * 4u, c2 * 4u) +
                        ld_u32(sum_f, e * 4u, c3 * 4u);
-    const uint64_t q = ld_u64(sq_f, e * 8u, c0 * 8u) - ld_u64(sq_f, e * 8u, c1 * 8u) - ld_u64(sq_f, e * 8u, c2 * 8u) +
-                       ld_u64(sq_f, e * 8u, c3 * 8u);
     const float mean = (signed_mean ? (float)(int32_t)s : (float)s) / area;
-    float variance = (float)q;
+    float variance = window_sq_f32(sq_f, e, c0, e_dw, e_dh, sq_u32, sq_strip);
     variance = (variance / area) - (mean * mean);
     return variance >= 0.0f ? sqrtf(variance) : 1.0f;
 }
@@ -1118,7 +1162,9 @@
             const float area = scales[slot].area;
             const size_t frame_off = (size_t)frame * a.frame_elems;
             const rsrc_t sum_f = make_rsrc(a.sum + frame_off, frame_bytes4);
-            const rsrc_t sq_f = make_rsrc(a.sqsum + frame_off, frame_bytes4 * 2u);
+            const bool sq_u32 = a.sq_u32 != 0u;
+            const uint32_t sq_strip = scales[slot].sq_strip;
+            const rsrc_t sq_f = sq_frame_rsrc(a, frame, sq_u32);
             const uint32_t frame_bytes = frame * frame_bytes4;
             const uint32_t bw = units[r].bw, ny = scales[slot].ny;
             uint32_t n_q = 0;
@@ -1141,7 +1187,7 @@
                     const uint32_t x = window_pos(a, pos_base, ix, step);
                     const uint32_t y = window_pos(a, pos_base, iy, step);
                     const uint32_t e = y * a.stride + x;
-                    en.var = window_variance(sum_f, sq_f, e, e_lt, e_dw, e_dh, area, a.signed_mean != 0u);
+                    en.var = window_variance(sum_f, sq_f, e, e_lt, e_dw, e_dh, area, a.signed_mean != 0u, sq_u32, sq_strip);
                     en.off = frame_bytes + e * 4u;
                 }
                 const unsigned long long mask = __ballot(valid);
@@ -1342,11 +1388,11 @@
         if (lane < count) {
             const size_t frame_off = (size_t)frame * a.frame_elems;
             const rsrc_t sum_f = make_rsrc(a.sum + frame_off, frame_bytes4);
-            const rsrc_t sq_f = make_rsrc(a.sqsum + frame_off, frame_bytes4 * 2u);
+            const rsrc_t sq_f = sq_frame_rsrc(a, frame, a.sq_u32 != 0u);
             const uint32_t x = window_pos(a, pos_base, ix, step), y = window_pos(a, pos_base, iy, step);
             const uint32_t e = y * a.stride + x;
             const float var = window_variance(sum_f, sq_f, e, scales[slot].e_lt, scales[slot].e_dw, scales[slot].e_dh, scales[slot].area,
-                                              a.signed_mean != 0u);
+                                              a.signed_mean != 0u, a.sq_u32 != 0u, scales[slot].sq_strip);
             kptr<NodeRecDev> tab = as_k(reinterpret_cast<const NodeRecDev*>(a.table)) + scales[slot].table_first + stages[0].first_node;
             fail = !(stage_sum_of<TREES>(GlobalImg{img}, tab, stages[0].n_nodes, frame * frame_bytes4 + e * 4u, var) >= stages[0].threshold);
         }
@@ -1494,7 +1540,7 @@
                 const uint32_t x = x0 + (uint32_t)__float2int_rn((float)ix * step);
                 const uint32_t y = y0 + (uint32_t)__float2int_rn((float)iy * step);
                 const uint32_t e = y * a.stride + x;
-                en.var = window_variance(sum_f, sq_f, e, e_lt, e_dw, e_dh, area, a.signed_mean != 0u);
+                en.var = window_variance(sum_f, sq_f, e, e_lt, e_dw, e_dh, area, a.signed_mean != 0u, false, 0u);
                 en.off = frame_bytes + e * 4u;
             }
             const unsigned long long mask = __ballot(valid);
@@ -2029,7 +2075,8 @@
         const uint32_t frame_bytes = frame * frame_bytes4;
         const size_t frame_off = (size_t)frame * a.frame_elems;
         const rsrc_t sum_f = make_rsrc(a.sum + frame_off, frame_bytes4);
-        const rsrc_t sq_f = make_rsrc(a.sqsum + frame_off, frame_bytes4 * 2u);
+        const bool sq_u32 = !ROI && a.sq_u32 != 0u;
+        const rsrc_t sq_f = sq_frame_rsrc(a, frame, sq_u32);
         const uint32_t x0 = ox + __builtin_amdgcn_readfirstlane(window_pos(a, scales[slot0].pos_base, ix0, step));
         const uint32_t y0 = oy + __builtin_amdgcn_readfirstlane(window_pos(a, scales[slot0].pos_base, iy0, step));
 
@@ -2099,7 +2146,13 @@
                     const uint32_t e = y * a.stride + x;
                     w_lo4[k] = ((y - y0) * pitch + (half ? (x - x0) >> 1 : x - x0)) * 4u;
                     const uint32_t c0 = e_lt, c1 = e_lt + e_dw, c2 = e_lt + e_dh, c3 = e_lt + e_dh + e_dw;
-                    if (sq32)
+                    if (sq_u32) {
+                        if (sq32)
+                            w_q[k] = (float)(uint32_t)(ld_u32(sq_f, e * 4u, c0 * 4u) - ld_u32(sq_f, e * 4u, c1 * 4u) -
+                                                       ld_u32(sq_f, e * 4u, c2 * 4u) + ld_u32(sq_f, e * 4u, c3 * 4u));
+                        else
+                            w_q[k] = window_sq_f32(sq_f, e, c0, e_dw, e_dh, true, scales[slot].sq_strip);
+                    } else if (sq32)
                         w_q[k] = (float)(uint32_t)(ld_u32(sq_f, e * 8u, c0 * 8u) - ld_u32(sq_f, e * 8u, c1 * 8u) -
                                                    ld_u32(sq_f, e * 8u, c2 * 8u) + ld_u32(sq_f, e * 8u, c3 * 8u));
                     else
diff --git a/clfacedetection_amd/csrc/vj_sq_strips.hpp b/clfacedetection_amd/csrc/vj_sq_strips.hpp
--- /dev/null
+++ b/clfacedetection_amd/csrc/vj_sq_strips.hpp
@@ -0,0 +1,27 @@
+#pragma once
+#include <stdint.h>
+
+namespace vj {
+
+constexpr uint32_t SQ32_MAX_AREA = 66051;
+static_assert(65025ull * SQ32_MAX_AREA < (1ull << 32) && 65025ull * (SQ32_MAX_AREA + 1ull) >= (1ull << 32), "SQ32_MAX_AREA");
+
+constexpr uint32_t sq_strip_rows(uint32_t w) { return w == 0u || w > SQ32_MAX_AREA ? 0u : SQ32_MAX_AREA / w; }
+constexpr uint32_t sq_strip_count(uint32_t h, uint32_t rows) { return (h + rows - 1u) / rows; }
+
+template <typename Ld>
+constexpr uint64_t sq_window_strips(Ld ld, uint32_t c0, uint32_t dw, uint32_t dh, uint32_t strip) {
+    uint64_t q = 0;
+    if (strip == 0u) strip = dh;
+    uint32_t top_l = ld(c0), top_r = ld(c0 + dw);
+    for (uint32_t off = 0; off < dh;) {
+        off += strip < dh - off ? strip : dh - off;
+        const uint32_t bot_l = ld(c0 + off), bot_r = ld(c0 + off + dw);
+        q += (uint32_t)(bot_r - bot_l - top_r + top_l);
+        top_l = bot_l;
+        top_r = bot_r;
+    }
+    return q;
+}
+
+}
diff --git a/include/vj.h b/include/vj.h
--- a/include/vj.h
+++ b/include/vj.h
@@ -161,6 +161,7 @@
 
 struct vj_image;
 int  vj_integral_image(vj_env* e, const struct vj_image* image, uint32_t* sum, uint64_t* sqsum);
+int  vj_integral_batch_sq32(vj_env* e, const struct vj_image* frames, int n_frames, uint32_t* sum, uint32_t* sqsum32);
 int  vj_grayscale(vj_env* e, const struct vj_image* image, uint8_t* gray, int gray_stride);
 int  vj_integral_tilted(vj_env* e, const struct vj_image* image, uint32_t* tilted);
 int  vj_canny(vj_env* e, const struct vj_image* image, uint8_t* edges, int edges_stride);
```

New measurement: 11.74 billion windows/s, median of 6. 2.2% higher.
